# potamides/DeTikZify

Hardware: AMD Instinct MI355X
Metric: tikz_tokens_per_sec (higher is better)
Workload: dtype bf16; 1 GPU; detikzify-ds-7b (synthetic weights, seed 1234), 1 image 224x224->384x384, 243-token prefix, greedy decode of 512 tokens per rollout, batch 1 per GPU, hipGraph per token; rollouts_per_gpu=5

## Files before the change

### detikzify_amd/_lib.py

```python
from __future__ import annotations

import ctypes as C
import os
from pathlib import Path

_HERE = Path(__file__).resolve().parent
LIB_PATH = _HERE / "lib" / "libdtk_hip.so"

DTK_ABI_VERSION = 7
DTK_VIT_BATCH = 8
DTK_F32, DTK_BF16, DTK_F16 = 0, 1, 2
DTK_ARCH_PROJ_NO_BIAS = 1
DTK_PREFILL_REUSE_PREFIX, DTK_PREFILL_REUSE_IMAGE = 1, 2
DTK_MAX_INFLIGHT = 4
DTK_MAX_BATCH = 64
DTK_MAX_TOP = 8
DTK_EPI_BIAS, DTK_EPI_GELU, DTK_EPI_RESIDUAL, DTK_GEMM_NAIVE = 1, 2, 4, 256
DTK_GEMM_WT = 512
DTK_GEMM_SL = 1024
DTK_GEMM_KSLICES_SHIFT = 12


class DtkConfig(C.Structure):
    _fields_ = [
        ("hidden", C.c_int32), ("layers", C.c_int32), ("heads", C.c_int32), ("head_dim", C.c_int32),
        ("ffn", C.c_int32), ("vocab", C.c_int32), ("max_positions", C.c_int32),
        ("rms_eps", C.c_float), ("rope_theta", C.c_float), ("rope_factor", C.c_float),
        ("vit_dim", C.c_int32), ("vit_depth", C.c_int32), ("vit_heads", C.c_int32),
        ("vit_mlp", C.c_int32), ("vit_patch", C.c_int32), ("vit_image", C.c_int32),
        ("vit_feature_layer", C.c_int32), ("vit_ln_eps", C.c_float), ("vit_gelu_tanh", C.c_int32),
        ("concat_patches", C.c_int32), ("image_token_id", C.c_int32), ("attn_splits", C.c_int32),
        ("reserved", C.c_int32 * 7),
    ]


class DtkAdapterConfig(C.Structure):
    _fields_ = [
        ("every_n", C.c_int32), ("text_max", C.c_int32),
        ("hidden", C.c_int32), ("layers", C.c_int32), ("heads", C.c_int32), ("kv_heads", C.c_int32), ("head_dim", C.c_int32),
        ("ffn", C.c_int32), ("vocab", C.c_int32), ("rms_eps", C.c_float), ("rope_theta", C.c_float), ("rope_factor", C.c_float),
        ("rope_low_freq_factor", C.c_float), ("rope_high_freq_factor", C.c_float), ("rope_original_max_position", C.c_int32),
        ("reserved", C.c_int32 * 3),
    ]


class DtkSampling(C.Structure):
    _fields_ = [
        ("do_sample", C.c_int32), ("temperature", C.c_float), ("top_p", C.c_float),
        ("top_k", C.c_int32), ("seed", C.c_uint64),
        ("n_bad", C.c_int32), ("bad_ids", C.c_int32 * 8),
        ("n_begin_suppress", C.c_int32), ("begin_suppress_ids", C.c_int32 * 8),
        ("n_always_suppress", C.c_int32), ("always_suppress_ids", C.c_int32 * 8),
    ]


class DtkSamplingExt(C.Structure):
    _fields_ = [("min_p", C.c_float), ("epsilon_cutoff", C.c_float), ("reserved", C.c_int32 * 6)]


class DtkStats(C.Structure):
    _fields_ = [
        ("weight_bytes_per_token", C.c_uint64), ("kv_bytes_per_ctx_token", C.c_uint64),
        ("decode_steps", C.c_uint64), ("prefill_tokens", C.c_uint64), ("vit_images", C.c_uint64),
        ("last_prefill_ms", C.c_double), ("last_vit_ms", C.c_double),
        ("probe_kernel_ms_sum", C.c_double), ("probe_kernel_launches", C.c_uint64),
        ("probe_kernel_bytes", C.c_uint64), ("probe_event_pair_ms", C.c_double),
        ("last_batch_step_slots", C.c_uint32), ("device_errors", C.c_uint32),
        ("last_batch_step_fp8_mfma", C.c_uint32), ("reserved0", C.c_uint32),
    ]


class DtkJoin(C.Structure):
    _fields_ = [
        ("slot", C.c_int32), ("n_ids", C.c_int32), ("ids", C.c_void_p), ("pixels", C.c_void_p), ("image_key", C.c_uint64),
        ("try_resume", C.c_int32), ("n_candidates", C.c_int32), ("candidates", C.c_int32 * DTK_MAX_BATCH),
        ("prefix_len", C.c_int32), ("prefix_src", C.c_int32), ("prefix_src_whole", C.c_int32), ("prefix_encode", C.c_int32),
        ("prefix_in_place", C.c_int32), ("full_flags", C.c_int32), ("sampling", DtkSampling),
        ("max_new_tokens", C.c_int32), ("n_stop", C.c_int32), ("stop_ids", C.c_int64 * 8),
        ("flush_mode", C.c_int32), ("flush_max", C.c_int32), ("slot_out", C.c_int32), ("how_out", C.c_int32),
        ("error_out", C.c_char * 240),
    ]


class DtkEngineStats(C.Structure):
    _fields_ = [(n, C.c_uint64) for n in ("steps", "tokens_out", "joins", "resumed", "steps_below_half_occupancy", "host_bound_steps",
                                          "reader_wakeups", "wasted_slot_steps")] + \
               [(n, C.c_double) for n in ("wait_s", "launch_s", "join_s", "idle_s", "drain_s", "first_launch_t", "last_collect_t")]


_I32P, _I64P = C.POINTER(C.c_int32), C.POINTER(C.c_int64)


class DtkEngineOps(C.Structure):
    LAUNCH = C.CFUNCTYPE(C.c_int, C.c_void_p, _I32P)
    WAIT = C.CFUNCTYPE(C.c_int, C.c_void_p, _I64P)
    PREFILL = C.CFUNCTYPE(C.c_int, C.c_void_p, C.c_int, _I64P, C.c_int, C.c_void_p, C.c_uint64, C.c_int)
    SAMPLING = C.CFUNCTYPE(C.c_int, C.c_void_p, C.c_int, C.POINTER(DtkSampling))
    FORK = C.CFUNCTYPE(C.c_int, C.c_void_p, C.c_int, C.c_int, C.c_int)
    LCP = C.CFUNCTYPE(C.c_int, C.c_void_p, C.c_int, _I64P, C.c_int, C.c_uint64, C.POINTER(C.c_int))
    RESUME = C.CFUNCTYPE(C.c_int, C.c_void_p, C.c_int, _I64P, C.c_int, C.c_uint64)
    CTXLEN = C.CFUNCTYPE(C.c_int, C.c_void_p, C.c_int)
    LASTERR = C.CFUNCTYPE(C.c_void_p, C.c_void_p)
    PREFILL_TEXT = C.CFUNCTYPE(C.c_int, C.c_void_p, C.c_int, _I64P, C.c_int, C.c_void_p, C.c_uint64, _I64P, C.c_int, C.c_uint64, C.c_int)
    WAIT_LP = C.CFUNCTYPE(C.c_int, C.c_void_p, _I64P, C.POINTER(C.c_float), C.POINTER(C.c_float))
    SAMPLING_EXT = C.CFUNCTYPE(C.c_int, C.c_void_p, C.c_int, C.POINTER(DtkSamplingExt))
    PENALTIES = C.CFUNCTYPE(C.c_int, C.c_void_p, C.c_int, C.c_float, C.c_float, C.c_int)
    _fields_ = [
        ("dev", C.c_void_p), ("launch", LAUNCH), ("wait", WAIT), ("prefill_slot", PREFILL), ("set_sampling_slot", SAMPLING),
        ("kv_fork", FORK), ("slot_lcp", LCP), ("resume_slot", RESUME), ("context_len_slot", CTXLEN), ("last_error", LASTERR),
        ("max_positions", C.c_int32), ("decode_slots", C.c_int32),
    ]


DTK_JOIN_FULL, DTK_JOIN_FORK_TAIL, DTK_JOIN_FORK_WHOLE, DTK_JOIN_RESUMED, DTK_JOIN_IN_PLACE = range(5)
DTK_SEQ_RUNNING, DTK_SEQ_FINISHED, DTK_SEQ_LEFT = 1, 2, 3

_P = C.c_void_p
SYMBOLS = {
    "dtk_abi_version": (C.c_int, []),
    "dtk_abi_struct_size": (C.c_int, [C.c_int]),
    "dtk_last_error": (C.c_char_p, [_P]),
# ... 22 lines not shown
    "dtk_engine_create": (C.c_int, [_P, C.POINTER(_P)]),
    "dtk_engine_create_ops": (C.c_int, [C.POINTER(DtkEngineOps), C.POINTER(_P)]),
    "dtk_engine_destroy": (None, [_P]),
    "dtk_engine_last_error": (C.c_char_p, [_P]),
    "dtk_engine_set_flush_tokens": (C.c_int, [_P, C.POINTER(C.c_int64), C.c_int]),
    "dtk_engine_set_option": (C.c_int, [_P, C.c_char_p, C.c_int]),
    "dtk_engine_expect": (C.c_int, [_P, C.c_int, C.c_int]),
    "dtk_engine_join": (C.c_int, [_P, C.POINTER(DtkJoin)]),
    "dtk_engine_submit": (C.c_int, [_P, C.POINTER(DtkJoin), C.POINTER(C.c_uint64)]),
    "dtk_engine_await": (C.c_int, [_P, C.c_uint64]),
    "dtk_engine_read": (C.c_int, [_P, C.c_int, C.POINTER(C.c_int64), C.c_int, C.POINTER(C.c_int32), C.POINTER(C.c_int32), C.c_int]),
    "dtk_engine_leave": (C.c_int, [_P, C.c_int]),
    "dtk_engine_get_stats": (C.c_int, [_P, C.POINTER(DtkEngineStats)]),
    "dtk_engine_submit_text": (C.c_int, [_P, C.POINTER(DtkJoin), C.POINTER(C.c_int64), C.c_int, C.c_uint64, C.POINTER(C.c_uint64)]),
    "dtk_engine_set_prefill_text_op": (C.c_int, [_P, DtkEngineOps.PREFILL_TEXT]),
    "dtk_prefill_slot": (C.c_int, [_P, C.c_int, _P, C.c_int, _P, C.c_uint64, C.c_int, _P]),
    "dtk_set_sampling_slot": (C.c_int, [_P, C.c_int, C.POINTER(DtkSampling)]),
    "dtk_decode_batch_launch": (C.c_int, [_P, C.POINTER(C.c_int32)]),
    "dtk_decode_batch_wait": (C.c_int, [_P, C.POINTER(C.c_int64)]),
    "dtk_kv_fork": (C.c_int, [_P, C.c_int, C.c_int, C.c_int]),
    "dtk_get_logits_slot": (C.c_int, [_P, C.c_int, _P]),
    "dtk_context_len_slot": (C.c_int, [_P, C.c_int]),
    "dtk_slot_lcp": (C.c_int, [_P, C.c_int, _P, C.c_int, C.c_uint64, C.POINTER(C.c_int)]),
    "dtk_slot_cached_ids": (C.c_int, [_P, C.c_int, _P, C.c_int]),
    "dtk_resume_slot": (C.c_int, [_P, C.c_int, _P, C.c_int, C.c_uint64]),
    "dtk_bench_gemv": (C.c_int, [_P, C.c_int, C.c_int, C.c_int, C.POINTER(C.c_float)]),
    "dtk_set_gemv_variant": (C.c_int, [_P, C.c_int, C.c_int]),
    "dtk_set_option": (C.c_int, [_P, C.c_char_p, C.c_int]),
    "dtk_op_gemm": (C.c_int, [_P, _P, _P, _P, _P, C.c_int, C.c_int, C.c_int, C.c_int, _P]),
    "dtk_adapter_create": (C.c_int, [_P, C.POINTER(DtkAdapterConfig)]),
    "dtk_adapter_destroy": (C.c_int, [_P]),
    "dtk_has_adapter": (C.c_int, [_P]),
    "dtk_vit_encode_text": (C.c_int, [_P, _P, C.c_int, _P, C.c_int, C.c_uint64, _P, _P]),
    "dtk_prefill_text": (C.c_int, [_P, _P, C.c_int, _P, C.c_uint64, _P, C.c_int, C.c_uint64, C.c_int, _P]),
    "dtk_prefill_slot_text": (C.c_int, [_P, C.c_int, _P, C.c_int, _P, C.c_uint64, _P, C.c_int, C.c_uint64, C.c_int, _P]),
    "dtk_adapter_embed": (C.c_int, [_P, _P, C.c_int, _P]),
    "dtk_text_image_key": (C.c_uint64, [C.c_uint64, C.c_uint64]),
    "dtk_op_gemm_gated": (C.c_int, [_P, _P, _P, _P, _P, _P, C.c_int, C.c_int, C.c_int, C.c_int, _P]),
    "dtk_score": (C.c_int, [_P, _P, C.c_int, _P, C.c_uint64, C.c_uint32, C.c_int, _P, _P, _P]),
    "dtk_score_text": (C.c_int, [_P, _P, C.c_int, _P, C.c_uint64, _P, C.c_int, C.c_uint64, C.c_uint32, C.c_int, _P, _P, _P]),
    "dtk_op_score": (C.c_int, [_P, _P, _P, _P, C.c_int, C.c_int, C.c_int, C.c_int, _P, _P, _P, _P]),
    "dtk_score_packed": (C.c_int, [_P, _P, C.c_int, _P, C.c_uint64, C.c_uint32, _P, _P, C.c_int, _P, _P, _P]),
    "dtk_score_packed_text": (C.c_int, [_P, _P, C.c_int, _P, C.c_uint64, _P, C.c_int, C.c_uint64, C.c_uint32, _P, _P, C.c_int, _P, _P, _P]),
    "dtk_op_attention_seg": (C.c_int, [_P, _P, _P, _P, C.c_int, C.c_int, C.c_int, C.c_int, C.c_int, _P, _P, _P]),
    "dtk_op_attn_decode": (C.c_int, [_P, _P, _P, _P, C.c_int, C.c_int, C.c_int, C.c_int, _P, C.c_int, C.c_int, C.c_int, C.c_int, C.c_int,
                                     _P, _P, _P, _P]),
    "dtk_op_attn_decode_b": (C.c_int, [_P, _P, _P, _P, C.c_int, C.c_int, C.c_int, C.c_int, _P, _P, _P, _P,
                                       C.c_int, C.c_int, C.c_int, C.c_int, C.c_int, _P]),
    "dtk_op_gemv_b": (C.c_int, [_P, C.c_int, _P, _P, _P, C.c_int, C.c_int, _P, _P, C.c_float, _P, _P, C.c_int,
                                C.c_int, C.c_int, C.c_int, C.c_int, C.c_int, _P, _P, _P, _P, _P, _P, _P, _P, _P, _P]),
    "dtk_op_gemv_bkp": (C.c_int, [_P, _P, _P, _P, C.c_int, C.c_int, _P, _P, C.c_int, _P, C.c_float, _P, _P, _P, _P]),
    "dtk_op_gemv_role": (C.c_int, [_P, C.c_int, C.c_int, C.c_int, _P, _P, _P, _P, _P] + [C.c_int] * 9 + [C.c_float, _P, _P, _P, _P,
                                   C.c_int, _P, _P, _P, C.c_int, _P, _P, _P, _P, _P]),
    "dtk_op_gemv": (C.c_int, [_P, _P, _P, _P, C.c_int, C.c_int, C.c_int, C.c_float, _P]),
    "dtk_op_gemv_mv": (C.c_int, [_P, _P, _P, _P, C.c_int, C.c_int, C.c_int, C.c_float, C.c_int, _P]),
    "dtk_op_gemv_q4": (C.c_int, [_P, _P, _P, _P, C.c_int, C.c_int, C.c_int, C.c_float, _P, _P]),
    "dtk_mx_layout": (C.c_int, [C.c_int, C.c_int, C.c_int, _P, _P]),
    "dtk_op_gemv_mx": (C.c_int, [_P, _P, _P, _P, C.c_int, C.c_int, C.c_int, C.c_int, C.c_int, _P, _P, _P, _P, _P]),
    "dtk_op_attention": (C.c_int, [_P, _P, _P, _P, C.c_int, C.c_int, C.c_int, C.c_int, C.c_int, C.c_int, _P]),
    "dtk_op_layernorm": (C.c_int, [_P, _P, _P, _P, C.c_int, C.c_int, C.c_float, _P]),
    "dtk_op_sample": (C.c_int, [_P, _P, C.c_int, C.c_int, C.POINTER(C.c_int64), _P]),
    "dtk_decode_wait_lp": (C.c_int, [_P, C.POINTER(C.c_int64), C.POINTER(C.c_float)]),
    "dtk_decode_batch_wait_lp": (C.c_int, [_P, C.POINTER(C.c_int64), C.POINTER(C.c_float), C.POINTER(C.c_float)]),
    "dtk_engine_read_lp": (C.c_int, [_P, C.c_int, C.POINTER(C.c_int64), C.POINTER(C.c_float), C.POINTER(C.c_float), C.c_int,
                                     C.POINTER(C.c_int32), C.POINTER(C.c_int32), C.c_int]),
    "dtk_engine_set_wait_lp_op": (C.c_int, [_P, DtkEngineOps.WAIT_LP]),
    "dtk_op_sample_lp": (C.c_int, [_P, _P, C.c_int, C.c_int, C.POINTER(C.c_int64), _P, C.POINTER(C.c_float)]),
    "dtk_score_top": (C.c_int, [_P, _P, C.c_int, _P, C.c_uint64, C.c_uint32, C.c_int, _P, _P, _P, C.c_int, _P, _P]),
    "dtk_score_top_text": (C.c_int, [_P, _P, C.c_int, _P, C.c_uint64, _P, C.c_int, C.c_uint64, C.c_uint32, C.c_int, _P, _P, _P,
                                     C.c_int, _P, _P]),
    "dtk_score_packed_top": (C.c_int, [_P, _P, C.c_int, _P, C.c_uint64, C.c_uint32, _P, _P, C.c_int, _P, _P, _P, C.c_int, _P, _P]),
    "dtk_score_packed_top_text": (C.c_int, [_P, _P, C.c_int, _P, C.c_uint64, _P, C.c_int, C.c_uint64, C.c_uint32, _P, _P, C.c_int,
                                            _P, _P, _P, C.c_int, _P, _P]),
    "dtk_op_score_top": (C.c_int, [_P, _P, _P, _P, C.c_int, C.c_int, C.c_int, C.c_int, _P, _P, _P, _P, C.c_int, _P, _P, _P]),
    "dtk_decode_wait_top": (C.c_int, [_P, C.POINTER(C.c_int64), C.POINTER(C.c_float), C.POINTER(C.c_int32), C.POINTER(C.c_float)]),
    "dtk_decode_batch_wait_top": (C.c_int, [_P, C.POINTER(C.c_int64), C.POINTER(C.c_float), C.POINTER(C.c_float),
                                            C.POINTER(C.c_int32), C.POINTER(C.c_float)]),
    "dtk_set_sampling_ext": (C.c_int, [_P, C.POINTER(DtkSamplingExt)]),
    "dtk_set_sampling_slot_ext": (C.c_int, [_P, C.c_int, C.POINTER(DtkSamplingExt)]),
    "dtk_op_sample_ext": (C.c_int, [_P, _P, C.c_int, C.c_int, C.POINTER(C.c_int64), _P, C.POINTER(C.c_float), C.POINTER(DtkSamplingExt)]),
    "dtk_engine_submit_ext": (C.c_int, [_P, C.POINTER(DtkJoin), C.POINTER(DtkSamplingExt), C.POINTER(C.c_int64), C.c_int, C.c_uint64,
                                        C.POINTER(C.c_uint64)]),
    "dtk_engine_set_sampling_ext_op": (C.c_int, [_P, DtkEngineOps.SAMPLING_EXT]),
    "dtk_set_penalties": (C.c_int, [_P, C.c_float, C.c_float, C.c_int]),
    "dtk_set_penalties_slot": (C.c_int, [_P, C.c_int, C.c_float, C.c_float, C.c_int]),
    "dtk_op_sample_pen": (C.c_int, [_P, _P, C.c_int, C.c_int, C.POINTER(C.c_int64), _P, C.POINTER(C.c_float), C.POINTER(DtkSamplingExt),
                                    C.c_float, C.c_float, C.POINTER(C.c_int64), C.c_int]),
    "dtk_token_counts": (C.c_int, [_P, C.c_int, C.POINTER(C.c_uint16), C.c_int]),
    "dtk_engine_submit_pen": (C.c_int, [_P, C.POINTER(DtkJoin), C.POINTER(DtkSamplingExt), C.c_float, C.c_float, C.c_int,
                                        C.POINTER(C.c_int64), C.c_int, C.c_uint64, C.POINTER(C.c_uint64)]),
    "dtk_engine_set_penalties_op": (C.c_int, [_P, DtkEngineOps.PENALTIES]),
}

_lib = None


class DtkError(RuntimeError):
    pass


def load_library() -> C.CDLL:
    global _lib
    if _lib is not None:
        return _lib
    if not LIB_PATH.exists():
        raise DtkError(
# ... 37 lines not shown
```

### detikzify_amd/csrc/dtk_api.hip

```cpp
#include <hip/hip_runtime.h>

#include <cmath>
#include <cstdarg>
#include <cstdio>
#include <cstdlib>
#include <cstring>
#include <atomic>
#include <mutex>
#include <string>
#include <unordered_map>
#include <vector>

#include "../../include/dtk.h"
#include "kernels.h"
#include "mx_quant.h"

int& dtk_lds_attr_error(int device) {
  static int e[65] = {};
  return e[(device >= 0 && device < 64) ? device : 64];
}

namespace {

thread_local std::string g_create_error;
thread_local std::string g_thread_error;
thread_local const void* g_thread_error_ctx = nullptr;

struct TensorEntry {
  std::string name;
  bf16_t* ptr = nullptr;
  int64_t rows = 1;
  int64_t cols = 0;
  int64_t stride = 0;
  float synth_scale = 0.02f;
  float synth_offset = 0.f;
  bool loaded = false;
  int64_t numel() const { return rows * cols; }
};

struct SeqHost {
  std::vector<int64_t> cached_ids;
  bool cached_with_image = false;
  uint64_t image_key = 0;
  int host_next_pos = 0;
  bool have_logits = false;
  int share_src = -1;
  int share_len = 0;
  int last_reuse_start = 0;
  int64_t forced_pending = -1;
};

struct LayerW {
  bf16_t *wqkv, *wo, *wgu, *wdown, *ln1, *ln2;
  bf16_t *t_wqkv = nullptr, *t_wo = nullptr, *t_wgu = nullptr, *t_wdown = nullptr;
  bf16_t *p_wqkv = nullptr, *p_wo = nullptr, *p_wgu = nullptr, *p_wdown = nullptr;
  bf16_t* p_wgui = nullptr;
  uint8_t *q_wqkv = nullptr, *q_wo = nullptr, *q_wgu = nullptr, *q_wdown = nullptr;
  float *s_wqkv = nullptr, *s_wo = nullptr, *s_wgu = nullptr, *s_wdown = nullptr;
  uint8_t *f4_wqkv = nullptr, *f4_wo = nullptr, *f4_wgu = nullptr, *f4_wdown = nullptr;
  uint8_t *e4_wqkv = nullptr, *e4_wo = nullptr, *e4_wgu = nullptr, *e4_wdown = nullptr;
  uint8_t *t8_wqkv = nullptr, *t8_wo = nullptr, *t8_wgu = nullptr, *t8_wdown = nullptr;
  uint8_t *m_wqkv = nullptr, *m_wo = nullptr, *m_wgu = nullptr, *m_wdown = nullptr;
};
struct VitBlockW {
  bf16_t *n1w, *n1b, *qkvw, *qkvb, *projw, *projb, *n2w, *n2b, *fc1w, *fc1b, *fc2w, *fc2b;
};
struct CrossW {
  bf16_t *ln1w, *ln1b, *qw, *qb, *kw, *kb, *vw, *vb, *ow, *ob, *qnw, *qnb, *knw, *knb, *ln2w, *ln2b, *f1w, *f1b, *f2w, *f2b;
  bf16_t *gate_a, *gate_m;
  bf16_t *K, *V;
};
struct Adapter {
  dtk_adapter_config cfg{};
  dtk_ctx* emb = nullptr;
  unsigned char* arena = nullptr;
  size_t first_tensor = 0;
  bf16_t *conn_w = nullptr, *conn_b = nullptr, *dummy = nullptr, *ctext = nullptr;
  std::vector<CrossW> layers;
  std::vector<char> present;
  std::vector<int64_t> text_ids;
  std::vector<float> dummy_host;
};

}

struct dtk_ctx {
  dtk_config cfg;
  int device = 0;
  hipStream_t stream = nullptr;
  std::string err;
  std::mutex err_mu;
  std::mutex vit_mu;

  int d, L, H, ff, V, Tmax, S;
  int vD, vDepth, vH, vHd, vMlp, vN, vPatchK, vPatchLd, nImg;

  unsigned char* arena = nullptr;
  size_t arena_bytes = 0;
  std::vector<TensorEntry> tensors;
  std::unordered_map<std::string, int> tindex;
  std::vector<LayerW> layers;
  bf16_t *embed, *final_norm, *lm_head, *mm_w, *mm_b;
  bf16_t *rope_cos, *rope_sin;
  std::vector<VitBlockW> vblocks;
  bf16_t *pe_w, *pe_b, *pos_embed, *vnorm_w, *vnorm_b;
  bf16_t *ap_latent, *ap_qw, *ap_qb, *ap_kvw, *ap_kvb, *ap_pw, *ap_pb, *ap_nw, *ap_nb, *ap_f1w,
      *ap_f1b, *ap_f2w, *ap_f2b;

  bf16_t* kv = nullptr;

  bf16_t *X, *Xn, *QKV, *Qh, *AO, *GU, *ACT;
  int sk_sl_min_rows = SK_SL_MIN_ROWS;
  float* skpart = nullptr;
  size_t skpart_floats = 0;
  int swiglu_fused = 1;
  int qkv_rope_fused = 1;
  int prefill_sk = 1;
  int32_t* ids_dev = nullptr;
  float* score_rec = nullptr;
  float* score_out = nullptr;
  float* score_top = nullptr;
  int32_t* packed_rows = nullptr;
  bf16_t *x, *q, *act;
  float *logits, *pm, *pl, *po;
  bf16_t* attn_out = nullptr;
  unsigned* attn_ctr = nullptr;
  int attn_combine = 0;
  DecState* st = nullptr;
  SamplingDev* sp = nullptr;
  int64_t* tok_ring_dev = nullptr;
  int64_t* tok_ring_host = nullptr;
  float* probs_dev = nullptr;
  int logprobs = 0;
  std::atomic<int> engine_holds{0};
  float2* lp_ring_dev = nullptr;
  float2* lp_ring_host = nullptr;
  float2* lpb_dev = nullptr;
  float2* lpb_host = nullptr;
  int top_logprobs = 0;
  TopRec* top_ring_dev = nullptr;
  TopRec* top_ring_host = nullptr;
  float* lse_ring_dev = nullptr;
  float* lse_ring_host = nullptr;
  TopRec* topb_dev = nullptr;
  TopRec* topb_host = nullptr;
  float* lseb_dev = nullptr;
  float* lseb_host = nullptr;
  float* pixels_dev = nullptr;
  bf16_t *patches, *VX, *VN, *VQKV, *VAO, *VH, *feats, *last_hidden;
  bf16_t *pq, *pkv, *pao, *px, *pn, *ph, *pooled;
  bf16_t* IMG;
  Adapter* ad = nullptr;
  unsigned char* scratch = nullptr;
  size_t scratch_bytes = 0;

  SeqHost seq0;
  int wfmt = 0;
  bool fp8_ready = false;
  uint8_t* q_lm_head = nullptr;
  float* s_lm_head = nullptr;
  uint64_t cached_image_key = 0;
  bool have_image = false;
  int KVH = 0;
  int hd = 128;
  bool proj_bias = true;
  int nb = 0;
  bool share_reads = true;
  int nt = 1;
  std::vector<SeqHost> bseq;
  bf16_t* kvb = nullptr;
  size_t kv_slot_stride = 0;
  bf16_t *xb = nullptr, *xnb = nullptr, *qb = nullptr, *aob = nullptr, *actb = nullptr;
  float* logits_b = nullptr;
  float* kpart = nullptr; unsigned* kctr = nullptr;
  int attn_nt = 1;
  bool resid_kparts = true;
  float *pfx_m = nullptr, *pfx_l = nullptr, *pfx_o = nullptr;
  int prefix_mfma = 0;
  int pfx_splits = 4;
  int gqa_fused = 1;
  int tail_threads = 256;
  DecState* st_b = nullptr;
  SamplingDev* sp_b = nullptr;
  BatchState* bs_dev = nullptr;
  bf16_t* t_lm_head = nullptr;
  uint8_t* t8_lm_head = nullptr;
  uint8_t* m_lm_head = nullptr;
  uint8_t *xn8 = nullptr, *xns = nullptr, *ao8 = nullptr, *aos = nullptr, *act8 = nullptr, *acts = nullptr;
  bool mx_ok = false;
  int act_fp8 = 0;
  bool launch_refused = false;
  bool tiled_ready = false;
  bool ptiled_ready = false;
  BatchState* bs_host = nullptr;
  SamplingDev* sp_stage = nullptr; uint32_t* draw_stage = nullptr;
  DecState* st_stage = nullptr;
  int64_t* tokb_dev = nullptr;
  int64_t* tokb_host = nullptr;
  uint64_t blaunched = 0, bwaited = 0;
  hipEvent_t bstep_done[DTK_MAX_INFLIGHT] = {};
  bool bgraph_ready[6] = {false, false, false, false, false, false};
  hipGraph_t bgraph[6] = {nullptr, nullptr, nullptr, nullptr, nullptr, nullptr};
  hipGraphExec_t bgraph_exec[6] = {nullptr, nullptr, nullptr, nullptr, nullptr, nullptr};
  int nt_step = 1;
  int mv_slots = 4;
  int mv_step = 0;
  int mv_tail_threads = 512;
  dtk_sampling sampling{};
  SampleMB* smb = nullptr;
  SampleMB* smb_b = nullptr;
  bool mb_single = false;
  bool mb_batch = false;
  bool slot_topk[DTK_MAX_SLOTS] = {};
// ... 493 lines not shown
    a.nbatch = B; a.q_sb = 0; a.k_sb = a.v_sb = (long)N * 2 * D; a.o_sb = D;
    launch_attention(a, s);
  }
  gemm(c, c->pao, D, c->ap_pw, D, c->ap_pb, nullptr, 0, c->px, D, B, D, D, GEMM_BIAS);
  launch_layernorm_rows(c->px, D, c->ap_nw, c->ap_nb, c->pn, D, B, D, c->cfg.vit_ln_eps, s);
  gemm(c, c->pn, D, c->ap_f1w, D, c->ap_f1b, nullptr, 0, c->ph, mlp, B, mlp, D, GEMM_BIAS | gelu_flag(c));
  gemm(c, c->ph, mlp, c->ap_f2w, mlp, c->ap_f2b, c->px, D, c->pooled, D, B, D, mlp, GEMM_BIAS | GEMM_RESIDUAL);
}

void project_image(dtk_ctx* c) {
  const int K = c->cfg.concat_patches * c->vD;
  gemm(c, c->feats, K, c->mm_w, K, c->proj_bias ? c->mm_b : nullptr, nullptr, 0, c->IMG, c->d, c->nImg, c->d, K,
       c->proj_bias ? GEMM_BIAS : 0);
}

#define TOKB_ERR ((size_t)DTK_MAX_INFLIGHT * DTK_MAX_BATCH)
#define TOKB_WORDS (TOKB_ERR + 1)
static inline unsigned* batch_err_word(const dtk_ctx* c) { return reinterpret_cast<unsigned*>(c->tokb_dev + TOKB_ERR); }

#define LPB_BYTES (sizeof(float2) * (size_t)DTK_MAX_INFLIGHT * DTK_MAX_BATCH)
static inline hipError_t copy_lp_ring(dtk_ctx* c, bool batch) {
  if (!c->logprobs) return hipSuccess;
  if (c->top_logprobs) {
    hipError_t e = batch ? hipMemcpyAsync(c->topb_host, c->topb_dev, sizeof(TopRec) * (size_t)DTK_MAX_INFLIGHT * DTK_MAX_BATCH, hipMemcpyDeviceToHost, c->stream)
                         : hipMemcpyAsync(c->top_ring_host, c->top_ring_dev, sizeof(TopRec) * DTK_MAX_INFLIGHT, hipMemcpyDeviceToHost, c->stream);
    if (e != hipSuccess) return e;
    e = batch ? hipMemcpyAsync(c->lseb_host, c->lseb_dev, sizeof(float) * (size_t)DTK_MAX_INFLIGHT * DTK_MAX_BATCH, hipMemcpyDeviceToHost, c->stream)
              : hipMemcpyAsync(c->lse_ring_host, c->lse_ring_dev, sizeof(float) * DTK_MAX_INFLIGHT, hipMemcpyDeviceToHost, c->stream);
    if (e != hipSuccess) return e;
  }
  return batch ? hipMemcpyAsync(c->lpb_host, c->lpb_dev, LPB_BYTES, hipMemcpyDeviceToHost, c->stream)
               : hipMemcpyAsync(c->lp_ring_host, c->lp_ring_dev, sizeof(float2) * DTK_MAX_INFLIGHT, hipMemcpyDeviceToHost, c->stream);
}

static void pen_args(const dtk_ctx* c, SampleArgs& sa, bool batch) {
  if (!(batch ? c->pen_batch : c->pen_single) || !c->pen_tab) return;
  const int first = batch ? 1 : 0;
  sa.pen = c->pen_dev + first; sa.pen_cnt = c->pen_tab + (size_t)first * c->pen_stride; sa.pen_stride = c->pen_stride; sa.pen_tok = c->pen_tok + first;
}
static void sampler_launch(dtk_ctx* c, SampleArgs& sa, bool mb, bool batch) {
  pen_args(c, sa, batch);
  if (mb) launch_sample_mb(sa, c->stream); else launch_sample_b(sa, c->stream);
  if (sa.pen) launch_count_token(sa, c->stream);
}

static void top_logits_launch(dtk_ctx* c, const SampleArgs& sa) {
  if (!c->top_logprobs || !c->logprobs) return;
  TopArgs t;
  t.logits = sa.logits; t.V = sa.V; t.logits_stride = sa.logits_stride; t.st = sa.st; t.bs = sa.bs; t.nslots = sa.nslots;
  t.ring = sa.ring; t.k = c->top_logprobs; t.top_ring = sa.bs ? c->topb_dev : c->top_ring_dev;
  launch_top_logits(t, c->stream);
}

void decode_step_launches(dtk_ctx* c, bool with_probe, bool short_ctx = false) {
  hipStream_t s = c->stream;
  SampleArgs sa;
  sa.logits = c->logits; sa.V = c->V; sa.sp = c->sp; sa.st = c->st; sa.embed = c->embed;
  sa.x = c->x; sa.d = c->d; sa.tok_ring = c->tok_ring_dev; sa.ring = DTK_MAX_INFLIGHT;
  sa.probs_out = nullptr; sa.advance = 1; sa.step_override = -1; sa.bs = nullptr; sa.logits_stride = 0; sa.nslots = 1; sa.mb = c->smb;
  sa.lp_ring = c->logprobs ? c->lp_ring_dev : nullptr;
  sa.trunc = c->trunc_single ? 1 : 0;
  sa.lse_ring = (c->logprobs && c->top_logprobs) ? c->lse_ring_dev : nullptr;
  top_logits_launch(c, sa);
  sampler_launch(c, sa, c->mb_single, false);
  const float scale = 1.0f / sqrtf((float)c->hd);
  for (int l = 0; l < c->L; ++l) {
    const LayerW& w = c->layers[l];
    GemvArgs g{};
    g.eps = c->cfg.rms_eps; g.st = c->st; g.T_max = c->Tmax; g.d = c->d; g.ff = c->ff; g.H = c->H; g.KVH = c->KVH; g.hd = c->hd;
    g.rope_cos = c->rope_cos; g.rope_sin = c->rope_sin;
    g.pm = c->pm; g.pl = c->pl; g.po = c->po; g.S = c->S;
    g.W = w.wqkv; g.W8 = w.q_wqkv; g.wscale = w.s_wqkv; g.N = c->d + 2 * c->KVH * c->hd; g.K = c->d; g.x = c->x; g.norm_w = w.ln1;
    g.W4 = w.f4_wqkv; g.S4 = w.e4_wqkv;
    g.q_out = c->q; g.kcache = kcache(c, l); g.vcache = vcache(c, l);
    launch_gemv(PRO_RMSNORM, EPI_QKV, g, s);
    AttnDecArgs ad;
    ad.q = c->q; ad.kcache = kcache(c, l); ad.vcache = vcache(c, l); ad.st = c->st;
    ad.pm = c->pm; ad.pl = c->pl; ad.po = c->po; ad.H = c->H; ad.S = c->S; ad.T_max = c->Tmax; ad.G = c->H / c->KVH;
    ad.scale = scale; ad.hd = c->hd;
    ad.threads = c->attn_threads;
    ad.combine = (!ad.threads && short_ctx && c->attn_combine == 2) ? 3 : c->attn_combine; ad.out = c->attn_out; ad.counters = c->attn_ctr;
    if (ad.threads && ad.combine == 1) ad.combine = 2;
    launch_attn_decode(ad, s);
    g.W = w.wo; g.W8 = w.q_wo; g.wscale = w.s_wo; g.N = c->d; g.K = c->d; g.y = c->x;
    g.W4 = w.f4_wo; g.S4 = w.e4_wo;
    const bool partials = ad.combine == 0 && !(ad.threads && ad.S == 1);
    if (!partials) { g.x = c->attn_out; launch_gemv(PRO_COPY, EPI_RESID, g, s); }
    else launch_gemv(PRO_ATTN, EPI_RESID, g, s);
    g.W = w.wgu; g.W8 = w.q_wgu; g.wscale = w.s_wgu; g.N = 2 * c->ff; g.K = c->d; g.x = c->x; g.norm_w = w.ln2; g.y = c->act;
    g.W4 = w.f4_wgu; g.S4 = w.e4_wgu;
    const bool probe_here = with_probe && (l == c->L / 2);
    if (probe_here) (void)hipEventRecord(c->probe_a, s);
    launch_gemv(PRO_RMSNORM, EPI_SWIGLU, g, s);
    if (probe_here) (void)hipEventRecord(c->probe_b, s);
    g.W = w.wdown; g.W8 = w.q_wdown; g.wscale = w.s_wdown; g.N = c->d; g.K = c->ff; g.x = c->act; g.y = c->x;
    g.W4 = w.f4_wdown; g.S4 = w.e4_wdown;
    launch_gemv(PRO_COPY, EPI_RESID, g, s);
  }
  GemvArgs g{};
  g.W = c->lm_head; g.W8 = c->q_lm_head; g.wscale = c->s_lm_head; g.N = c->V; g.K = c->d; g.x = c->x; g.norm_w = c->final_norm;
  g.eps = c->cfg.rms_eps; g.logits = c->logits;
  launch_gemv(PRO_RMSNORM, EPI_LOGITS, g, s);
}

static inline bool mx_step(const dtk_ctx* c) { return c->wfmt == 1 && c->mx_ok && c->act_fp8 != 0; }

void batch_step_launches_mx(dtk_ctx* c) {
  hipStream_t s = c->stream;
  const int d = c->d, ff = c->ff, nslots = 16 * c->nt_step;
  SampleArgs sa;
  sa.logits = c->logits_b; sa.V = c->V; sa.sp = c->sp_b; sa.st = c->st_b; sa.embed = c->embed;
  sa.x = c->xb; sa.d = d; sa.tok_ring = c->tokb_dev; sa.ring = DTK_MAX_INFLIGHT;
  sa.probs_out = nullptr; sa.advance = 1; sa.step_override = -1; sa.bs = c->bs_dev; sa.logits_stride = c->V; sa.nslots = nslots; sa.mb = c->smb_b;
  sa.lp_ring = c->logprobs ? c->lpb_dev : nullptr;
  sa.trunc = c->trunc_batch ? 1 : 0;
  sa.lse_ring = (c->logprobs && c->top_logprobs) ? c->lseb_dev : nullptr;
  top_logits_launch(c, sa);
  sampler_launch(c, sa, c->mb_batch, true);
  const float scale = 1.0f / sqrtf(128.f);
  const size_t kv_layer = (size_t)2 * c->KVH * c->Tmax * 128;
  for (int l = 0; l < c->L; ++l) {
    const LayerW& w = c->layers[l];
    bf16_t* kc = c->kvb + (size_t)l * kv_layer;
    bf16_t* vc = kc + (size_t)c->KVH * c->Tmax * 128;
    GemvBArgs g{};
    g.bs = c->bs_dev; g.st = c->st_b; g.T_max = c->Tmax; g.d = d; g.ff = ff; g.H = c->H; g.KVH = c->KVH; g.nt = c->nt_step;
    g.rope_cos = c->rope_cos; g.rope_sin = c->rope_sin; g.kv_slot_stride = c->kv_slot_stride; g.kpart = c->kpart; g.err = batch_err_word(c);
    if (l == 0) launch_rmsnorm_b(c->xb, d, w.ln1, c->xnb, d, d, c->cfg.rms_eps, c->bs_dev, nslots, s, c->xn8, c->xns);
    g.Wm = w.m_wqkv; g.wscale = w.s_wqkv; g.N = d + 2 * c->KVH * 128; g.K = d; g.X8 = c->xn8; g.XS = c->xns; g.q_out = c->qb; g.kcache = kc; g.vcache = vc;
    launch_gemv_mxu(EPI_QKV, g, s);
    AttnDecBArgs ad;
    ad.q = c->qb; ad.kcache = kc; ad.vcache = vc; ad.kv_slot_stride = c->kv_slot_stride; ad.st = c->st_b; ad.bs = c->bs_dev;
    ad.out = c->aob; ad.H = c->H; ad.T_max = c->Tmax; ad.d = d; ad.G = c->H / c->KVH; ad.nslots = nslots;
    ad.scale = scale;
    ad.use_prefix = c->prefix_mfma; ad.pfx_splits = c->pfx_splits; ad.tail_threads = c->tail_threads; ad.gqa_fused = c->gqa_fused; ad.nt_private = c->attn_nt;
    ad.pfx_m = c->pfx_m; ad.pfx_l = c->pfx_l; ad.pfx_o = c->pfx_o;
    ad.out8 = c->ao8; ad.outs = c->aos;
    launch_attn_decode_b(ad, s);
    g.Wm = w.m_wo; g.wscale = w.s_wo; g.N = d; g.K = d; g.X8 = c->ao8; g.XS = c->aos;
    if (!launch_gemv_mxk(g, 32, s)) c->launch_refused = true;
    launch_resid_norm_b(c->kpart, c->xb, d, w.ln2, c->xnb, d, c->cfg.rms_eps, c->bs_dev, nslots, s, c->xn8, c->xns);
    g.Wm = w.m_wgu; g.wscale = w.s_wgu; g.N = 2 * ff; g.K = d; g.X8 = c->xn8; g.XS = c->xns; g.Y8 = c->act8; g.YS = c->acts;
    launch_gemv_mxu(EPI_SWIGLU, g, s);
    g.Wm = w.m_wdown; g.wscale = w.s_wdown; g.N = d; g.K = ff; g.X8 = c->act8; g.XS = c->acts;
    if (!launch_gemv_mxk(g, 16, s)) c->launch_refused = true;
    launch_resid_norm_b(c->kpart, c->xb, d, l + 1 < c->L ? c->layers[l + 1].ln1 : c->final_norm, c->xnb, d, c->cfg.rms_eps, c->bs_dev, nslots, s, c->xn8, c->xns);
  }
  GemvBArgs g{};
  g.bs = c->bs_dev; g.st = c->st_b; g.Wm = c->m_lm_head; g.wscale = c->s_lm_head; g.N = c->V; g.K = d; g.X8 = c->xn8; g.XS = c->xns; g.logits = c->logits_b;
  g.d = d; g.ff = ff; g.nt = c->nt_step; g.H = c->H; g.KVH = c->KVH; g.err = batch_err_word(c);
  launch_gemv_mxu(EPI_LOGITS, g, s);
}
// ... 84 lines not shown
  const float scale = 1.0f / sqrtf(128.f);
  const size_t kv_layer = (size_t)2 * c->KVH * c->Tmax * 128;
  GemvMvArgs g{};
  g.bs = c->bs_dev; g.st = c->st_b; g.T_max = c->Tmax; g.d = d; g.ff = ff; g.H = c->H; g.KVH = c->KVH; g.eps = c->cfg.rms_eps;
  g.rope_cos = c->rope_cos; g.rope_sin = c->rope_sin; g.kv_slot_stride = c->kv_slot_stride;
  for (int l = 0; l < c->L; ++l) {
    const LayerW& w = c->layers[l];
    bf16_t* kc = c->kvb + (size_t)l * kv_layer;
    bf16_t* vc = kc + (size_t)c->KVH * c->Tmax * 128;
    g.W = w.wqkv; g.W8 = w.q_wqkv; g.wscale = w.s_wqkv; g.N = d + 2 * c->KVH * 128; g.K = d; g.X = c->xb; g.ldx = d; g.norm_w = w.ln1;
    g.q_out = c->qb; g.kcache = kc; g.vcache = vc;
    launch_gemv_mv(PRO_RMSNORM, EPI_QKV, NB, g, s);
    AttnDecBArgs ad;
    ad.q = c->qb; ad.kcache = kc; ad.vcache = vc; ad.kv_slot_stride = c->kv_slot_stride; ad.st = c->st_b; ad.bs = c->bs_dev;
    ad.out = c->aob; ad.H = c->H; ad.T_max = c->Tmax; ad.d = d; ad.G = c->H / c->KVH; ad.nslots = NB;
    ad.scale = scale;
    ad.use_prefix = 0; ad.pfx_splits = c->pfx_splits; ad.tail_threads = c->mv_tail_threads; ad.gqa_fused = c->gqa_fused; ad.nt_private = c->attn_nt;
    ad.pfx_m = c->pfx_m; ad.pfx_l = c->pfx_l; ad.pfx_o = c->pfx_o;
    launch_attn_decode_b(ad, s);
    g.W = w.wo; g.W8 = w.q_wo; g.wscale = w.s_wo; g.N = d; g.K = d; g.X = c->aob; g.Y = c->xb; g.ldy = d;
    launch_gemv_mv(PRO_COPY, EPI_RESID, NB, g, s);
    g.W = w.wgu; g.W8 = w.q_wgu; g.wscale = w.s_wgu; g.N = 2 * ff; g.K = d; g.X = c->xb; g.ldx = d; g.norm_w = w.ln2; g.Y = c->actb; g.ldy = ff;
    launch_gemv_mv(PRO_RMSNORM, EPI_SWIGLU, NB, g, s);
    g.W = w.wdown; g.W8 = w.q_wdown; g.wscale = w.s_wdown; g.N = d; g.K = ff; g.X = c->actb; g.Y = c->xb; g.ldy = d;
    launch_gemv_mv(PRO_COPY, EPI_RESID, NB, g, s);
  }
  g.W = c->lm_head; g.W8 = c->q_lm_head; g.wscale = c->s_lm_head; g.N = c->V; g.K = d; g.X = c->xb; g.ldx = d; g.norm_w = c->final_norm;
  g.logits = c->logits_b;
  launch_gemv_mv(PRO_RMSNORM, EPI_LOGITS, NB, g, s);
}

void ensure_fp8_weights(dtk_ctx* c) {
  if (c->wfmt == 0 || c->fp8_ready) return;
  for (int l = 0; l < c->L && c->wfmt == 2; ++l) {
    LayerW& w = c->layers[l];
    launch_quant_mxfp4_rows(w.wqkv, w.f4_wqkv, w.e4_wqkv, c->d + 2 * c->KVH * c->hd, c->d, c->stream);
    launch_quant_mxfp4_rows(w.wo, w.f4_wo, w.e4_wo, c->d, c->d, c->stream);
    launch_quant_mxfp4_rows(w.wgu, w.f4_wgu, w.e4_wgu, 2 * c->ff, c->d, c->stream);
    launch_quant_mxfp4_rows(w.wdown, w.f4_wdown, w.e4_wdown, c->d, c->ff, c->stream);
  }
  for (int l = 0; l < c->L && c->wfmt == 1; ++l) {
    LayerW& w = c->layers[l];
    launch_quant_fp8_rows(w.wqkv, w.q_wqkv, w.s_wqkv, c->d + 2 * c->KVH * c->hd, c->d, c->stream);
    launch_quant_fp8_rows(w.wo, w.q_wo, w.s_wo, c->d, c->d, c->stream);
    launch_quant_fp8_rows(w.wgu, w.q_wgu, w.s_wgu, 2 * c->ff, c->d, c->stream);
    launch_quant_fp8_rows(w.wdown, w.q_wdown, w.s_wdown, c->d, c->ff, c->stream);
  }
  launch_quant_fp8_rows(c->lm_head, c->q_lm_head, c->s_lm_head, c->V, c->d, c->stream);
  c->fp8_ready = true;
  c->tiled_ready = false;
  c->ptiled_ready = false;
}

void ensure_tiled_weights(dtk_ctx* c);
void ensure_prefill_tiles(dtk_ctx* c) {
  ensure_fp8_weights(c);
  if (c->ptiled_ready) return;
  for (int l = 0; l < c->L; ++l)
    if (c->layers[l].p_wgui) launch_retile_pairs(c->layers[l].wgu, c->layers[l].p_wgui, c->ff, c->d, c->stream);
  if (c->nb > 0 && c->wfmt != 1) { ensure_tiled_weights(c); c->ptiled_ready = true; return; }
  for (int l = 0; l < c->L; ++l) {
    LayerW& w = c->layers[l];
    launch_retile(w.wqkv, w.p_wqkv, c->d + 2 * c->KVH * c->hd, c->d, c->stream);
    launch_retile(w.wo, w.p_wo, c->d, c->d, c->stream);
    launch_retile(w.wgu, w.p_wgu, 2 * c->ff, c->d, c->stream);
    launch_retile(w.wdown, w.p_wdown, c->d, c->ff, c->stream);
  }
  c->ptiled_ready = true;
}

void ensure_tiled_weights(dtk_ctx* c) {
  ensure_fp8_weights(c);
  if (c->tiled_ready || c->nb <= 0) return;
  if (c->wfmt == 1) {
    const int qkvn = c->d + 2 * c->KVH * 128;
    for (int l = 0; l < c->L; ++l) {
      LayerW& w = c->layers[l];
      launch_retile_f8(w.q_wqkv, w.t8_wqkv, qkvn, c->d, c->stream);
      launch_retile_f8(w.q_wo, w.t8_wo, c->d, c->d, c->stream);
      launch_retile_f8(w.q_wgu, w.t8_wgu, 2 * c->ff, c->d, c->stream);
      launch_retile_f8(w.q_wdown, w.t8_wdown, c->d, c->ff, c->stream);
    }
    launch_retile_f8(c->q_lm_head, c->t8_lm_head, c->V, c->d, c->stream);
    if (c->mx_ok) {
      for (int l = 0; l < c->L; ++l) {
        LayerW& w = c->layers[l];
        launch_retile_mx(w.q_wqkv, w.m_wqkv, qkvn, c->d, 32, c->stream);
        launch_retile_mx(w.q_wo, w.m_wo, c->d, c->d, 32, c->stream);
        launch_retile_mx(w.q_wgu, w.m_wgu, 2 * c->ff, c->d, 32, c->stream);
        launch_retile_mx(w.q_wdown, w.m_wdown, c->d, c->ff, 16, c->stream);
      }
      launch_retile_mx(c->q_lm_head, c->m_lm_head, c->V, c->d, 32, c->stream);
    }
    c->tiled_ready = true;
    return;
  }
  for (int l = 0; l < c->L; ++l) {
    LayerW& w = c->layers[l];
    launch_retile(w.wqkv, w.t_wqkv, c->d + 2 * c->KVH * 128, c->d, c->stream);
    launch_retile(w.wo, w.t_wo, c->d, c->d, c->stream);
    launch_retile(w.wgu, w.t_wgu, 2 * c->ff, c->d, c->stream);
    launch_retile(w.wdown, w.t_wdown, c->d, c->ff, c->stream);
  }
  launch_retile(c->lm_head, c->t_lm_head, c->V, c->d, c->stream);
  c->tiled_ready = true;
}
// ... 232 lines not shown
  if (const char* fm = getenv("DTK_ATTN_FULL_MAX")) c->attn_full_max = atoi(fm);
  if (const char* gv = getenv("DTK_GEMV_VARIANTS")) {
    int e = 0, v = 0;
    const char* p = gv;
    while (sscanf(p, "%d:%d", &e, &v) == 2) {
      set_gemv_default_variant(e, v);
      p = strchr(p, ',');
      if (!p) break;
      ++p;
    }
  }

#define CCHK(call)                                                                         \
  do {                                                                                     \
    hipError_t e_ = (call);                                                                \
    if (e_ != hipSuccess) {                                                                \
      fail(nullptr, DTK_ERR_HIP, "%s failed: %s", #call, hipGetErrorString(e_));           \
      dtk_destroy(c);                                                                      \
      return DTK_ERR_HIP;                                                                  \
    }                                                                                      \
  } while (0)
  CCHK(hipSetDevice(device));
  CCHK(hipStreamCreateWithFlags(&c->stream, hipStreamNonBlocking));
  CCHK(hipStreamCreateWithFlags(&c->stream_vit, hipStreamNonBlocking));
  Planner sz;
  plan(c, sz, false);
  c->arena_bytes = align_up(sz.off, 256) + 256;
  CCHK(hipMalloc((void**)&c->arena, c->arena_bytes));
  Planner real;
  real.base = c->arena;
  plan(c, real, true);
  CCHK(hipMemsetAsync(c->arena, 0, c->arena_bytes, c->stream));
  CCHK(hipHostMalloc((void**)&c->tok_ring_host, sizeof(int64_t) * DTK_MAX_INFLIGHT, hipHostMallocDefault));
  CCHK(hipHostMalloc((void**)&c->lp_ring_host, sizeof(float2) * DTK_MAX_INFLIGHT, hipHostMallocDefault));
  for (int i = 0; i < DTK_MAX_INFLIGHT; ++i) CCHK(hipEventCreateWithFlags(&c->step_done[i], hipEventDisableTiming));
  if (c->nb > 0) {
    CCHK(hipHostMalloc((void**)&c->bs_host, sizeof(BatchState) * DTK_MAX_INFLIGHT, hipHostMallocDefault));
    CCHK(hipHostMalloc((void**)&c->tokb_host, sizeof(int64_t) * TOKB_WORDS, hipHostMallocDefault));
    CCHK(hipHostMalloc((void**)&c->lpb_host, LPB_BYTES, hipHostMallocDefault));
    CCHK(hipHostMalloc((void**)&c->st_stage, sizeof(DecState) * (DTK_MAX_SLOTS), hipHostMallocDefault));
    CCHK(hipHostMalloc((void**)&c->sp_stage, sizeof(SamplingDev) * (DTK_MAX_SLOTS), hipHostMallocDefault));
    CCHK(hipHostMalloc((void**)&c->draw_stage, sizeof(uint32_t) * (DTK_MAX_SLOTS), hipHostMallocDefault));
    for (int i = 0; i < DTK_MAX_INFLIGHT; ++i) CCHK(hipEventCreateWithFlags(&c->bstep_done[i], hipEventDisableTiming));
  }
  CCHK(hipEventCreate(&c->ev_a)); CCHK(hipEventCreate(&c->ev_b)); CCHK(hipEventCreate(&c->ev_c));
  CCHK(hipEventCreate(&c->ev_va)); CCHK(hipEventCreate(&c->ev_vb));
  CCHK(hipEventCreate(&c->probe_a)); CCHK(hipEventCreate(&c->probe_b));
  std::vector<uint16_t> cosv, sinv;
  compute_rope_tables(*cfg, cosv, sinv);
  CCHK(hipMemcpyAsync(c->rope_cos, cosv.data(), cosv.size() * 2, hipMemcpyHostToDevice, c->stream));
  CCHK(hipMemcpyAsync(c->rope_sin, sinv.data(), sinv.size() * 2, hipMemcpyHostToDevice, c->stream));
  CCHK(hipStreamSynchronize(c->stream));
#undef CCHK
  const uint64_t kvd = (uint64_t)c->KVH * c->hd;
  const uint64_t attn_lin = (uint64_t)2 * c->d * c->d + 2 * kvd * c->d;
  const uint64_t per_layer = attn_lin + (uint64_t)3 * c->d * c->ff + 2 * (uint64_t)c->d;
  c->stats.weight_bytes_per_token = 2 * (per_layer * c->L + (uint64_t)c->d + (uint64_t)c->V * c->d);
  if (c->wfmt == 1) {
    const uint64_t lin = attn_lin + (uint64_t)3 * c->d * c->ff;
    const uint64_t rows = (uint64_t)3 * c->d + 2 * kvd + (uint64_t)2 * c->ff;
    c->stats.weight_bytes_per_token = (lin + 4 * rows + 4 * (uint64_t)c->d) * c->L + 2 * (uint64_t)c->d + (uint64_t)c->V * c->d + 4 * (uint64_t)c->V;
  }
  if (c->wfmt == 2) {
    const uint64_t bd = mxfp4_row_scales(c->d), bf = mxfp4_row_scales(c->ff);
    const uint64_t blocks = ((uint64_t)2 * c->d + 2 * kvd + (uint64_t)2 * c->ff) * bd + (uint64_t)c->d * bf;
    c->stats.weight_bytes_per_token = (17 * blocks + 4 * (uint64_t)c->d) * c->L + 2 * (uint64_t)c->d + (uint64_t)c->V * c->d + 4 * (uint64_t)c->V;
  }
  c->stats.kv_bytes_per_ctx_token = (uint64_t)2 * c->L * kvd * 2;
  c->stats.probe_kernel_bytes = (uint64_t)2 * c->ff * c->d * (c->wfmt == 1 ? 1 : 2);
  if (c->wfmt == 2) c->stats.probe_kernel_bytes = (uint64_t)2 * c->ff * 17 * mxfp4_row_scales(c->d);
  *out = c;
  if (c->nb > 0) {
    const bool big = max_decode_slots(c) >= 64;
    c->prefix_mfma = big ? 1 : 0;
    c->tail_threads = big ? 128 : 256;
  }
  if (const char* opts = getenv("DTK_OPTIONS")) {
    std::string all(opts);
    size_t at = 0;
    while (at < all.size()) {
      size_t end = all.find(',', at);
      if (end == std::string::npos) end = all.size();
      const std::string item = all.substr(at, end - at);
      const size_t eq = item.find('=');
      if (eq != std::string::npos && dtk_set_option(c, item.substr(0, eq).c_str(), atoi(item.c_str() + eq + 1)) != DTK_OK)
        fprintf(stderr, "DTK_OPTIONS: %s rejected (%s)\n", item.c_str(), c->err.c_str());
      at = end + 1;
    }
  }
  return DTK_OK;
}

void dtk_destroy(dtk_ctx* c) {
  if (!c) return;
  (void)hipSetDevice(c->device);
  if (c->ad) (void)dtk_adapter_destroy(c);
  if (c->stream) (void)hipStreamSynchronize(c->stream);
  if (c->graph_exec) (void)hipGraphExecDestroy(c->graph_exec);
  if (c->graph) (void)hipGraphDestroy(c->graph);
  if (c->graph_short_exec) (void)hipGraphExecDestroy(c->graph_short_exec);
  if (c->graph_short) (void)hipGraphDestroy(c->graph_short);
  drop_batch_graphs(c);
  for (int i = 0; i < DTK_MAX_INFLIGHT; ++i) if (c->bstep_done[i]) (void)hipEventDestroy(c->bstep_done[i]);
  if (c->bs_host) (void)hipHostFree(c->bs_host);
  if (c->tokb_host) (void)hipHostFree(c->tokb_host);
  if (c->lpb_host) (void)hipHostFree(c->lpb_host);
  if (c->lp_ring_host) (void)hipHostFree(c->lp_ring_host);
  if (c->st_stage) (void)hipHostFree(c->st_stage);
  if (c->sp_stage) (void)hipHostFree(c->sp_stage);
  if (c->draw_stage) (void)hipHostFree(c->draw_stage);
  for (int i = 0; i < DTK_MAX_INFLIGHT; ++i) if (c->step_done[i]) (void)hipEventDestroy(c->step_done[i]);
  hipEvent_t evs[] = {c->ev_a, c->ev_b, c->ev_c, c->probe_a, c->probe_b};
  for (hipEvent_t e : evs) if (e) (void)hipEventDestroy(e);
  if (c->tok_ring_host) (void)hipHostFree(c->tok_ring_host);
  if (c->arena) (void)hipFree(c->arena);
  if (c->score_rec) (void)hipFree(c->score_rec);
  if (c->score_out) (void)hipFree(c->score_out);
  if (c->score_top) (void)hipFree(c->score_top);
  if (c->pen_tab) (void)hipFree(c->pen_tab);
  if (c->pen_dev) (void)hipFree(c->pen_dev);
  if (c->pen_tok) (void)hipFree(c->pen_tok);
  if (c->pen_ids_dev) (void)hipFree(c->pen_ids_dev);
  if (c->pen_ids_stage) (void)hipHostFree(c->pen_ids_stage);
  if (c->pen_stage) (void)hipHostFree(c->pen_stage);
  if (c->top_ring_dev) (void)hipFree(c->top_ring_dev);
  if (c->lse_ring_dev) (void)hipFree(c->lse_ring_dev);
  if (c->topb_dev) (void)hipFree(c->topb_dev);
  if (c->lseb_dev) (void)hipFree(c->lseb_dev);
  if (c->top_ring_host) (void)hipHostFree(c->top_ring_host);
  if (c->lse_ring_host) (void)hipHostFree(c->lse_ring_host);
  if (c->topb_host) (void)hipHostFree(c->topb_host);
  if (c->lseb_host) (void)hipHostFree(c->lseb_host);
  if (c->packed_rows) (void)hipFree(c->packed_rows);
  if (c->stream_vit) (void)hipStreamDestroy(c->stream_vit);
  if (c->ev_va) (void)hipEventDestroy(c->ev_va);
  if (c->ev_vb) (void)hipEventDestroy(c->ev_vb);
  if (c->stream) (void)hipStreamDestroy(c->stream);
  delete c;
}

int dtk_num_tensors(const dtk_ctx* c) { return c ? (int)c->tensors.size() : 0; }
const char* dtk_tensor_name(const dtk_ctx* c, int i) {
  if (!c || i < 0 || i >= (int)c->tensors.size()) return nullptr;
  return c->tensors[i].name.c_str();
}
int64_t dtk_tensor_numel(const dtk_ctx* c, const char* name) {
  if (!c || !name) return -1;
  auto it = c->tindex.find(name);
  return it == c->tindex.end() ? -1 : c->tensors[it->second].numel();
}

int dtk_load_tensor(dtk_ctx* c, const char* name, const void* host, int dtype, const int64_t* shape, int ndim) {
  if (!c || !name || !host || !shape || ndim < 1) return fail(c, DTK_ERR_ARG, "dtk_load_tensor: null argument");
  auto it = c->tindex.find(name);
  if (it == c->tindex.end()) return fail(c, DTK_ERR_ARG, "unknown tensor '%s'", name);
  TensorEntry& t = c->tensors[it->second];
  int64_t n = 1;
  for (int i = 0; i < ndim; ++i) n *= shape[i];
  if (n != t.numel()) return fail(c, DTK_ERR_ARG, "tensor '%s': %lld elements given, %lld expected", name, (long long)n, (long long)t.numel());
  HIPCHK(c, hipSetDevice(c->device));
  std::vector<uint16_t> tmp;
  const uint16_t* src16 = nullptr;
  if (dtype == DTK_BF16) {
    src16 = static_cast<const uint16_t*>(host);
  } else if (dtype == DTK_F32) {
    tmp.resize((size_t)n);
    const float* f = static_cast<const float*>(host);
    for (int64_t i = 0; i < n; ++i) tmp[(size_t)i] = host_f2bf(f[i]);
    src16 = tmp.data();
  } else if (dtype == DTK_F16) {
    tmp.resize((size_t)n);
    const uint16_t* hf = static_cast<const uint16_t*>(host);
    for (int64_t i = 0; i < n; ++i) tmp[(size_t)i] = host_f2bf(host_h2f(hf[i]));
    src16 = tmp.data();
  } else {
    return fail(c, DTK_ERR_ARG, "bad dtype %d", dtype);
  }
  HIPCHK(c, hipStreamSynchronize(c->stream));
  HIPCHK(c, hipMemcpy2D(t.ptr, (size_t)t.stride * 2, src16, (size_t)t.cols * 2, (size_t)t.cols * 2, (size_t)t.rows, hipMemcpyHostToDevice));
  t.loaded = true;
  if (c->ad) { c->ad->text_ids.clear(); c->ad->dummy_host.clear(); c->ad->emb->ptiled_ready = false; }
  c->have_image = false;
  c->seq0.cached_ids.clear();
  for (auto& b : c->bseq) b.cached_ids.clear();
  pen_clear_all(c);
  c->tiled_ready = false;
  c->ptiled_ready = false;
  c->fp8_ready = false;
  return DTK_OK;
}

int dtk_read_tensor(dtk_ctx* c, const char* name, void* host_out, int64_t n_elems) {
  if (!c || !name || !host_out) return fail(c, DTK_ERR_ARG, "dtk_read_tensor: null argument");
  auto it = c->tindex.find(name);
  if (it == c->tindex.end()) return fail(c, DTK_ERR_ARG, "unknown tensor '%s'", name);
  const TensorEntry& t = c->tensors[it->second];
  if (n_elems != t.numel()) return fail(c, DTK_ERR_ARG, "tensor '%s' has %lld elements", name, (long long)t.numel());
  HIPCHK(c, hipSetDevice(c->device));
  ensure_fp8_weights(c);
  HIPCHK(c, hipStreamSynchronize(c->stream));
  HIPCHK(c, hipMemcpy2D(host_out, (size_t)t.cols * 2, t.ptr, (size_t)t.stride * 2, (size_t)t.cols * 2, (size_t)t.rows, hipMemcpyDeviceToHost));
  return DTK_OK;
}

int dtk_fill_synthetic(dtk_ctx* c, uint64_t seed) {
  if (!c) return DTK_ERR_ARG;
  HIPCHK(c, hipSetDevice(c->device));
  for (size_t i = 0; i < c->tensors.size(); ++i) {
    TensorEntry& t = c->tensors[i];
    if (t.name == "rope.cos" || t.name == "rope.sin" || t.name == "embedding_model.rope.cos" || t.name == "embedding_model.rope.sin") continue;
    t.loaded = true;
    if (t.stride == t.cols) {
      launch_fill_synth(t.ptr, t.numel(), seed, (uint32_t)i, t.synth_scale, t.synth_offset, c->stream);
    } else {
      if ((size_t)t.numel() * 2 > c->scratch_bytes) return fail(c, DTK_ERR_ARG, "scratch too small");
      bf16_t* tmp = reinterpret_cast<bf16_t*>(c->scratch);
      launch_fill_synth(tmp, t.numel(), seed, (uint32_t)i, t.synth_scale, t.synth_offset, c->stream);
      HIPCHK(c, hipMemcpy2DAsync(t.ptr, (size_t)t.stride * 2, tmp, (size_t)t.cols * 2, (size_t)t.cols * 2, (size_t)t.rows, hipMemcpyDeviceToDevice, c->stream));
    }
  }
  HIPCHK(c, hipStreamSynchronize(c->stream));
  if (c->ad) { c->ad->text_ids.clear(); c->ad->dummy_host.clear(); c->ad->emb->ptiled_ready = false; }
  c->have_image = false;
  c->seq0.cached_ids.clear();
  for (auto& b : c->bseq) b.cached_ids.clear();
  pen_clear_all(c);
  c->tiled_ready = false;
  c->ptiled_ready = false;
  c->fp8_ready = false;
  return DTK_OK;
}

static int vit_encode_impl(dtk_ctx* c, const float* pixels, int batch, void* feats_out, void* pooled_out, const int64_t* text_ids, int T_text);
static int text_prepare(dtk_ctx* c, const int64_t* ids, int T, hipStream_t s);
int dtk_vit_encode(dtk_ctx* c, const float* pixels, int batch, void* feats_out, void* pooled_out) {
  return vit_encode_impl(c, pixels, batch, feats_out, pooled_out, nullptr, 0);
}

static int vit_encode_impl(dtk_ctx* c, const float* pixels, int batch, void* feats_out, void* pooled_out, const int64_t* text_ids, int T_text) {
  if (!c || !pixels || batch < 1) return fail(c, DTK_ERR_ARG, "dtk_vit_encode: bad argument");
  if (pooled_out) {
    for (const TensorEntry& t : c->tensors)
      if (!t.loaded && t.name.compare(0, 23, "vision_model.attn_pool.") == 0)
        return fail(c, DTK_ERR_STATE, "pooler_output requested but '%s' was never loaded (checkpoint without the pooling head)", t.name.c_str());
  }
  std::lock_guard<std::mutex> vit_guard(c->vit_mu);
  HIPCHK(c, hipSetDevice(c->device));
  const size_t img = (size_t)3 * c->cfg.vit_image * c->cfg.vit_image;
  hipStream_t sv = c->stream_vit;
  const bf16_t* hidden = (pooled_out && c->cfg.vit_feature_layer != c->vDepth - 1) ? c->last_hidden : c->feats;
  if (text_ids) { const int rc = text_prepare(c, text_ids, T_text, sv); if (rc != DTK_OK) return rc; }
  for (int b0 = 0; b0 < batch; b0 += DTK_VIT_BATCH) {
    const int B = std::min(batch - b0, (int)DTK_VIT_BATCH);
    HIPCHK(c, hipMemcpyAsync(c->pixels_dev, pixels + (size_t)b0 * img, (size_t)B * img * 4, hipMemcpyHostToDevice, sv));
    HIPCHK(c, hipEventRecord(c->ev_va, sv));
    vit_forward(c, pooled_out != nullptr, sv, B, text_ids != nullptr);
    HIPCHK(c, hipEventRecord(c->ev_vb, sv));
    if (feats_out)
      HIPCHK(c, hipMemcpyAsync((bf16_t*)feats_out + (size_t)b0 * c->vN * c->vD, hidden, (size_t)B * c->vN * c->vD * 2, hipMemcpyDeviceToHost, sv));
    if (pooled_out)
      HIPCHK(c, hipMemcpyAsync((bf16_t*)pooled_out + (size_t)b0 * c->vD, c->pooled, (size_t)B * c->vD * 2, hipMemcpyDeviceToHost, sv));
    HIPCHK(c, hipStreamSynchronize(sv));
    HIPCHK(c, hipGetLastError());
    float ms = 0.f;
    if (hipEventElapsedTime(&ms, c->ev_va, c->ev_vb) == hipSuccess) c->stats.last_vit_ms = ms / (float)B;
    c->stats.vit_images += (uint64_t)B;
  }
  return DTK_OK;
}

struct PackedRows { const int2* rope; const int2* seg; int shared_len; };
static void decoder_layers(dtk_ctx* c, int n, int start, int T, bf16_t* kvbase, hipStream_t s, const PackedRows* pk = nullptr) {
  const int hd = c->hd, d = c->d, ff = c->ff;
  const size_t kv_layer = (size_t)2 * c->KVH * c->Tmax * hd;
  auto kc = [&](int l) { return kvbase + (size_t)l * kv_layer; };
  auto vc = [&](int l) { return kvbase + (size_t)l * kv_layer + (size_t)c->KVH * c->Tmax * hd; };
  const float scale = 1.0f / sqrtf((float)hd);
  for (int l = 0; l < c->L; ++l) {
    const LayerW& w = c->layers[l];
    const int qkvn = d + 2 * c->KVH * hd;
    if (!qkv_rope_fused(c, w, n, start, kc(l), vc(l), s, pk ? pk->rope : nullptr)) {
      gemm_role(c, c->Xn, d, w.wqkv, w.p_wqkv, d, nullptr, 0, c->QKV, qkvn, n, qkvn, d, 0, nullptr, nullptr, 0);
// ... 831 lines not shown
  sh.cached_ids.resize((size_t)T - 1);
  sh.forced_pending = ids[T - 1];
  if (const int rc = pen_rebuild(c, 1 + slot, ids, T)) return rc;
  sh.host_next_pos = T - 1;
  sh.have_logits = true;
  sh.last_reuse_start = T - 1;
  DecState& st0 = c->st_stage[slot];
  st0 = DecState{};
  st0.pos = T - 2; st0.next_pos = T - 1; st0.token = (int32_t)ids[T - 2]; st0.draw = 0; st0.force_plus1 = (int32_t)ids[T - 1] + 1;
  HIPCHK(c, hipMemcpyAsync(c->st_b + slot, &st0, sizeof st0, hipMemcpyHostToDevice, c->stream));
  return DTK_OK;
}

int dtk_get_logits_slot(dtk_ctx* c, int slot, float* out) {
  if (!c || !out || slot < 0 || slot >= c->nb) return fail(c, DTK_ERR_ARG, "dtk_get_logits_slot: bad argument");
  if (!c->bseq[(size_t)slot].have_logits) return fail(c, DTK_ERR_STATE, "no logits yet");
  HIPCHK(c, hipSetDevice(c->device));
  HIPCHK(c, hipStreamSynchronize(c->stream));
  HIPCHK(c, hipMemcpy(out, c->logits_b + (size_t)slot * c->V, (size_t)c->V * 4, hipMemcpyDeviceToHost));
  return DTK_OK;
}

int dtk_context_len_slot(const dtk_ctx* c, int slot) {
  return (c && slot >= 0 && slot < c->nb) ? c->bseq[(size_t)slot].host_next_pos : -1;
}

int dtk_set_graph_mode(dtk_ctx* c, int enabled) {
  if (!c) return DTK_ERR_ARG;
  c->use_graph = enabled == 1;
  c->probe = enabled == 2;
  if (c->probe && c->stats.probe_event_pair_ms == 0.0) {
    HIPCHK(c, hipSetDevice(c->device));
    HIPCHK(c, hipStreamSynchronize(c->stream));
    double sum = 0.0; int n = 0;
    for (int i = 0; i < 40; ++i) {
      HIPCHK(c, hipEventRecord(c->probe_a, c->stream));
      HIPCHK(c, hipEventRecord(c->probe_b, c->stream));
      HIPCHK(c, hipEventSynchronize(c->probe_b));
      float ms = 0.f;
      if (hipEventElapsedTime(&ms, c->probe_a, c->probe_b) == hipSuccess && i >= 8) { sum += ms; ++n; }
    }
    if (n) c->stats.probe_event_pair_ms = sum / n;
  }
  return DTK_OK;
}

int dtk_decode_launch(dtk_ctx* c) {
  if (!c) return DTK_ERR_ARG;
  if (!c->seq0.have_logits) return fail(c, DTK_ERR_STATE, "dtk_decode before dtk_prefill");
  if (c->launched - c->waited >= DTK_MAX_INFLIGHT) return fail(c, DTK_ERR_STATE, "too many decode steps in flight");
  if (c->seq0.host_next_pos >= c->Tmax) return fail(c, DTK_ERR_RANGE, "context length %d reached max_positions", c->seq0.host_next_pos);
  HIPCHK(c, hipSetDevice(c->device));
  ensure_fp8_weights(c);
  if (c->use_graph) {
    int rc = ensure_graph(c);
    if (rc) return rc;
    const bool short_ctx = c->seq0.host_next_pos < c->attn_full_max;
    HIPCHK(c, hipGraphLaunch(short_ctx ? c->graph_short_exec : c->graph_exec, c->stream));
  } else {
    if (c->probe && c->launched > c->waited) HIPCHK(c, hipStreamSynchronize(c->stream));
    if (c->probe && c->probe_pending) {
      float ms = 0.f;
      HIPCHK(c, hipStreamSynchronize(c->stream));
      if (hipEventElapsedTime(&ms, c->probe_a, c->probe_b) == hipSuccess) {
        c->stats.probe_kernel_ms_sum += ms;
        c->stats.probe_kernel_launches++;
      }
      c->probe_pending = false;
    }
    decode_step_launches(c, c->probe != 0, c->seq0.host_next_pos < c->attn_full_max);
    if (c->probe) c->probe_pending = true;
    HIPCHK(c, hipMemcpyAsync(c->tok_ring_host, c->tok_ring_dev, sizeof(int64_t) * DTK_MAX_INFLIGHT, hipMemcpyDeviceToHost, c->stream));
    HIPCHK(c, copy_lp_ring(c, false));
  }
  HIPCHK(c, hipEventRecord(c->step_done[c->launched % DTK_MAX_INFLIGHT], c->stream));
  c->launched++;
  c->seq0.host_next_pos++;
  c->stats.decode_steps++;
  c->seq0.cached_ids.push_back(-1);
  return DTK_OK;
}

static int decode_wait_impl(dtk_ctx* c, int64_t* token_out, float* lp_out, int32_t* top_ids_out = nullptr, float* top_logprob_out = nullptr) {
  if (c->waited >= c->launched) return fail(c, DTK_ERR_STATE, "no decode step in flight");
  HIPCHK(c, hipSetDevice(c->device));
  const uint64_t k = c->waited;
  HIPCHK(c, hipEventSynchronize(c->step_done[k % DTK_MAX_INFLIGHT]));
  const int64_t tok = ((volatile int64_t*)c->tok_ring_host)[k % DTK_MAX_INFLIGHT];
  *token_out = tok;
  if (lp_out) {
    const volatile float* lp = (volatile float*)(c->lp_ring_host + k % DTK_MAX_INFLIGHT);
    lp_out[0] = lp[0]; lp_out[1] = lp[1];
  }
  if (top_ids_out)
    top_unpack(c->top_ring_host + k % DTK_MAX_INFLIGHT, c->lse_ring_host + k % DTK_MAX_INFLIGHT, c->top_logprobs, top_ids_out, top_logprob_out);
  const size_t idx = c->seq0.cached_ids.size() - (size_t)(c->launched - k);
  c->seq0.cached_ids[idx] = tok;
  c->waited++;
  return DTK_OK;
}

int dtk_decode_wait(dtk_ctx* c, int64_t* token_out) {
  if (!c || !token_out) return fail(c, DTK_ERR_ARG, "dtk_decode_wait: null argument");
  return decode_wait_impl(c, token_out, nullptr);
}

int dtk_decode_wait_lp(dtk_ctx* c, int64_t* token_out, float* lp_out) {
  if (!c || !token_out || !lp_out) return fail(c, DTK_ERR_ARG, "dtk_decode_wait_lp: null argument");
  if (!c->logprobs) return fail(c, DTK_ERR_ARG, "dtk_decode_wait_lp: the context does not compute log-probabilities (dtk_set_option \"logprobs\", 1)");
  return decode_wait_impl(c, token_out, lp_out);
}

int dtk_decode_wait_top(dtk_ctx* c, int64_t* token_out, float* lp_out, int32_t* top_ids_out, float* top_logprob_out) {
  if (!c || !token_out || !lp_out || !top_ids_out || !top_logprob_out) return fail(c, DTK_ERR_ARG, "dtk_decode_wait_top: null argument");
  if (!c->logprobs || !c->top_logprobs)
    return fail(c, DTK_ERR_ARG, "dtk_decode_wait_top: the context does not compute top-k alternatives (dtk_set_option \"logprobs\", 1 and \"top_logprobs\", k)");
  return decode_wait_impl(c, token_out, lp_out, top_ids_out, top_logprob_out);
}

int dtk_decode(dtk_ctx* c, int64_t* token_out) {
  int rc = dtk_decode_launch(c);
  if (rc) return rc;
  return dtk_decode_wait(c, token_out);
}

int dtk_get_logits(dtk_ctx* c, float* out) {
  if (!c || !out) return fail(c, DTK_ERR_ARG, "dtk_get_logits: null argument");
  if (!c->seq0.have_logits) return fail(c, DTK_ERR_STATE, "no logits yet");
  HIPCHK(c, hipSetDevice(c->device));
  HIPCHK(c, hipStreamSynchronize(c->stream));
  HIPCHK(c, hipMemcpy(out, c->logits, (size_t)c->V * 4, hipMemcpyDeviceToHost));
  return DTK_OK;
}

int dtk_context_len(const dtk_ctx* c) { return c ? c->seq0.host_next_pos : -1; }

int dtk_synchronize(dtk_ctx* c) {
  if (!c) return DTK_ERR_ARG;
  HIPCHK(c, hipSetDevice(c->device));
  HIPCHK(c, hipStreamSynchronize(c->stream));
  HIPCHK(c, hipGetLastError());
  return DTK_OK;
}

int dtk_get_stats(dtk_ctx* c, dtk_stats* out) {
  if (!c || !out) return DTK_ERR_ARG;
  *out = c->stats;
  return DTK_OK;
}

int dtk_bench_gemv(dtk_ctx* c, int role, int variant, int reps, float* avg_us) {
  if (!c || !avg_us || reps < 1) return fail(c, DTK_ERR_ARG, "dtk_bench_gemv: bad argument");
  HIPCHK(c, hipSetDevice(c->device));
  hipStream_t s = c->stream;
  if (role < 0 || role > 4) return fail(c, DTK_ERR_ARG, "dtk_bench_gemv: role %d (0 qkv, 1 o_proj, 2 gate/up, 3 down, 4 lm_head)", role);
  const bool same_layer = (variant & 0x100) != 0;
  const int plain = (variant >> 9) & 3;
  const bool fmt = (variant & 0x800) != 0;
  if (fmt && ((variant & 0xff) != 0xff || plain))
    return fail(c, DTK_ERR_ARG, "dtk_bench_gemv: 0x800 (the context's weight format) goes with variant 0xff only");
  if (fmt) ensure_fp8_weights(c);
  variant &= 0xff;
  const bool shipped = variant == 0xff;
  auto launch = [&](int pro, int epi, const GemvArgs& g) { if (shipped) launch_gemv(pro, epi, g, s); else launch_gemv_variant(pro, epi, variant, g, s); };
  auto one_pass = [&]() {
    for (int l = 0; l < c->L; ++l) {
      const LayerW& w = c->layers[same_layer ? 0 : l];
      GemvArgs g{};
      if (plain) {
        g.eps = c->cfg.rms_eps; g.y = c->GU;
        if (role == 0) { g.W = w.wqkv; g.N = c->d + 2 * c->KVH * c->hd; g.K = c->d; g.x = c->x; g.norm_w = w.ln1; }
        else if (role == 1) { g.W = w.wo; g.N = c->d; g.K = c->d; g.x = c->attn_out; g.norm_w = w.ln1; }
        else if (role == 2) { g.W = w.wgu; g.N = 2 * c->ff; g.K = c->d; g.x = c->x; g.norm_w = w.ln2; }
        else if (role == 3) { g.W = w.wdown; g.N = c->d; g.K = c->ff; g.x = c->act; g.norm_w = w.ln2; }
        else { g.W = c->lm_head; g.N = c->V; g.K = c->d; g.x = c->x; g.norm_w = c->final_norm; }
        launch_gemv_variant(plain == 2 ? PRO_RMSNORM : PRO_COPY, EPI_STORE, variant, g, s);
        continue;
      }
      g.eps = c->cfg.rms_eps; g.st = c->st; g.T_max = c->Tmax; g.d = c->d; g.ff = c->ff; g.H = c->H; g.KVH = c->KVH; g.hd = c->hd;
      g.rope_cos = c->rope_cos; g.rope_sin = c->rope_sin; g.pm = c->pm; g.pl = c->pl; g.po = c->po; g.S = c->S;
      if (fmt) {
        if (role == 0) { g.W8 = w.q_wqkv; g.wscale = w.s_wqkv; g.W4 = w.f4_wqkv; g.S4 = w.e4_wqkv; }
        else if (role == 1) { g.W8 = w.q_wo; g.wscale = w.s_wo; g.W4 = w.f4_wo; g.S4 = w.e4_wo; }
        else if (role == 2) { g.W8 = w.q_wgu; g.wscale = w.s_wgu; g.W4 = w.f4_wgu; g.S4 = w.e4_wgu; }
        else if (role == 3) { g.W8 = w.q_wdown; g.wscale = w.s_wdown; g.W4 = w.f4_wdown; g.S4 = w.e4_wdown; }
        else { g.W8 = c->q_lm_head; g.wscale = c->s_lm_head; }
      }
      if (role == 0) { g.W = w.wqkv; g.N = c->d + 2 * c->KVH * c->hd; g.K = c->d; g.x = c->x; g.norm_w = w.ln1; g.q_out = c->q; g.kcache = kcache(c, l); g.vcache = vcache(c, l); launch(PRO_RMSNORM, EPI_QKV, g); }
      else if (role == 1) { g.W = w.wo; g.N = c->d; g.K = c->d; g.x = c->attn_out; g.y = c->q; launch(PRO_COPY, EPI_RESID, g); }
      else if (role == 2) { g.W = w.wgu; g.N = 2 * c->ff; g.K = c->d; g.x = c->x; g.norm_w = w.ln2; g.y = c->act; launch(PRO_RMSNORM, EPI_SWIGLU, g); }
      else if (role == 3) { g.W = w.wdown; g.N = c->d; g.K = c->ff; g.x = c->act; g.y = c->q; launch(PRO_COPY, EPI_RESID, g); }
      else { g.W = c->lm_head; g.N = c->V; g.K = c->d; g.x = c->x; g.norm_w = c->final_norm; g.logits = c->logits; launch(PRO_RMSNORM, EPI_LOGITS, g); }
    }
  };
  one_pass();
  HIPCHK(c, hipEventRecord(c->ev_a, s));
  for (int r = 0; r < reps; ++r) one_pass();
  HIPCHK(c, hipEventRecord(c->ev_b, s));
  HIPCHK(c, hipStreamSynchronize(s));
  HIPCHK(c, hipGetLastError());
  float ms = 0.f;
  HIPCHK(c, hipEventElapsedTime(&ms, c->ev_a, c->ev_b));
  *avg_us = ms * 1e3f / (float)(reps * c->L);
  c->seq0.have_logits = false;
  return DTK_OK;
}

int dtk_set_option(dtk_ctx* c, const char* name, int value) {
  if (!c || !name) return DTK_ERR_ARG;
  HIPCHK(c, hipSetDevice(c->device));
  HIPCHK(c, hipStreamSynchronize(c->stream));
  if (!strcmp(name, "attn_full_max")) c->attn_full_max = value;
  else if (!strcmp(name, "logprobs")) {
    if (value != 0 && value != 1) return fail(c, DTK_ERR_ARG, "logprobs must be 0 or 1");
    if (value == 0 && c->top_logprobs) return fail(c, DTK_ERR_STATE, "logprobs: top_logprobs = %d needs it (set \"top_logprobs\" to 0 first)", c->top_logprobs);
    if ((value != 0) != (c->logprobs != 0)) {
      if (c->blaunched != c->bwaited) return fail(c, DTK_ERR_STATE, "logprobs: a batch step is in flight");
      if (c->engine_holds.load() > 0) return fail(c, DTK_ERR_STATE, "logprobs: an engine holds %d sequence(s) in this context's slots", c->engine_holds.load());
      if (c->launched != c->waited) return fail(c, DTK_ERR_STATE, "logprobs: %d single-sequence decode step(s) are unread", (int)(c->launched - c->waited));
      c->logprobs = value; drop_graph(c); drop_batch_graphs(c);
    }
  }
  else if (!strcmp(name, "top_logprobs")) {
    if (value < 0 || value > DTK_MAX_TOP) return fail(c, DTK_ERR_ARG, "top_logprobs must be 0 .. %d", DTK_MAX_TOP);
    if (value > c->V) return fail(c, DTK_ERR_ARG, "top_logprobs = %d exceeds the vocabulary (%d)", value, c->V);
    if (value != 0 && !c->logprobs) return fail(c, DTK_ERR_STATE, "top_logprobs needs logprobs = 1 (dtk_set_option \"logprobs\", 1 first)");
    if (value != c->top_logprobs) {
      if (c->blaunched != c->bwaited) return fail(c, DTK_ERR_STATE, "top_logprobs: a batch step is in flight");
      if (c->engine_holds.load() > 0) return fail(c, DTK_ERR_STATE, "top_logprobs: an engine holds %d sequence(s) in this context's slots", c->engine_holds.load());
      if (c->launched != c->waited) return fail(c, DTK_ERR_STATE, "top_logprobs: %d single-sequence decode step(s) are unread", (int)(c->launched - c->waited));
      if (value) {
        const size_t n1 = DTK_MAX_INFLIGHT, nb = c->nb > 0 ? (size_t)DTK_MAX_INFLIGHT * DTK_MAX_BATCH : 0;
        if (!c->top_ring_dev) { HIPCHK(c, hipMalloc(&c->top_ring_dev, sizeof(TopRec) * n1)); HIPCHK(c, hipMemset(c->top_ring_dev, 0, sizeof(TopRec) * n1)); }
        if (!c->lse_ring_dev) { HIPCHK(c, hipMalloc(&c->lse_ring_dev, sizeof(float) * n1)); HIPCHK(c, hipMemset(c->lse_ring_dev, 0, sizeof(float) * n1)); }
        if (!c->top_ring_host) HIPCHK(c, hipHostMalloc((void**)&c->top_ring_host, sizeof(TopRec) * n1, hipHostMallocDefault));
        if (!c->lse_ring_host) HIPCHK(c, hipHostMalloc((void**)&c->lse_ring_host, sizeof(float) * n1, hipHostMallocDefault));
        if (nb && !c->topb_dev) { HIPCHK(c, hipMalloc(&c->topb_dev, sizeof(TopRec) * nb)); HIPCHK(c, hipMemset(c->topb_dev, 0, sizeof(TopRec) * nb)); }
        if (nb && !c->lseb_dev) { HIPCHK(c, hipMalloc(&c->lseb_dev, sizeof(float) * nb)); HIPCHK(c, hipMemset(c->lseb_dev, 0, sizeof(float) * nb)); }
        if (nb && !c->topb_host) HIPCHK(c, hipHostMalloc((void**)&c->topb_host, sizeof(TopRec) * nb, hipHostMallocDefault));
        if (nb && !c->lseb_host) HIPCHK(c, hipHostMalloc((void**)&c->lseb_host, sizeof(float) * nb, hipHostMallocDefault));
      }
      c->top_logprobs = value; drop_graph(c); drop_batch_graphs(c);
    }
  }
  else if (!strcmp(name, "gemm_tile")) {
    if (value < 0 || value > 5) return fail(c, DTK_ERR_ARG, "gemm_tile must be 0..5");
    set_gemm_tile(value);
  }
  else if (!strcmp(name, "share_prefix_reads")) c->share_reads = value != 0;
  else if (!strcmp(name, "prefix_mfma") || !strcmp(name, "pfx_splits") || !strcmp(name, "gemv_b_wide") ||
           !strcmp(name, "tail_threads")) {
    if (!strcmp(name, "prefix_mfma")) c->prefix_mfma = value != 0;
    else if (!strcmp(name, "tail_threads")) { if (value != 64 && value != 128 && value != 256 && value != 512) return fail(c, DTK_ERR_ARG, "tail_threads must be 64, 128, 256 or 512"); c->tail_threads = value; }
    else if (!strcmp(name, "pfx_splits")) { if (value < 1 || value > 4) return fail(c, DTK_ERR_ARG, "pfx_splits must be 1..4"); c->pfx_splits = value; }
    else { if (value < 0 || value > 6) return fail(c, DTK_ERR_ARG, "gemv_b_wide must be 0..6"); set_gemv_b_wide(value); }
    drop_batch_graphs(c);
  }
  else if (!strcmp(name, "gemm_impl")) {
    if (value < 0 || value > 4 || value == 1) return fail(c, DTK_ERR_ARG, "gemm_impl must be 0 (registers), 2 (k_gemm_glds where the shape has the tiles), 3 (auto) or 4 (k_gemm_g3: 8 waves, 3 LDS stages)");
    set_gemm_impl(value);
  }
  else if (!strcmp(name, "gemm_g3_min_blocks")) {
    if (value < 1) return fail(c, DTK_ERR_ARG, "gemm_g3_min_blocks must be >= 1");
    set_gemm_g3_min_blocks(value);
  }
// ... 800 lines not shown
  HIPCHK(c, hipMemcpyAsync(dq, q, (size_t)nslots * d * 2, hipMemcpyHostToDevice, s));
  HIPCHK(c, hipMemcpyAsync(dst, hst.data(), sizeof(DecState) * (size_t)nslots, hipMemcpyHostToDevice, s));
  HIPCHK(c, hipMemcpyAsync(dbs, &hbs, sizeof hbs, hipMemcpyHostToDevice, s));
  HIPCHK(c, hipMemsetAsync(dout, 0xFF, out_elems * 2, s));
  HIPCHK(c, hipMemsetAsync(dm, 0xFF, recs * 4, s));
  HIPCHK(c, hipMemsetAsync(dl, 0xFF, recs * 4, s));
  HIPCHK(c, hipMemsetAsync(dpo, 0xFF, recs * 128 * 4, s));
  AttnDecBArgs ad;
  ad.q = dq; ad.kcache = dK; ad.vcache = dV; ad.kv_slot_stride = kv_slot; ad.st = dst; ad.bs = dbs;
  ad.out = dout; ad.H = H; ad.T_max = T_max; ad.d = d; ad.G = G; ad.nslots = nslots; ad.scale = 1.0f / sqrtf(128.f);
  ad.use_prefix = use_prefix != 0; ad.pfx_splits = pfx_splits; ad.tail_threads = tail_threads; ad.gqa_fused = gqa_fused; ad.nt_private = attn_nt != 0;
  ad.pfx_m = dm; ad.pfx_l = dl; ad.pfx_o = dpo;
  launch_attn_decode_b(ad, s);
  HIPCHK(c, hipGetLastError());
  std::vector<bf16_t> frag(out_elems);
  HIPCHK(c, hipMemcpyAsync(frag.data(), dout, out_elems * 2, hipMemcpyDeviceToHost, s));
  HIPCHK(c, hipStreamSynchronize(s));
  HIPCHK(c, hipGetLastError());
  for (int j = 0; j < nslots; ++j)
    for (int k = 0; k < d; ++k)
      out[(size_t)j * d + k] = frag[((size_t)((j >> 4) * nsteps + (k >> 5)) * 64 + ((k & 31) >> 3) * 16 + (j & 15)) * 8 + (k & 7)];
  return DTK_OK;
}

static bool gemv_role_variant_ok(int fmt, int pro, int epi, int v) {
  if (fmt == 2) {
    const bool pair = (pro == PRO_RMSNORM && (epi == EPI_QKV || epi == EPI_SWIGLU || epi == EPI_STORE)) || (pro == PRO_ATTN && epi == EPI_RESID) ||
                      (pro == PRO_COPY && (epi == EPI_RESID || epi == EPI_STORE));
    return pair && v == -1;
  }
  if (fmt == 1) {
    const bool pair = (pro == PRO_RMSNORM && (epi == EPI_QKV || epi == EPI_SWIGLU || epi == EPI_LOGITS)) || ((pro == PRO_ATTN || pro == PRO_COPY) && epi == EPI_RESID);
    return pair && v >= -1 && v <= 9;
  }
  if (v < -1) return false;
  if (pro == PRO_RMSNORM && (epi == EPI_QKV || epi == EPI_SWIGLU)) return v <= 11;
  if (pro == PRO_COPY && epi == EPI_RESID) return v <= 22;
  if (pro == PRO_ATTN && epi == EPI_RESID) return v <= 8;
  if (pro == PRO_RMSNORM && epi == EPI_LOGITS) return v <= 4;
  if (pro == PRO_RMSNORM && epi == EPI_STORE) return v <= 0 || v == 20;
  if (pro == PRO_COPY && epi == EPI_STORE) return v <= 0 || v == 20 || v == 21;
  return false;
}

int dtk_op_gemv_role(dtk_ctx* c, int pro, int epi, int variant, const uint16_t* W, const uint8_t* W8, const float* wscale,
                     const uint8_t* W4, const uint8_t* S4, int N, int K, int d, int ff, int H, int KVH, int hd, int T_max, int pos, float eps,
                     const uint16_t* x, const uint16_t* norm_w, const uint16_t* rope_cos, const uint16_t* rope_sin,
                     int S, const float* pm, const float* pl, const float* po, int scratch_fill,
                     uint16_t* q_io, uint16_t* k_io, uint16_t* v_io, uint16_t* y_io, float* logits_io) {
  if (!c) return DTK_ERR_ARG;
  if ((W != nullptr) + (W8 != nullptr) + (W4 != nullptr) != 1 || (W8 && !wscale) || (!W8 && wscale) || (!W4 != !S4))
    return fail(c, DTK_ERR_ARG, "dtk_op_gemv_role: exactly one of W | W8 + wscale | W4 + S4");
  const int fmt = W4 ? 2 : (W8 ? 1 : 0);
  if (N < 1 || K < 8 || (K & 7) || (fmt == 1 && (K & 15))) return fail(c, DTK_ERR_ARG, "dtk_op_gemv_role: N >= 1, K a multiple of 8 (16 for fp8 weights)");
  if (pro < PRO_COPY || pro > PRO_ATTN || epi < EPI_STORE || epi > EPI_LOGITS) return fail(c, DTK_ERR_ARG, "dtk_op_gemv_role: unknown prologue %d or epilogue %d", pro, epi);
  if (!gemv_role_variant_ok(fmt, pro, epi, variant))
    return fail(c, DTK_ERR_ARG, "dtk_op_gemv_role: no %s kernel for prologue %d, epilogue %d, variant %d", fmt == 2 ? "MXFP4" : (fmt == 1 ? "fp8" : "bf16"), pro, epi, variant);
  if (hd != 128 && hd != 64) return fail(c, DTK_ERR_ARG, "dtk_op_gemv_role: head dim %d (128 or 64)", hd);
  if (scratch_fill < 0 || scratch_fill > 255 || d < 0) return fail(c, DTK_ERR_ARG, "dtk_op_gemv_role: scratch_fill is a byte, d >= 0");
  if (pro == PRO_ATTN) {
    if (S < 1 || S > 16) return fail(c, DTK_ERR_ARG, "dtk_op_gemv_role: S must be 1..16");
    if (H < 1 || K != H * hd || !pm || !pl || !po) return fail(c, DTK_ERR_ARG, "dtk_op_gemv_role: PRO_ATTN needs K = H * hd and the partials pm / pl / po");
  } else if (!x || (pro == PRO_RMSNORM && !norm_w)) return fail(c, DTK_ERR_ARG, "dtk_op_gemv_role: x (and norm_w for PRO_RMSNORM) required");
  if (epi == EPI_QKV) {
    if (H < 1 || KVH < 1 || H % KVH) return fail(c, DTK_ERR_ARG, "dtk_op_gemv_role: H %d query heads over KVH %d key / value heads", H, KVH);
    if (N != (H + 2 * KVH) * hd || d != H * hd) return fail(c, DTK_ERR_ARG, "dtk_op_gemv_role: QKV needs N = (H + 2 KVH) * hd and d = H * hd");
    if (T_max < 1 || pos < 0 || pos >= T_max) return fail(c, DTK_ERR_ARG, "dtk_op_gemv_role: position %d of %d rows", pos, T_max);
    if (!rope_cos || !rope_sin || !q_io || !k_io || !v_io) return fail(c, DTK_ERR_ARG, "dtk_op_gemv_role: QKV needs the rope tables and q / k / v buffers");
  } else if (epi == EPI_SWIGLU) {
    if (ff < 8 || (ff & 7) || N != 2 * ff || !y_io) return fail(c, DTK_ERR_ARG, "dtk_op_gemv_role: SWIGLU needs ff a multiple of 8 (as dtk_create), N = 2 ff and y");
  } else if (epi == EPI_LOGITS) {
    if (!logits_io) return fail(c, DTK_ERR_ARG, "dtk_op_gemv_role: LOGITS needs the logits buffer");
  } else if (!y_io) return fail(c, DTK_ERR_ARG, "dtk_op_gemv_role: RESID / STORE need y");
  HIPCHK(c, hipSetDevice(c->device));
  hipStream_t s = c->stream;
  const int KC4 = (K + 31) >> 5, hd2 = hd / 2;
  const size_t w_bytes = fmt == 2 ? (size_t)N * KC4 * 16 : (fmt == 1 ? (size_t)N * K : (size_t)N * K * 2);
  const size_t kv = epi == EPI_QKV ? (size_t)KVH * T_max * hd : 0, qn = epi == EPI_QKV ? (size_t)H * hd : 0, rope = epi == EPI_QKV ? (size_t)T_max * hd2 : 0;
  const size_t ny = epi == EPI_SWIGLU ? (size_t)ff : ((epi == EPI_STORE || epi == EPI_RESID) ? (size_t)N : 0), nl = epi == EPI_LOGITS ? (size_t)N : 0;
  const size_t hs = pro == PRO_ATTN ? (size_t)H * S : 0;
  size_t off = 0;
  OPBUF(uint8_t, dW, w_bytes); OPBUF(float, dws, fmt == 1 ? N : 0); OPBUF(uint8_t, dS4, fmt == 2 ? (size_t)N * KC4 : 0);
  OPBUF(bf16_t, dx, K); OPBUF(bf16_t, dn, K); OPBUF(bf16_t, dcos, rope); OPBUF(bf16_t, dsin, rope); OPBUF(DecState, dst, 1);
  OPBUF(float, dpm, hs); OPBUF(float, dpl, hs); OPBUF(float, dpo, hs * hd);
  constexpr size_t GUARD = 256;
  OPBUF(bf16_t, dq, qn + GUARD / 2); OPBUF(bf16_t, dk, kv + GUARD / 2); OPBUF(bf16_t, dv, kv + GUARD / 2); OPBUF(bf16_t, dy, ny + GUARD / 2);
  OPBUF(float, dl, nl + GUARD / 4);
  off = align_up(off, 256);
  if (off + 256 > c->scratch_bytes) return fail(c, DTK_ERR_ARG, "op scratch exhausted (%zu bytes)", off + 256);
  HIPCHK(c, hipMemsetAsync(c->scratch, scratch_fill, off + 256, s));
  HIPCHK(c, hipMemcpyAsync(dW, fmt == 2 ? (const void*)W4 : (fmt == 1 ? (const void*)W8 : (const void*)W), w_bytes, hipMemcpyHostToDevice, s));
  if (fmt == 1) HIPCHK(c, hipMemcpyAsync(dws, wscale, (size_t)N * 4, hipMemcpyHostToDevice, s));
  if (fmt == 2) HIPCHK(c, hipMemcpyAsync(dS4, S4, (size_t)N * KC4, hipMemcpyHostToDevice, s));
  if (pro != PRO_ATTN) HIPCHK(c, hipMemcpyAsync(dx, x, (size_t)K * 2, hipMemcpyHostToDevice, s));
  if (pro == PRO_RMSNORM) HIPCHK(c, hipMemcpyAsync(dn, norm_w, (size_t)K * 2, hipMemcpyHostToDevice, s));
  if (pro == PRO_ATTN) {
    HIPCHK(c, hipMemcpyAsync(dpm, pm, hs * 4, hipMemcpyHostToDevice, s));
    HIPCHK(c, hipMemcpyAsync(dpl, pl, hs * 4, hipMemcpyHostToDevice, s));
    HIPCHK(c, hipMemcpyAsync(dpo, po, hs * hd * 4, hipMemcpyHostToDevice, s));
  }
  DecState hst; memset(&hst, 0, sizeof hst);
  hst.pos = pos; hst.next_pos = pos + 1;
  HIPCHK(c, hipMemcpyAsync(dst, &hst, sizeof hst, hipMemcpyHostToDevice, s));
  if (epi == EPI_QKV) {
    HIPCHK(c, hipMemcpyAsync(dcos, rope_cos, rope * 2, hipMemcpyHostToDevice, s));
    HIPCHK(c, hipMemcpyAsync(dsin, rope_sin, rope * 2, hipMemcpyHostToDevice, s));
    HIPCHK(c, hipMemcpyAsync(dq, q_io, qn * 2, hipMemcpyHostToDevice, s));
    HIPCHK(c, hipMemcpyAsync(dk, k_io, kv * 2, hipMemcpyHostToDevice, s));
    HIPCHK(c, hipMemcpyAsync(dv, v_io, kv * 2, hipMemcpyHostToDevice, s));
  } else if (epi == EPI_LOGITS) HIPCHK(c, hipMemcpyAsync(dl, logits_io, nl * 4, hipMemcpyHostToDevice, s));
  else HIPCHK(c, hipMemcpyAsync(dy, y_io, ny * 2, hipMemcpyHostToDevice, s));
  HIPCHK(c, hipStreamSynchronize(s));
  GemvArgs g{};
  if (fmt == 0) g.W = reinterpret_cast<const bf16_t*>(dW);
  else if (fmt == 1) { g.W8 = dW; g.wscale = dws; }
  else { g.W4 = dW; g.S4 = dS4; }
  g.N = N; g.K = K; g.x = dx; g.norm_w = dn; g.eps = eps; g.pm = dpm; g.pl = dpl; g.po = dpo; g.S = S;
  g.y = dy; g.logits = dl; g.q_out = dq; g.kcache = dk; g.vcache = dv; g.rope_cos = dcos; g.rope_sin = dsin; g.st = dst;
  g.T_max = T_max; g.d = d; g.ff = ff; g.H = H; g.KVH = KVH; g.hd = hd;
  if (variant < 0) launch_gemv(pro, epi, g, s);
  else if (fmt == 1) launch_gemv_f8_variant(pro, epi, variant, g, s);
  else launch_gemv_variant(pro, epi, variant, g, s);
  HIPCHK(c, hipGetLastError());
  HIPCHK(c, hipStreamSynchronize(s));
  HIPCHK(c, hipGetLastError());
  {
    const unsigned char* ends[5] = {(unsigned char*)(dq + qn), (unsigned char*)(dk + kv), (unsigned char*)(dv + kv), (unsigned char*)(dy + ny), (unsigned char*)(dl + nl)};
    unsigned char guard[5][GUARD];
    for (int i = 0; i < 5; ++i) HIPCHK(c, hipMemcpy(guard[i], ends[i], GUARD, hipMemcpyDeviceToHost));
    for (int i = 0; i < 5; ++i)
      for (size_t j = 0; j < GUARD; ++j)
        if (guard[i][j] != (unsigned char)scratch_fill) return fail(c, DTK_ERR_STATE, "dtk_op_gemv_role: byte %zu behind the end of %s was written", j, i == 0 ? "q" : (i == 1 ? "k" : (i == 2 ? "v" : (i == 3 ? "y" : "logits"))));
  }
  if (epi == EPI_QKV) {
    HIPCHK(c, hipMemcpy(q_io, dq, qn * 2, hipMemcpyDeviceToHost));
    HIPCHK(c, hipMemcpy(k_io, dk, kv * 2, hipMemcpyDeviceToHost));
    HIPCHK(c, hipMemcpy(v_io, dv, kv * 2, hipMemcpyDeviceToHost));
  } else if (epi == EPI_LOGITS) HIPCHK(c, hipMemcpy(logits_io, dl, nl * 4, hipMemcpyDeviceToHost));
  else HIPCHK(c, hipMemcpy(y_io, dy, ny * 2, hipMemcpyDeviceToHost));
  return DTK_OK;
}

static inline size_t host_xtile_off(int slot, int k, int nsteps) {
  return ((size_t)((slot >> 4) * nsteps + (k >> 5)) * 64 + ((k & 31) >> 3) * 16 + (slot & 15)) * 8 + (k & 7);
}
static inline int op_nt_of(int nslots) { const int hi = nslots - 1; return hi < 16 ? 1 : (hi < 32 ? 2 : 4); }
static int op_tiled_weights(dtk_ctx* c, size_t& off, const uint16_t* W, const uint8_t* W8, const float* wscale, int N, int K, GemvBArgs& g) {
  hipStream_t s = c->stream;
  if (W8) {
    OPBUF(uint8_t, dW, (size_t)N * K); OPBUF(uint8_t, dT, tiled_bytes_f8(N, K)); OPBUF(float, dS, N);
    HIPCHK(c, hipMemcpyAsync(dW, W8, (size_t)N * K, hipMemcpyHostToDevice, s));
    HIPCHK(c, hipMemcpyAsync(dS, wscale, (size_t)N * 4, hipMemcpyHostToDevice, s));
    launch_retile_f8(dW, dT, N, K, s);
    g.W8 = dT; g.wscale = dS;
  } else {
    OPBUF(bf16_t, dW, (size_t)N * K); OPBUF(bf16_t, dT, tiled_elems(N, K));
    HIPCHK(c, hipMemcpyAsync(dW, W, (size_t)N * K * 2, hipMemcpyHostToDevice, s));
    launch_retile(dW, dT, N, K, s);
    g.W = dT;
  }
  g.N = N; g.K = K;
  return DTK_OK;
}
static int op_batch_state(dtk_ctx* c, size_t& off, const int32_t* active, const int32_t* pos, int nslots, GemvBArgs& g) {
  OPBUF(BatchState, dbs, 1); OPBUF(DecState, dst, DTK_MAX_BATCH);
  BatchState hbs; memset(&hbs, 0, sizeof hbs);
  DecState hst[DTK_MAX_BATCH]; memset(hst, 0, sizeof hst);
  for (int j = 0; j < DTK_MAX_BATCH; ++j) hbs.share_src[j] = -1;
  for (int j = 0; j < nslots; ++j) {
    hbs.active[j] = active[j] ? 1 : 0;
    if (pos) { hst[j].pos = pos[j]; hst[j].next_pos = pos[j] + 1; }
  }
  HIPCHK(c, hipMemcpyAsync(dbs, &hbs, sizeof hbs, hipMemcpyHostToDevice, c->stream));
  HIPCHK(c, hipMemcpyAsync(dst, hst, sizeof hst, hipMemcpyHostToDevice, c->stream));
  HIPCHK(c, hipStreamSynchronize(c->stream));
  g.bs = dbs; g.st = dst; g.nt = op_nt_of(nslots);
  return DTK_OK;
}
static int op_x_fragments(dtk_ctx* c, size_t& off, const uint16_t* X, int nslots, int K, bf16_t** out) {
  const int nsteps = (K + 31) >> 5;
  const size_t elems = (size_t)4 * nsteps * 512;
  OPBUF(bf16_t, dXf, elems);
  std::vector<bf16_t> h(elems, (bf16_t)0);
  for (int j = 0; j < nslots; ++j)
    for (int k = 0; k < K; ++k) h[host_xtile_off(j, k, nsteps)] = X[(size_t)j * K + k];
  HIPCHK(c, hipMemcpy(dXf, h.data(), elems * 2, hipMemcpyHostToDevice));
  *out = dXf;
  return DTK_OK;
}

int dtk_op_gemv_b(dtk_ctx* c, int epi, const uint16_t* W, const uint8_t* W8, const float* wscale, int N, int K,
                  const uint16_t* X, const uint16_t* norm_w, float eps, const int32_t* active, const int32_t* pos, int nslots,
                  int d, int ff, int H, int KVH, int T_max, const uint16_t* rope_cos, const uint16_t* rope_sin,
                  uint16_t* q_io, uint16_t* k_io, uint16_t* v_io, uint16_t* y_io, uint16_t* frag_io, float* logits_io,
// ... 241 lines not shown
```

### detikzify_amd/csrc/gemv_inl.h

```cpp
#pragma once
#include "common.h"

template <int NR, int U>
__device__ __forceinline__ void gemv_load(u32x4 (&w)[NR][U], const u32x4* (&rows)[NR],
                                          int g, int lane, int K8) {
  if (64 * (g * U + U) <= K8) {
#pragma unroll
    for (int u = 0; u < U; ++u) {
      const int c = lane + 64 * (g * U + u);
#pragma unroll
      for (int r = 0; r < NR; ++r) w[r][u] = ld_nt(rows[r] + c);
    }
    return;
  }
#pragma unroll
  for (int u = 0; u < U; ++u) {
    const int c = lane + 64 * (g * U + u);
    const bool ok = c < K8;
#pragma unroll
    for (int r = 0; r < NR; ++r) {
      u32x4 z = {0u, 0u, 0u, 0u};
      w[r][u] = ok ? ld_nt(rows[r] + c) : z;
    }
  }
}

template <int NR, int U>
__device__ __forceinline__ void gemv_fma(float (&acc)[NR], const u32x4 (&w)[NR][U],
                                         const u32x4* xs, int g, int lane, int K8) {
  const bool full = 64 * (g * U + U) <= K8;
#pragma unroll
  for (int u = 0; u < U; ++u) {
    const int c = lane + 64 * (g * U + u);
    u32x4 xv = {0u, 0u, 0u, 0u};
    if (full || c < K8) xv = xs[c];
#pragma unroll
    for (int r = 0; r < NR; ++r) acc[r] = dot8(w[r][u], xv, acc[r]);
  }
}

__device__ __forceinline__ float dot16_f8(const u32x4& w, const u32x4& x0, const u32x4& x1, float c) {
#pragma unroll
  for (int j = 0; j < 4; ++j) {
    const bf16x2_t lo = __builtin_amdgcn_cvt_scalef32_pk_bf16_fp8(w[j], 1.0f, false);
    const bf16x2_t hi = __builtin_amdgcn_cvt_scalef32_pk_bf16_fp8(w[j], 1.0f, true);
    const uint32_t xa = (j < 2) ? x0[2 * j] : x1[2 * j - 4];
    const uint32_t xb = (j < 2) ? x0[2 * j + 1] : x1[2 * j - 3];
    c = __builtin_amdgcn_fdot2_f32_bf16(lo, __builtin_bit_cast(bf16x2_t, xa), c, false);
    c = __builtin_amdgcn_fdot2_f32_bf16(hi, __builtin_bit_cast(bf16x2_t, xb), c, false);
  }
  return c;
}

template <int NR, int U>
// ... 3 lines not shown
  for (int u = 0; u < U; ++u) {
    const int c = lane + 64 * (g * U + u);
    u32x4 x0 = {0u, 0u, 0u, 0u}, x1 = {0u, 0u, 0u, 0u};
    if (64 * (g * U + U) <= KC || c < KC) { x0 = xs[2 * c]; x1 = xs[2 * c + 1]; }
#pragma unroll
    for (int r = 0; r < NR; ++r) acc[r] = dot16_f8(w[r][u], x0, x1, acc[r]);
  }
}

__device__ __forceinline__ int f4_xswz(int q) { return (q & ~63) | ((q & 3) << 4) | (((q >> 2) & 15) ^ ((q & 3) << 1)); }
__device__ __forceinline__ int f4_xrows(int KC) { return (4 * KC + 63) & ~63; }
__device__ __forceinline__ float f4_scale(unsigned e8m0) { return __uint_as_float(e8m0 << 23); }

__device__ __forceinline__ float dot32_f4(const u32x4& w, float sc, const u32x4& x0, const u32x4& x1, const u32x4& x2, const u32x4& x3, float c) {
#define F4_WORD(J, X)                                                                                                           \
  { const uint32_t xa = X[0], xb = X[1], xc = X[2], xd = X[3];                                                                  \
    c = __builtin_amdgcn_fdot2_f32_bf16(__builtin_amdgcn_cvt_scalef32_pk_bf16_fp4(w[J], sc, 0), __builtin_bit_cast(bf16x2_t, xa), c, false); \
    c = __builtin_amdgcn_fdot2_f32_bf16(__builtin_amdgcn_cvt_scalef32_pk_bf16_fp4(w[J], sc, 1), __builtin_bit_cast(bf16x2_t, xb), c, false); \
    c = __builtin_amdgcn_fdot2_f32_bf16(__builtin_amdgcn_cvt_scalef32_pk_bf16_fp4(w[J], sc, 2), __builtin_bit_cast(bf16x2_t, xc), c, false); \
    c = __builtin_amdgcn_fdot2_f32_bf16(__builtin_amdgcn_cvt_scalef32_pk_bf16_fp4(w[J], sc, 3), __builtin_bit_cast(bf16x2_t, xd), c, false); }
  F4_WORD(0, x0) F4_WORD(1, x1) F4_WORD(2, x2) F4_WORD(3, x3)
#undef F4_WORD
  return c;
}

template <int NR, int U>
__device__ __forceinline__ void gemv_load_f4(u32x4 (&w)[NR][U], unsigned (&sc)[NR][U], const u32x4* (&rows)[NR], const uint8_t* (&srows)[NR],
                                             int g, int lane, int KC) {
  gemv_load<NR, U>(w, rows, g, lane, KC);
  const bool full = 64 * (g * U + U) <= KC;
#pragma unroll
  for (int u = 0; u < U; ++u) {
    const int c = lane + 64 * (g * U + u);
#pragma unroll
    for (int r = 0; r < NR; ++r) sc[r][u] = (full || c < KC) ? (unsigned)srows[r][c] : 127u;
  }
}

template <int NR, int U>
__device__ __forceinline__ void gemv_fma_f4(float (&acc)[NR], const u32x4 (&w)[NR][U], const unsigned (&sc)[NR][U],
                                            const u32x4* xs, int g, int lane, int KC) {
#pragma unroll
  for (int u = 0; u < U; ++u) {
    const int c = lane + 64 * (g * U + u);
    u32x4 x0 = {0u, 0u, 0u, 0u}, x1 = x0, x2 = x0, x3 = x0;
    if (64 * (g * U + U) <= KC || c < KC) {
      const int b = ((c >> 4) << 6) | (c & 15);
      x0 = xs[b]; x1 = xs[(b + 16) ^ 2]; x2 = xs[(b + 32) ^ 4]; x3 = xs[(b + 48) ^ 6];
    }
#pragma unroll
    for (int r = 0; r < NR; ++r) acc[r] = dot32_f4(w[r][u], f4_scale(sc[r][u]), x0, x1, x2, x3, acc[r]);
  }
}
```

### detikzify_amd/csrc/kernels.h

```cpp
#pragma once
#include "common.h"
#include <stdlib.h>
#include <string.h>

enum { PRO_COPY = 0, PRO_RMSNORM = 1, PRO_ATTN = 2 };
enum { EPI_STORE = 0, EPI_RESID = 1, EPI_QKV = 2, EPI_SWIGLU = 3, EPI_LOGITS = 4 };

struct GemvArgs {
  const bf16_t* W;
  const uint8_t* W8;
  const float* wscale;
  int N;
  int K;
  const bf16_t* x;
  const bf16_t* norm_w;
  float eps;
  const float* pm;
  const float* pl;
  const float* po;
  int S;
  bf16_t* y;
  float* logits;
  bf16_t* q_out;
  bf16_t* kcache;
  bf16_t* vcache;
  const bf16_t* rope_cos;
  const bf16_t* rope_sin;
  const DecState* st;
  int T_max;
  int d;
  int ff;
  int H;
  int KVH;
  int hd = 128;
  const uint8_t* W4 = nullptr;
  const uint8_t* S4 = nullptr;
};

void launch_gemv(int pro, int epi, const GemvArgs& a, hipStream_t s);
void launch_gemv_q4(int pro, int epi, const GemvArgs& a, hipStream_t s);
void launch_gemv_variant(int pro, int epi, int variant, const GemvArgs& a, hipStream_t s);
void launch_gemv_f8(int pro, int epi, const GemvArgs& a, hipStream_t s);
void launch_gemv_f8_variant(int pro, int epi, int variant, const GemvArgs& a, hipStream_t s);
void set_gemv_default_variant(int epi, int variant);

struct AttnDecArgs {
  const bf16_t* q;
  const bf16_t* kcache;
  const bf16_t* vcache;
  const DecState* st;
  float* pm; float* pl; float* po;
  int H; int S; int T_max; float scale;
  int combine;
  bf16_t* out;
  unsigned* counters;
  int G;
  int threads;
  int hd = 128;
};
void launch_attn_decode(const AttnDecArgs& a, hipStream_t s);

struct SampleArgs {
  const float* logits; int V;
  const SamplingDev* sp;
  DecState* st;
  const bf16_t* embed;
  bf16_t* x;
  int d;
  int64_t* tok_ring;
  int ring;
  float* probs_out;
  int advance;
  int step_override;
  const BatchState* bs;
  int logits_stride;
  int nslots;
  SampleMB* mb;
  float2* lp_ring = nullptr;
  int trunc = 0;
  float* lse_ring = nullptr;
  const PenDev* pen = nullptr;
  const uint16_t* pen_cnt = nullptr;
  int pen_stride = 0;
  int32_t* pen_tok = nullptr;
};
void launch_count_token(const SampleArgs& a, hipStream_t s);
void launch_count_scatter(const int32_t* ids, int n, uint16_t* cnt, int V, hipStream_t s);
void launch_sample_b(const SampleArgs& a, hipStream_t s);
void launch_sample(const SampleArgs& a, hipStream_t s);
void launch_sample_mb(const SampleArgs& a, hipStream_t s);
struct TopArgs {
  const float* logits; int V; int logits_stride;
  const DecState* st; const BatchState* bs; int nslots;
  int ring; int k;
// ... 212 lines not shown
```

### detikzify_amd/csrc/kernels_decode.hip

```cpp
#include <cstdlib>
#include <cstring>
#include "kernels.h"
#include "gemv_inl.h"

template <int EPI, bool F8, int HD = 128>
__device__ __forceinline__ void gemv_epilogue(const GemvArgs& a, int u, float a0, float a1, float pre0, float pre1, int pos) {
    constexpr int HD2 = HD / 2, HSH = HD == 128 ? 6 : 5;
    static_assert(HD == 128 || HD == 64, "head dim 128 or 64");
    if (F8) {
      if (EPI == EPI_QKV) {
        const int r0 = (u >> HSH) * HD + (u & (HD2 - 1));
        a0 *= a.wscale[r0];
        a1 *= a.wscale[r0 + HD2];
      } else if (EPI == EPI_SWIGLU) {
        a0 *= a.wscale[u];
        a1 *= a.wscale[a.ff + u];
      } else {
        a0 *= a.wscale[u];
      }
    }
    if (EPI == EPI_STORE) {
      a.y[u] = f2bf(a0);
    } else if (EPI == EPI_RESID) {
      a.y[u] = f2bf(pre0 + rbf(a0));
    } else if (EPI == EPI_LOGITS) {
      a.logits[u] = rbf(a0);
    } else if (EPI == EPI_SWIGLU) {
      const float gte = rbf(a0);
      const float up = rbf(a1);
      const float sl = rbf(gte / (1.f + expf(-gte)));
      a.y[u] = f2bf(sl * up);
    } else if (EPI == EPI_QKV) {
      const int hb = u >> HSH, i = u & (HD2 - 1);
      const int sec = hb < a.H ? 0 : (hb < a.H + a.KVH ? 1 : 2);
      const int head = sec == 0 ? hb : (sec == 1 ? hb - a.H : hb - a.H - a.KVH);
      const float x1 = rbf(a0);
      const float x2 = rbf(a1);
      if (sec == 2) {
        bf16_t* dst = a.vcache + ((size_t)head * a.T_max + pos) * HD;
        dst[i] = f2bf(x1);
        dst[i + HD2] = f2bf(x2);
      } else {
        const float c = pre0, s = pre1;
        const float o1 = rbf(rbf(x1 * c) + rbf(-x2 * s));
        const float o2 = rbf(rbf(x2 * c) + rbf(x1 * s));
        bf16_t* dst = (sec == 0) ? (a.q_out + head * HD)
                                 : (a.kcache + ((size_t)head * a.T_max + pos) * HD);
        dst[i] = f2bf(o1);
        dst[i + HD2] = f2bf(o2);
      }
    }
}

template <int PRO, int EPI, int R, int U, int WAVES, bool PERSIST, bool F8 = false, int KS = 1, int HD = 128, bool F4 = false>
__global__ __launch_bounds__(WAVES * 64) void k_gemv(GemvArgs a) {
  static_assert(!(F4 && F8), "one weight format");
  constexpr bool PAIRED = (EPI == EPI_QKV) || (EPI == EPI_SWIGLU);
  constexpr int NR = PAIRED ? 2 * R : R;
  constexpr int THREADS = WAVES * 64;
  constexpr int RW = WAVES / KS;
  constexpr int HD2 = HD / 2, HC = HD / 8;
  constexpr int HSH = HD == 128 ? 6 : 5, CSH = HSH - 2;
  static_assert(HD == 128 || HD == 64, "head dim 128 or 64");
  static_assert(WAVES % KS == 0 && (KS == 1 || !PERSIST), "split-K variants are not persistent");
  extern __shared__ __attribute__((aligned(16))) unsigned char smem[];
  u32x4* xs = reinterpret_cast<u32x4*>(smem);
  const int K8 = a.K >> 3;
  const int KC = F4 ? ((a.K + 31) >> 5) : (F8 ? (a.K >> 4) : K8);
  const size_t row_bytes = F4 ? (size_t)KC * 16 : (F8 ? (size_t)a.K : (size_t)a.K * 2);
  const unsigned char* Wb = reinterpret_cast<const unsigned char*>(F4 ? (const void*)a.W4 : (F8 ? (const void*)a.W8 : (const void*)a.W));
  float* red = reinterpret_cast<float*>(smem + (size_t)(F4 ? f4_xrows(KC) : K8) * 16);
#define XI(c) (F4 ? f4_xswz(c) : (c))

  const int tid = threadIdx.x;
  const int lane = tid & 63;
  const int wave = tid >> 6;
  const int rw = KS > 1 ? wave / KS : wave;
  const int ks = KS > 1 ? wave % KS : 0;

  int n_units;
  if (EPI == EPI_QKV) n_units = (a.N >> 1);
  else if (EPI == EPI_SWIGLU) n_units = a.ff;
  else n_units = a.N;
  const int chunk_stride = PERSIST ? (int)gridDim.x * WAVES : 0;
  int chunk = PERSIST ? (int)blockIdx.x + (int)gridDim.x * wave : (int)blockIdx.x * RW + rw;
  int unit0 = chunk * R;

  const u32x4* rows[NR];
  const uint8_t* srows[NR];
  auto set_rows = [&](int u0) {
#pragma unroll
    for (int j = 0; j < R; ++j) {
      int u = u0 + j;
      if (u >= n_units) u = n_units - 1;
      int r0, r1 = 0;
      if (EPI == EPI_QKV) {
        r0 = (u >> HSH) * HD + (u & (HD2 - 1));
        r1 = r0 + HD2;
      } else if (EPI == EPI_SWIGLU) {
        r0 = u;
        r1 = a.ff + u;
      } else {
        r0 = u;
      }
      if (PAIRED) {
        rows[2 * j] = reinterpret_cast<const u32x4*>(Wb + (size_t)r0 * row_bytes);
        rows[2 * j + 1] = reinterpret_cast<const u32x4*>(Wb + (size_t)r1 * row_bytes);
      } else {
        rows[j] = reinterpret_cast<const u32x4*>(Wb + (size_t)r0 * row_bytes);
      }
      if (F4) {
        if (PAIRED) { srows[2 * j] = a.S4 + (size_t)r0 * KC; srows[2 * j + 1] = a.S4 + (size_t)r1 * KC; }
        else srows[j] = a.S4 + (size_t)r0 * KC;
      }
    }
  };
  set_rows(unit0);

  const int iters = (KC + 63) >> 6;
  const int Gall = (iters + U - 1) / U;
  const int G = KS > 1 ? (Gall - ks + KS - 1) / KS : Gall;
#define GIDX(g) (KS > 1 ? ks + KS * (g) : (g))
  u32x4 wa[NR][U], wb[NR][U];
  unsigned sa[NR][U], sb[NR][U];
  float acc[NR];
#define GLOAD(w, sc, g) do { if (F4) gemv_load_f4<NR, U>(w, sc, rows, srows, (g), lane, KC); else gemv_load<NR, U>(w, rows, (g), lane, KC); } while (0)
#define GFMA(w, sc, g) do { if (F4) gemv_fma_f4<NR, U>(acc, w, sc, xs, (g), lane, KC); else if (F8) gemv_fma_f8<NR, U>(acc, w, xs, (g), lane, KC); else gemv_fma<NR, U>(acc, w, xs, (g), lane, KC); } while (0)

  if (G > 0) GLOAD(wa, sa, GIDX(0));

  float pre0[R], pre1[R];
  int pos = 0;
  if (EPI == EPI_QKV) pos = a.st->pos;
  auto prefetch_epilogue = [&](int u0) {
#pragma unroll
    for (int j = 0; j < R; ++j) {
      pre0[j] = 0.f; pre1[j] = 0.f;
      if (lane == 0 && ks == 0) {
        int u = u0 + j;
        if (u >= n_units) u = n_units - 1;
        if (EPI == EPI_RESID) pre0[j] = bf2f(a.y[u]);
        if (EPI == EPI_QKV) {
          pre0[j] = bf2f(a.rope_cos[(size_t)pos * HD2 + (u & (HD2 - 1))]);
          pre1[j] = bf2f(a.rope_sin[(size_t)pos * HD2 + (u & (HD2 - 1))]);
        }
      }
    }
  };
  if (EPI == EPI_RESID || EPI == EPI_QKV) prefetch_epilogue(unit0);

  if (PRO == PRO_COPY) {
    const u32x4* x4 = reinterpret_cast<const u32x4*>(a.x);
    for (int c = tid; c < K8; c += THREADS) xs[XI(c)] = x4[c];
  } else if (PRO == PRO_RMSNORM) {
    const u32x4* x4 = reinterpret_cast<const u32x4*>(a.x);
    const u32x4* w4 = reinterpret_cast<const u32x4*>(a.norm_w);
    if (K8 <= 2 * THREADS) {
      const int c0 = tid, c1 = tid + THREADS;
      const bool h0 = c0 < K8, h1 = c1 < K8;
      const u32x4 zz = {0u, 0u, 0u, 0u};
      const u32x4 v0 = h0 ? x4[c0] : zz, v1 = h1 ? x4[c1] : zz;
      const u32x4 g0 = h0 ? w4[c0] : zz, g1 = h1 ? w4[c1] : zz;
      float ss = 0.f;
#pragma unroll
      for (int e = 0; e < 4; ++e) {
        const float lo = pk_lo(v0[e]), hi = pk_hi(v0[e]);
        ss += lo * lo;
        ss += hi * hi;
      }
#pragma unroll
      for (int e = 0; e < 4; ++e) {
        const float lo = pk_lo(v1[e]), hi = pk_hi(v1[e]);
        ss += lo * lo;
        ss += hi * hi;
      }
      ss = wave_sum(ss);
      if (lane == 0) red[wave] = ss;
      __syncthreads();
      float tot = 0.f;
#pragma unroll
// ... 133 lines not shown
#pragma unroll
        for (int r = 0; r < NR; ++r) {
          float t = part[(rw * NR + r) * KS];
#pragma unroll
          for (int k = 1; k < KS; ++k) t += part[(rw * NR + r) * KS + k];
          acc[r] = t;
        }
      }
    }

    if (active && lane == 0 && ks == 0) {
#pragma unroll
      for (int j = 0; j < R; ++j) {
        const int u = cur + j;
        if (u >= n_units) break;
        gemv_epilogue<EPI, F8, HD>(a, u, PAIRED ? acc[2 * j] : acc[j], PAIRED ? acc[2 * j + 1] : 0.f, q0[j], q1[j], pos);
      }
    }
    if (!PERSIST || unit0 >= n_units) break;
  }
#undef GIDX
#undef GLOAD
#undef GFMA
#undef XI
}

static int num_cus() {
  static int n = 0;
  if (!n) {
    int dev = 0;
    hipDeviceProp_t p;
    if (hipGetDevice(&dev) == hipSuccess && hipGetDeviceProperties(&p, dev) == hipSuccess) n = p.multiProcessorCount;
    if (n <= 0) n = 256;
  }
  return n;
}

template <int PRO, int EPI, int R, int U, int WAVES, bool PERSIST, int KS = 1>
static void launch_gemv_t(const GemvArgs& a, hipStream_t s, int blocks_per_cu) {
  int n_units = (EPI == EPI_QKV) ? (a.N >> 1) : (EPI == EPI_SWIGLU ? a.ff : a.N);
  const int per_block = (WAVES / KS) * R;
  int grid = (n_units + per_block - 1) / per_block;
  if (PERSIST) {
    const int cap = num_cus() * (blocks_per_cu > 0 ? blocks_per_cu : 2);
    if (grid > cap) grid = cap;
  }
  const size_t lds = (size_t)(a.K >> 3) * 16 + 64 + 1024;
  if constexpr (EPI == EPI_QKV || PRO == PRO_ATTN) {
    if (a.hd == 64) { hipLaunchKernelGGL((k_gemv<PRO, EPI, R, U, WAVES, PERSIST, false, KS, 64>), dim3(grid), dim3(WAVES * 64), lds, s, a); return; }
  }
  hipLaunchKernelGGL((k_gemv<PRO, EPI, R, U, WAVES, PERSIST, false, KS>), dim3(grid), dim3(WAVES * 64), lds, s, a);
}

#define GV(PRO, EPI, R, U, W, P, BPC) return launch_gemv_t<PRO, EPI, R, U, W, P>(a, s, BPC)
#define GVK(PRO, EPI, R, U, W, KS) return launch_gemv_t<PRO, EPI, R, U, W, false, KS>(a, s, 0)
void launch_gemv_variant(int pro, int epi, int variant, const GemvArgs& a, hipStream_t s) {
  if (pro == PRO_RMSNORM && epi == EPI_QKV) {
    switch (variant) {
      default: GV(PRO_RMSNORM, EPI_QKV, 1, 2, 4, false, 0);
      case 8: GV(PRO_RMSNORM, EPI_QKV, 2, 2, 4, false, 0);
      case 9: GV(PRO_RMSNORM, EPI_QKV, 1, 1, 4, false, 0);
      case 10: GV(PRO_RMSNORM, EPI_QKV, 1, 2, 8, false, 0);
      case 11: GV(PRO_RMSNORM, EPI_QKV, 1, 2, 2, false, 0);
      case 1: GV(PRO_RMSNORM, EPI_QKV, 1, 4, 4, false, 0);
      case 2: GV(PRO_RMSNORM, EPI_QKV, 2, 2, 8, false, 0);
      case 3: GV(PRO_RMSNORM, EPI_QKV, 2, 2, 4, true, 4);
      case 4: GV(PRO_RMSNORM, EPI_QKV, 2, 2, 8, true, 2);
      case 5: GV(PRO_RMSNORM, EPI_QKV, 1, 4, 8, true, 2);
      case 6: GV(PRO_RMSNORM, EPI_QKV, 4, 1, 4, false, 0);
      case 7: GV(PRO_RMSNORM, EPI_QKV, 1, 2, 4, false, 0);
    }
  }
  if (pro == PRO_RMSNORM && epi == EPI_SWIGLU) {
    switch (variant) {
      default: GV(PRO_RMSNORM, EPI_SWIGLU, 1, 2, 4, false, 0);
      case 8: GV(PRO_RMSNORM, EPI_SWIGLU, 2, 2, 4, false, 0);
      case 9: GV(PRO_RMSNORM, EPI_SWIGLU, 1, 1, 4, false, 0);
      case 10: GV(PRO_RMSNORM, EPI_SWIGLU, 1, 2, 8, false, 0);
      case 11: GV(PRO_RMSNORM, EPI_SWIGLU, 1, 2, 2, false, 0);
      case 1: GV(PRO_RMSNORM, EPI_SWIGLU, 1, 4, 4, false, 0);
      case 2: GV(PRO_RMSNORM, EPI_SWIGLU, 2, 2, 8, false, 0);
      case 3: GV(PRO_RMSNORM, EPI_SWIGLU, 2, 2, 4, true, 4);
      case 4: GV(PRO_RMSNORM, EPI_SWIGLU, 2, 2, 8, true, 2);
      case 5: GV(PRO_RMSNORM, EPI_SWIGLU, 1, 4, 8, true, 2);
      case 6: GV(PRO_RMSNORM, EPI_SWIGLU, 4, 1, 4, false, 0);
      case 7: GV(PRO_RMSNORM, EPI_SWIGLU, 1, 2, 4, false, 0);
    }
  }
  if (pro == PRO_COPY && epi == EPI_RESID) {
    switch (variant) {
      default: GV(PRO_COPY, EPI_RESID, 1, 8, 4, false, 0);
      case 8: GV(PRO_COPY, EPI_RESID, 2, 4, 4, false, 0);
      case 9: GV(PRO_COPY, EPI_RESID, 1, 2, 4, false, 0);
      case 10: GV(PRO_COPY, EPI_RESID, 1, 8, 8, false, 0);
      case 11: GV(PRO_COPY, EPI_RESID, 1, 8, 2, false, 0);
      case 12: GV(PRO_COPY, EPI_RESID, 1, 4, 2, false, 0);
      case 1: GV(PRO_COPY, EPI_RESID, 1, 4, 4, false, 0);
      case 2: GV(PRO_COPY, EPI_RESID, 4, 2, 4, false, 0);
      case 3: GV(PRO_COPY, EPI_RESID, 2, 4, 8, false, 0);
      case 4: GV(PRO_COPY, EPI_RESID, 2, 4, 4, true, 4);
      case 5: GV(PRO_COPY, EPI_RESID, 2, 4, 8, true, 2);
      case 6: GV(PRO_COPY, EPI_RESID, 1, 8, 4, false, 0);
      case 7: GV(PRO_COPY, EPI_RESID, 2, 2, 4, false, 0);
      case 13: GVK(PRO_COPY, EPI_RESID, 1, 4, 8, 2);
      case 14: GVK(PRO_COPY, EPI_RESID, 2, 4, 8, 2);
      case 15: GVK(PRO_COPY, EPI_RESID, 1, 6, 8, 2);
      case 16: GVK(PRO_COPY, EPI_RESID, 2, 6, 8, 2);
      case 17: GVK(PRO_COPY, EPI_RESID, 1, 6, 16, 4);
      case 18: GVK(PRO_COPY, EPI_RESID, 1, 2, 16, 4);
      case 19: GVK(PRO_COPY, EPI_RESID, 1, 3, 8, 2);
      case 20: GVK(PRO_COPY, EPI_RESID, 1, 4, 4, 2);
      case 21: GVK(PRO_COPY, EPI_RESID, 1, 6, 4, 2);
      case 22: GVK(PRO_COPY, EPI_RESID, 4, 2, 8, 2);
    }
  }
  if (pro == PRO_ATTN && epi == EPI_RESID) {
    switch (variant) {
      default: GV(PRO_ATTN, EPI_RESID, 2, 4, 8, false, 0);
      case 1: GV(PRO_ATTN, EPI_RESID, 2, 4, 4, false, 0);
      case 2: GV(PRO_ATTN, EPI_RESID, 1, 8, 8, false, 0);
      case 3: GV(PRO_ATTN, EPI_RESID, 4, 2, 8, false, 0);
      case 4: GV(PRO_ATTN, EPI_RESID, 4, 2, 4, false, 0);
      case 5: GVK(PRO_ATTN, EPI_RESID, 2, 4, 8, 2);
      case 6: GVK(PRO_ATTN, EPI_RESID, 4, 4, 8, 2);
      case 7: GV(PRO_ATTN, EPI_RESID, 2, 4, 16, false, 0);
      case 8: GVK(PRO_ATTN, EPI_RESID, 2, 4, 16, 2);
    }
  }
  if (pro == PRO_RMSNORM && epi == EPI_LOGITS) {
    switch (variant) {
      default: GV(PRO_RMSNORM, EPI_LOGITS, 2, 4, 4, false, 0);
      case 1: GV(PRO_RMSNORM, EPI_LOGITS, 4, 2, 8, true, 2);
      case 2: GV(PRO_RMSNORM, EPI_LOGITS, 4, 2, 4, false, 0);
      case 3: GV(PRO_RMSNORM, EPI_LOGITS, 1, 4, 4, false, 0);
      case 4: GV(PRO_RMSNORM, EPI_LOGITS, 1, 8, 4, false, 0);
    }
  }
  if (pro == PRO_RMSNORM && epi == EPI_STORE) {
    if (variant == 20) GV(PRO_RMSNORM, EPI_STORE, 1, 2, 4, false, 0);
    GV(PRO_RMSNORM, EPI_STORE, 4, 2, 4, false, 0);
  }
  if (variant == 20) GV(PRO_COPY, EPI_STORE, 1, 2, 4, false, 0);
  if (variant == 21) GV(PRO_COPY, EPI_STORE, 1, 8, 4, false, 0);
  GV(PRO_COPY, EPI_STORE, 4, 2, 4, false, 0);
}
#undef GV
#undef GVK

template <int PRO, int EPI, int R, int U, int WAVES, bool PERSIST = false, int BPC = 4>
static void launch_gemv_f8_t(const GemvArgs& a, hipStream_t s) {
  int n_units = (EPI == EPI_QKV) ? (a.N >> 1) : (EPI == EPI_SWIGLU ? a.ff : a.N);
  const int per_block = WAVES * R;
  int grid = (n_units + per_block - 1) / per_block;
  if (PERSIST && grid > num_cus() * BPC) grid = num_cus() * BPC;
  const size_t lds = (size_t)(a.K >> 3) * 16 + 64 + 1024;
  if constexpr (EPI == EPI_QKV || PRO == PRO_ATTN) {
    if (a.hd == 64) { hipLaunchKernelGGL((k_gemv<PRO, EPI, R, U, WAVES, PERSIST, true, 1, 64>), dim3(grid), dim3(WAVES * 64), lds, s, a); return; }
  }
  hipLaunchKernelGGL((k_gemv<PRO, EPI, R, U, WAVES, PERSIST, true>), dim3(grid), dim3(WAVES * 64), lds, s, a);
}
static int f8_variant() {
  static int v = -1;
  if (v < 0) { const char* e = getenv("DTK_F8_VARIANT"); v = e ? atoi(e) : 8; }
  return v;
}
#define F8(PRO, EPI, R, U, W) return launch_gemv_f8_t<PRO, EPI, R, U, W>(a, s)
#define F8P(PRO, EPI, R, U, W, BPC) return launch_gemv_f8_t<PRO, EPI, R, U, W, true, BPC>(a, s)
void launch_gemv_f8(int pro, int epi, const GemvArgs& a, hipStream_t s) { launch_gemv_f8_variant(pro, epi, f8_variant(), a, s); }
void launch_gemv_f8_variant(int pro, int epi, int v, const GemvArgs& a, hipStream_t s) {
  if (pro == PRO_RMSNORM && (epi == EPI_QKV || epi == EPI_SWIGLU)) {
    if (epi == EPI_QKV) {
      switch (v) { default: F8(PRO_RMSNORM, EPI_QKV, 2, 2, 4); case 0: F8(PRO_RMSNORM, EPI_QKV, 1, 2, 4);
                   case 2: F8(PRO_RMSNORM, EPI_QKV, 2, 4, 4); case 3: F8(PRO_RMSNORM, EPI_QKV, 4, 2, 4);
                   case 4: F8(PRO_RMSNORM, EPI_QKV, 2, 2, 8); case 5: F8(PRO_RMSNORM, EPI_QKV, 1, 4, 4);
                   case 6: F8P(PRO_RMSNORM, EPI_QKV, 1, 2, 4, 4); case 7: F8P(PRO_RMSNORM, EPI_QKV, 2, 2, 4, 4);
                   case 8: F8P(PRO_RMSNORM, EPI_QKV, 1, 2, 8, 2); case 9: F8P(PRO_RMSNORM, EPI_QKV, 1, 4, 4, 4); }
    }
    switch (v) { default: F8(PRO_RMSNORM, EPI_SWIGLU, 2, 2, 4); case 0: F8(PRO_RMSNORM, EPI_SWIGLU, 1, 2, 4);
                 case 2: F8(PRO_RMSNORM, EPI_SWIGLU, 2, 4, 4); case 3: F8(PRO_RMSNORM, EPI_SWIGLU, 4, 2, 4);
                 case 4: F8(PRO_RMSNORM, EPI_SWIGLU, 2, 2, 8); case 5: F8(PRO_RMSNORM, EPI_SWIGLU, 1, 4, 4);
                 case 6: F8P(PRO_RMSNORM, EPI_SWIGLU, 1, 2, 4, 4); case 7: F8P(PRO_RMSNORM, EPI_SWIGLU, 2, 2, 4, 4);
                 case 8: F8P(PRO_RMSNORM, EPI_SWIGLU, 1, 2, 8, 2); case 9: F8P(PRO_RMSNORM, EPI_SWIGLU, 1, 4, 4, 4); }
  }
  if (pro == PRO_RMSNORM && epi == EPI_LOGITS) {
    switch (v) { default: F8(PRO_RMSNORM, EPI_LOGITS, 4, 2, 4); case 0: F8(PRO_RMSNORM, EPI_LOGITS, 2, 2, 4);
                 case 2: F8(PRO_RMSNORM, EPI_LOGITS, 4, 4, 4); case 3: F8(PRO_RMSNORM, EPI_LOGITS, 8, 2, 4); }
  }
  if (pro == PRO_ATTN && epi == EPI_RESID) F8(PRO_ATTN, EPI_RESID, 2, 2, 4);
  switch (v) { default: F8(PRO_COPY, EPI_RESID, 2, 4, 4); case 0: F8(PRO_COPY, EPI_RESID, 1, 4, 4);
               case 2: F8(PRO_COPY, EPI_RESID, 2, 8, 4); case 3: F8(PRO_COPY, EPI_RESID, 4, 4, 4);
               case 4: F8(PRO_COPY, EPI_RESID, 2, 4, 8); case 5: F8(PRO_COPY, EPI_RESID, 1, 8, 4);
               case 6: F8P(PRO_COPY, EPI_RESID, 1, 4, 4, 4); case 7: F8P(PRO_COPY, EPI_RESID, 2, 4, 4, 4);
               case 8: F8P(PRO_COPY, EPI_RESID, 1, 4, 8, 2); case 9: F8P(PRO_COPY, EPI_RESID, 1, 8, 4, 4); }
}
#undef F8
#undef F8P

template <int PRO, int EPI, int R, int U, int WAVES, bool PERSIST = false, int BPC = 2>
static void launch_gemv_q4_t(const GemvArgs& a, hipStream_t s) {
  int n_units = (EPI == EPI_QKV) ? (a.N >> 1) : (EPI == EPI_SWIGLU ? a.ff : a.N);
  const int per_block = WAVES * R;
  int grid = (n_units + per_block - 1) / per_block;
  if (PERSIST && grid > num_cus() * BPC) grid = num_cus() * BPC;
  const int KC = (a.K + 31) >> 5;
  const size_t lds = (size_t)((4 * KC + 63) & ~63) * 16 + 64 + 1024;
  if constexpr (EPI == EPI_QKV || PRO == PRO_ATTN) {
    if (a.hd == 64) { hipLaunchKernelGGL((k_gemv<PRO, EPI, R, U, WAVES, PERSIST, false, 1, 64, true>), dim3(grid), dim3(WAVES * 64), lds, s, a); return; }
  }
  hipLaunchKernelGGL((k_gemv<PRO, EPI, R, U, WAVES, PERSIST, false, 1, 128, true>), dim3(grid), dim3(WAVES * 64), lds, s, a);
}
#define Q4(PRO, EPI, R, U, W) return launch_gemv_q4_t<PRO, EPI, R, U, W>(a, s)
#define Q4P(PRO, EPI, R, U, W, BPC) return launch_gemv_q4_t<PRO, EPI, R, U, W, true, BPC>(a, s)
void launch_gemv_q4(int pro, int epi, const GemvArgs& a, hipStream_t s) {
  if (pro == PRO_RMSNORM && epi == EPI_QKV) Q4P(PRO_RMSNORM, EPI_QKV, 1, 2, 8, 2);
  if (pro == PRO_RMSNORM && epi == EPI_SWIGLU) Q4P(PRO_RMSNORM, EPI_SWIGLU, 1, 2, 8, 2);
  if (pro == PRO_ATTN && epi == EPI_RESID) Q4(PRO_ATTN, EPI_RESID, 2, 2, 4);
  if (pro == PRO_COPY && epi == EPI_RESID) Q4(PRO_COPY, EPI_RESID, 2, 2, 4);
  if (pro == PRO_RMSNORM && epi == EPI_STORE) Q4(PRO_RMSNORM, EPI_STORE, 2, 2, 4);
  if (pro == PRO_COPY && epi == EPI_STORE) Q4(PRO_COPY, EPI_STORE, 2, 2, 4);
  fprintf(stderr, "launch_gemv_q4: no MXFP4 kernel for prologue %d, epilogue %d\n", pro, epi);
  abort();
}
#undef Q4
#undef Q4P

static int g_variant[8] = {0, 0, 0, 0, 0, -1, 0, 0};
void set_gemv_default_variant(int epi, int variant) { if (epi >= 0 && epi < 8) g_variant[epi] = variant; }

void launch_gemv(int pro, int epi, const GemvArgs& a, hipStream_t s) {
  if (a.W4) return launch_gemv_q4(pro, epi, a, s);
  if (a.W8) return launch_gemv_f8(pro, epi, a, s);
  if (pro == PRO_ATTN) {
    const int v = g_variant[6] ? g_variant[6] : (a.d > 2048 ? 8 : 1);
    return launch_gemv_variant(pro, epi, v, a, s);
  }
  int v = g_variant[epi & 7];
  const bool o_proj = epi == EPI_RESID && a.K == a.d;
  if (o_proj && g_variant[5] >= 0) v = g_variant[5];
  if (v == 0 && a.d > 0 && a.d <= 2048) {
    if (epi == EPI_SWIGLU) v = 5;
    else if (epi == EPI_RESID) v = o_proj ? 1 : 15;
    else if (epi == EPI_LOGITS) v = 3;
  } else if (v == 0 && a.d > 2048) {
    if (epi == EPI_RESID) v = 10;
    else if (epi == EPI_LOGITS) v = 3;
  }
  launch_gemv_variant(pro, epi, v, a, s);
}

__global__ __launch_bounds__(256) void k_attn_decode(AttnDecArgs a) {
  const int h = blockIdx.x, sp = blockIdx.y;
  const int tid = threadIdx.x, lane = tid & 63, wave = tid >> 6;
  const int sub = lane & 15;
  const int grp = lane >> 4;
  const int n = a.st->pos + 1;
  int chunk = (n + a.S - 1) / a.S;
  chunk = (chunk + 15) & ~15;
  const int j_begin = sp * chunk;
  const int j_end = min(n, j_begin + chunk);

  const u32x4 qv = reinterpret_cast<const u32x4*>(a.q + h * 128)[sub];
  const int kvh = h / a.G;
  const bf16_t* kbase = a.kcache + (size_t)kvh * a.T_max * 128;
  const bf16_t* vbase = a.vcache + (size_t)kvh * a.T_max * 128;

  float m = -1e30f, l = 0.f;
  float o[8];
#pragma unroll
  for (int e = 0; e < 8; ++e) o[e] = 0.f;

  for (int j0 = j_begin; j0 < j_end; j0 += 64) {
    u32x4 kv[4], vv[4];
    bool ok[4];
#pragma unroll
    for (int i = 0; i < 4; ++i) {
      const int j = j0 + i * 16 + wave * 4 + grp;
      ok[i] = j < j_end;
      const int jj = ok[i] ? j : j_begin;
      kv[i] = reinterpret_cast<const u32x4*>(kbase + (size_t)jj * 128)[sub];
      vv[i] = reinterpret_cast<const u32x4*>(vbase + (size_t)jj * 128)[sub];
    }
#pragma unroll
    for (int i = 0; i < 4; ++i) {
      float s = dot8(qv, kv[i], 0.f);
      s += __shfl_xor(s, 1, 64);
      s += __shfl_xor(s, 2, 64);
      s += __shfl_xor(s, 4, 64);
      s += __shfl_xor(s, 8, 64);
      s *= a.scale;
      if (ok[i]) {
        const float mn = fmaxf(m, s);
        const float corr = __expf(m - mn);
        const float p = __expf(s - mn);
        l = l * corr + p;
#pragma unroll
        for (int e = 0; e < 4; ++e) {
          o[2 * e] = o[2 * e] * corr + p * pk_lo(vv[i][e]);
          o[2 * e + 1] = o[2 * e + 1] * corr + p * pk_hi(vv[i][e]);
        }
        m = mn;
      }
// ... 1093 lines not shown
```

### include/dtk.h

```cpp
#ifndef DTK_H
#define DTK_H

#include <stdint.h>

#ifdef __cplusplus
extern "C" {
#endif

#define DTK_ABI_VERSION 7

typedef struct dtk_ctx dtk_ctx;

enum { DTK_F32 = 0, DTK_BF16 = 1, DTK_F16 = 2 };

enum {
  DTK_OK = 0,
  DTK_ERR_ARG = -1,
  DTK_ERR_HIP = -2,
  DTK_ERR_STATE = -3,
  DTK_ERR_RANGE = -4
};

typedef struct dtk_config {
  int32_t hidden;
// ... 7 lines not shown
  float   rope_theta;
  float   rope_factor;
  int32_t vit_dim;
  int32_t vit_depth;
  int32_t vit_heads;
  int32_t vit_mlp;
  int32_t vit_patch;
  int32_t vit_image;
  int32_t vit_feature_layer;
  float   vit_ln_eps;
  int32_t vit_gelu_tanh;
  int32_t concat_patches;
  int32_t image_token_id;
  int32_t attn_splits;
  int32_t reserved[7];
} dtk_config;
#define DTK_ARCH_PROJ_NO_BIAS 1

typedef struct dtk_sampling {
  int32_t do_sample;
  float   temperature;
  float   top_p;
  int32_t top_k;
  uint64_t seed;
  int32_t n_bad;
  int32_t bad_ids[8];
  int32_t n_begin_suppress;
  int32_t begin_suppress_ids[8];
  int32_t n_always_suppress;
  int32_t always_suppress_ids[8];
} dtk_sampling;

typedef struct dtk_sampling_ext {
  float   min_p;
  float   epsilon_cutoff;
  int32_t reserved[6];
} dtk_sampling_ext;

typedef struct dtk_stats {
  uint64_t weight_bytes_per_token;
  uint64_t kv_bytes_per_ctx_token;
  uint64_t decode_steps;
  uint64_t prefill_tokens;
  uint64_t vit_images;
  double   last_prefill_ms;
  double   last_vit_ms;
  double   probe_kernel_ms_sum;
  uint64_t probe_kernel_launches;
  uint64_t probe_kernel_bytes;
  double   probe_event_pair_ms;
  uint32_t last_batch_step_slots;
  uint32_t device_errors;
  uint32_t last_batch_step_fp8_mfma;
  uint32_t reserved0;
} dtk_stats;

int  dtk_abi_version(void);
int  dtk_abi_struct_size(int which);
const char* dtk_last_error(const dtk_ctx* ctx);

int  dtk_create(const dtk_config* cfg, int device, dtk_ctx** out);
void dtk_destroy(dtk_ctx* ctx);

int  dtk_load_tensor(dtk_ctx* ctx, const char* name, const void* host, int dtype,
                     const int64_t* shape, int ndim);
int  dtk_read_tensor(dtk_ctx* ctx, const char* name, void* host_out_bf16, int64_t n_elems);
int  dtk_fill_synthetic(dtk_ctx* ctx, uint64_t seed);
int  dtk_num_tensors(const dtk_ctx* ctx);
const char* dtk_tensor_name(const dtk_ctx* ctx, int i);
int64_t dtk_tensor_numel(const dtk_ctx* ctx, const char* name);

int  dtk_vit_encode(dtk_ctx* ctx, const float* pixels, int batch,
                    void* feats_out_bf16, void* pooled_out_bf16);

#define DTK_PREFILL_REUSE_PREFIX 1
#define DTK_PREFILL_REUSE_IMAGE  2
int  dtk_prefill(dtk_ctx* ctx, const int64_t* ids, int T, const float* pixels,
                 uint64_t image_key, int flags, float* logits_last_out);

int  dtk_score(dtk_ctx* ctx, const int64_t* ids, int T, const float* pixels, uint64_t image_key, uint32_t flags,
               int first, float* logprob_out, int32_t* argmax_out, float* lse_out);

int  dtk_score_packed(dtk_ctx* ctx, const int64_t* prefix_ids, int P, const float* pixels, uint64_t image_key, uint32_t flags,
                      const int64_t* cand_ids, const int32_t* cand_len, int N,
                      float* logprob_out, int32_t* argmax_out, float* lse_out);

int  dtk_set_sampling(dtk_ctx* ctx, const dtk_sampling* s);

#define DTK_MAX_INFLIGHT 4
#define DTK_VIT_BATCH 8
int  dtk_decode_launch(dtk_ctx* ctx);
int  dtk_decode_wait(dtk_ctx* ctx, int64_t* token_out);
int  dtk_decode(dtk_ctx* ctx, int64_t* token_out);
int  dtk_get_logits(dtk_ctx* ctx, float* logits_out);
int  dtk_context_len(const dtk_ctx* ctx);
int  dtk_set_graph_mode(dtk_ctx* ctx, int enabled);
int  dtk_synchronize(dtk_ctx* ctx);
int  dtk_get_stats(dtk_ctx* ctx, dtk_stats* out);

#define DTK_MAX_BATCH 64
#define DTK_MAX_SLOTS (DTK_MAX_BATCH + 8)
int  dtk_num_slots(const dtk_ctx* ctx);
int  dtk_max_decode_slots(const dtk_ctx* ctx);
int  dtk_prefill_slot(dtk_ctx* ctx, int slot, const int64_t* ids, int T, const float* pixels,
                      uint64_t image_key, int flags, float* logits_last_out);
int  dtk_set_sampling_slot(dtk_ctx* ctx, int slot, const dtk_sampling* s);
int  dtk_decode_batch_launch(dtk_ctx* ctx, const int32_t* active );
// ... 113 lines not shown
                                                                         uint64_t image_key, const int64_t* text_ids, int n_text,
                                                                         uint64_t text_key, int flags));

int  dtk_bench_gemv(dtk_ctx* ctx, int role, int variant, int reps, float* avg_us);
int  dtk_set_gemv_variant(dtk_ctx* ctx, int epi, int variant);
int  dtk_set_option(dtk_ctx* ctx, const char* name, int value);

#define DTK_EPI_NONE 0
#define DTK_EPI_BIAS 1
#define DTK_EPI_GELU 2
#define DTK_EPI_RESIDUAL 4
#define DTK_GEMM_NAIVE 256
#define DTK_GEMM_WT 512
#define DTK_GEMM_SL 1024
#define DTK_GEMM_KSLICES_SHIFT 12
int  dtk_op_gemm(dtk_ctx* ctx, const uint16_t* A, const uint16_t* W, const uint16_t* bias,
                 const uint16_t* residual, int M, int N, int K, int flags, uint16_t* C);
int  dtk_op_gemm_gated(dtk_ctx* ctx, const uint16_t* A, const uint16_t* W, const uint16_t* bias, const uint16_t* residual,
                       const uint16_t* gate, int M, int N, int K, int flags, uint16_t* C);
int  dtk_op_score(dtk_ctx* ctx, const uint16_t* Xn, const uint16_t* W, const int32_t* targets, int M, int N, int K, int flags,
                  float* logprob_out, float* lse_out, int32_t* argmax_out, float* zmax_out);
int  dtk_op_gemv(dtk_ctx* ctx, const uint16_t* W, const uint16_t* x, const uint16_t* norm_w,
                 int N, int K, int mode, float eps, uint16_t* y);
int  dtk_op_gemv_q4(dtk_ctx* ctx, const uint16_t* W, const uint16_t* x, const uint16_t* norm_w,
                    int N, int K, int mode, float eps, uint16_t* y, uint16_t* w_eff_out);
int  dtk_op_gemv_mv(dtk_ctx* ctx, const uint16_t* W, const uint16_t* X, const uint16_t* norm_w,
                    int N, int K, int mode, float eps, int nb, uint16_t* Y);
int  dtk_mx_layout(int G, int slot, int k, int64_t* data_off, int64_t* scale_off);
int  dtk_op_gemv_mx(dtk_ctx* ctx, const uint8_t* W8, const float* wscale, const uint16_t* X, int N, int K, int G, int nslots, int mode,
                    float* Y, uint8_t* x8_out, uint8_t* xs_out, uint8_t* y8_out, uint8_t* ys_out);
int  dtk_op_attention(dtk_ctx* ctx, const uint16_t* Q, const uint16_t* K, const uint16_t* V,
                      int H, int Tq, int Tk, int hd, int causal, int q_offset, uint16_t* O);
int  dtk_op_attention_seg(dtk_ctx* ctx, const uint16_t* Q, const uint16_t* K, const uint16_t* V,
                          int H, int Tq, int Tk, int hd, int shared_len, const int32_t* seg_begin, const int32_t* kv_row, uint16_t* O);
int  dtk_op_attn_decode(dtk_ctx* ctx, const uint16_t* q, const uint16_t* K, const uint16_t* V, int H, int KVH, int hd, int T_max,
                        const int32_t* pos, int npos, int threads, int splits, int mode, int variant, uint16_t* out,
                        float* pm_out, float* pl_out, float* po_out);
int  dtk_op_attn_decode_b(dtk_ctx* ctx, const uint16_t* q, const uint16_t* K, const uint16_t* V, int nslots, int H, int KVH, int T_max,
                          const int32_t* pos, const int32_t* active, const int32_t* share_src, const int32_t* share_len,
                          int use_prefix, int pfx_splits, int tail_threads, int gqa_fused, int attn_nt, uint16_t* out);
int  dtk_op_gemv_b(dtk_ctx* ctx, int epi, const uint16_t* W, const uint8_t* W8, const float* wscale, int N, int K,
                   const uint16_t* X, const uint16_t* norm_w, float eps, const int32_t* active, const int32_t* pos, int nslots,
                   int d, int ff, int H, int KVH, int T_max, const uint16_t* rope_cos, const uint16_t* rope_sin,
                   uint16_t* q_io, uint16_t* k_io, uint16_t* v_io, uint16_t* y_io, uint16_t* frag_io, float* logits_io,
                   uint16_t* xn_out, uint32_t* err_out);
int  dtk_op_gemv_bkp(dtk_ctx* ctx, const uint16_t* W, const uint8_t* W8, const float* wscale, int N, int K, const uint16_t* X,
                     const int32_t* active, int nslots, const uint16_t* norm_w, float eps, uint16_t* resid_io, uint16_t* xn_io,
                     float* part_out, uint32_t* err_out);
int  dtk_op_gemv_role(dtk_ctx* ctx, int pro, int epi, int variant, const uint16_t* W, const uint8_t* W8, const float* wscale,
                      const uint8_t* W4, const uint8_t* S4, int N, int K, int d, int ff, int H, int KVH, int hd, int T_max, int pos, float eps,
                      const uint16_t* x, const uint16_t* norm_w, const uint16_t* rope_cos, const uint16_t* rope_sin,
                      int S, const float* pm, const float* pl, const float* po, int scratch_fill,
                      uint16_t* q_io, uint16_t* k_io, uint16_t* v_io, uint16_t* y_io, float* logits_io);
int  dtk_op_layernorm(dtk_ctx* ctx, const uint16_t* X, const uint16_t* w, const uint16_t* b,
                      int M, int D, float eps, uint16_t* Y);
int  dtk_op_sample(dtk_ctx* ctx, const float* logits, int V, int step, int64_t* token_out,
                   float* filtered_probs_out);

int  dtk_decode_wait_lp(dtk_ctx* ctx, int64_t* token_out, float* lp_out );
int  dtk_decode_batch_wait_lp(dtk_ctx* ctx, int64_t* tokens_out , float* logprob_out ,
                              float* sample_logprob_out );
int  dtk_engine_read_lp(dtk_engine* e, int slot, int64_t* tokens_out, float* logprob_out, float* sample_logprob_out, int cap,
                        int32_t* n_out, int32_t* state_out, int timeout_ms);
int  dtk_engine_set_wait_lp_op(dtk_engine* e, int (*wait_lp)(void* dev, int64_t* tokens_out, float* logprob_out, float* sample_logprob_out));
int  dtk_op_sample_lp(dtk_ctx* ctx, const float* logits, int V, int step, int64_t* token_out, float* filtered_probs_out,
                      float* lp_out );

#define DTK_MAX_TOP 8
int  dtk_score_top(dtk_ctx* ctx, const int64_t* ids, int T, const float* pixels, uint64_t image_key, uint32_t flags, int first,
                   float* logprob_out, int32_t* argmax_out, float* lse_out, int k, int32_t* top_ids_out, float* top_logprob_out);
int  dtk_score_top_text(dtk_ctx* ctx, const int64_t* ids, int T, const float* pixels, uint64_t image_key, const int64_t* text_ids, int T_text,
                        uint64_t text_key, uint32_t flags, int first, float* logprob_out, int32_t* argmax_out, float* lse_out,
                        int k, int32_t* top_ids_out, float* top_logprob_out);
int  dtk_score_packed_top(dtk_ctx* ctx, const int64_t* prefix_ids, int P, const float* pixels, uint64_t image_key, uint32_t flags,
                          const int64_t* cand_ids, const int32_t* cand_len, int N, float* logprob_out, int32_t* argmax_out, float* lse_out,
                          int k, int32_t* top_ids_out, float* top_logprob_out);
int  dtk_score_packed_top_text(dtk_ctx* ctx, const int64_t* prefix_ids, int P, const float* pixels, uint64_t image_key, const int64_t* text_ids,
                               int T_text, uint64_t text_key, uint32_t flags, const int64_t* cand_ids, const int32_t* cand_len, int N,
                               float* logprob_out, int32_t* argmax_out, float* lse_out, int k, int32_t* top_ids_out, float* top_logprob_out);
int  dtk_op_score_top(dtk_ctx* ctx, const uint16_t* Xn, const uint16_t* W, const int32_t* targets, int M, int N, int K, int flags,
                      float* logprob_out, float* lse_out, int32_t* argmax_out, float* zmax_out, int k, int32_t* top_ids_out,
                      float* top_logprob_out, float* top_z_out);
int  dtk_decode_wait_top(dtk_ctx* ctx, int64_t* token_out, float* lp_out , int32_t* top_ids_out ,
                         float* top_logprob_out );
int  dtk_decode_batch_wait_top(dtk_ctx* ctx, int64_t* tokens_out , float* logprob_out ,
                               float* sample_logprob_out , int32_t* top_ids_out ,
                               float* top_logprob_out );

int  dtk_set_sampling_ext(dtk_ctx* ctx, const dtk_sampling_ext* x);
int  dtk_set_sampling_slot_ext(dtk_ctx* ctx, int slot, const dtk_sampling_ext* x);
int  dtk_op_sample_ext(dtk_ctx* ctx, const float* logits, int V, int step, int64_t* token_out, float* filtered_probs_out,
                       float* lp_out , const dtk_sampling_ext* x);
int  dtk_engine_submit_ext(dtk_engine* e, dtk_join* j, const dtk_sampling_ext* x, const int64_t* text_ids, int n_text, uint64_t text_key,
                           uint64_t* ticket_out);
int  dtk_engine_set_sampling_ext_op(dtk_engine* e, int (*set_sampling_slot_ext)(void* dev, int slot, const dtk_sampling_ext* x));

int  dtk_set_penalties(dtk_ctx* ctx, float presence, float frequency, int start);
int  dtk_set_penalties_slot(dtk_ctx* ctx, int slot, float presence, float frequency, int start);
int  dtk_op_sample_pen(dtk_ctx* ctx, const float* logits, int V, int step, int64_t* token_out, float* filtered_probs_out,
                       float* lp_out , const dtk_sampling_ext* x , float presence, float frequency,
                       const int64_t* counted_ids, int n_counted);
int  dtk_token_counts(dtk_ctx* ctx, int slot, uint16_t* out, int V);
int  dtk_engine_submit_pen(dtk_engine* e, dtk_join* j, const dtk_sampling_ext* x , float presence, float frequency, int start,
                           const int64_t* text_ids, int n_text, uint64_t text_key, uint64_t* ticket_out);
int  dtk_engine_set_penalties_op(dtk_engine* e, int (*set_penalties_slot)(void* dev, int slot, float presence, float frequency, int start));

// ... 5 lines not shown
```

Before: 380.8 tokens/s.

## Pack bf16 decode weights into lossless 13-bit planes with per-row exponent base

Adds a lossless 13-bit weight format for the bf16 decode path. Each row stores the low 8 bits of every weight, a 4-bit exponent offset from the row's maximum exponent, and a sign bit. Matrices are packed on the GPU at first decode, and decode GEMV launches route to new 13-bit kernel shapes whenever planes exist. The goal is to cut the weight bytes read per token in this memory-bound decode. A row with an exponent more than 15 below its row maximum cannot be packed, and that whole matrix then falls back to plain bf16; packing also costs extra memory and one-time setup.

```diff
diff --git a/detikzify_amd/_lib.py b/detikzify_amd/_lib.py
--- a/detikzify_amd/_lib.py
+++ b/detikzify_amd/_lib.py
@@ -66,7 +66,7 @@
         ("probe_kernel_ms_sum", C.c_double), ("probe_kernel_launches", C.c_uint64),
         ("probe_kernel_bytes", C.c_uint64), ("probe_event_pair_ms", C.c_double),
         ("last_batch_step_slots", C.c_uint32), ("device_errors", C.c_uint32),
-        ("last_batch_step_fp8_mfma", C.c_uint32), ("reserved0", C.c_uint32),
+        ("last_batch_step_fp8_mfma", C.c_uint32), ("w13_counts", C.c_uint32),
     ]
 
 
@@ -195,6 +195,10 @@
     "dtk_op_gemv_bkp": (C.c_int, [_P, _P, _P, _P, C.c_int, C.c_int, _P, _P, C.c_int, _P, C.c_float, _P, _P, _P, _P]),
     "dtk_op_gemv_role": (C.c_int, [_P, C.c_int, C.c_int, C.c_int, _P, _P, _P, _P, _P] + [C.c_int] * 9 + [C.c_float, _P, _P, _P, _P,
                                    C.c_int, _P, _P, _P, C.c_int, _P, _P, _P, _P, _P]),
+    "dtk_w13_row_bytes": (C.c_int, [C.c_int]),
+    "dtk_w13_pack_host": (C.c_int, [_P, C.c_int, C.c_int, _P, _P, _P]),
+    "dtk_w13_unpack_host": (C.c_int, [_P, _P, C.c_int, C.c_int, _P]),
+    "dtk_w13_op_bad_rows": (C.c_int, [_P]),
     "dtk_op_gemv": (C.c_int, [_P, _P, _P, _P, C.c_int, C.c_int, C.c_int, C.c_float, _P]),
     "dtk_op_gemv_mv": (C.c_int, [_P, _P, _P, _P, C.c_int, C.c_int, C.c_int, C.c_float, C.c_int, _P]),
     "dtk_op_gemv_q4": (C.c_int, [_P, _P, _P, _P, C.c_int, C.c_int, C.c_int, C.c_float, _P, _P]),
diff --git a/detikzify_amd/csrc/dtk_api.hip b/detikzify_amd/csrc/dtk_api.hip
--- a/detikzify_amd/csrc/dtk_api.hip
+++ b/detikzify_amd/csrc/dtk_api.hip
@@ -13,6 +13,10 @@
 
 #include "../../include/dtk.h"
 #include "kernels.h"
+#include "w13.h"
+#ifndef W13_DEFAULT
+#define W13_DEFAULT 1
+#endif
 #include "mx_quant.h"
 
 int& dtk_lds_attr_error(int device) {
@@ -59,6 +63,8 @@
   float *s_wqkv = nullptr, *s_wo = nullptr, *s_wgu = nullptr, *s_wdown = nullptr;
   uint8_t *f4_wqkv = nullptr, *f4_wo = nullptr, *f4_wgu = nullptr, *f4_wdown = nullptr;
   uint8_t *e4_wqkv = nullptr, *e4_wo = nullptr, *e4_wgu = nullptr, *e4_wdown = nullptr;
+  uint8_t *p13_wqkv = nullptr, *p13_wo = nullptr, *p13_wgu = nullptr, *p13_wdown = nullptr;
+  uint8_t *h13_wqkv = nullptr, *h13_wo = nullptr, *h13_wgu = nullptr, *h13_wdown = nullptr;
   uint8_t *t8_wqkv = nullptr, *t8_wo = nullptr, *t8_wgu = nullptr, *t8_wdown = nullptr;
   uint8_t *m_wqkv = nullptr, *m_wo = nullptr, *m_wgu = nullptr, *m_wdown = nullptr;
 };
@@ -159,6 +165,12 @@
   bool fp8_ready = false;
   uint8_t* q_lm_head = nullptr;
   float* s_lm_head = nullptr;
+  int w13 = W13_DEFAULT;
+  bool w13_ready = false;
+  uint8_t *p13_lm_head = nullptr, *h13_lm_head = nullptr;
+  unsigned* w13_bad = nullptr;
+  int w13_op_bad_rows = -1;
+  uint32_t w13_packed = 0, w13_unpacked = 0, w13_bad_rows = 0;
   uint64_t cached_image_key = 0;
   bool have_image = false;
   int KVH = 0;
@@ -758,6 +770,8 @@
   launch_top_logits(t, c->stream);
 }
 
+static inline bool w13_on(const dtk_ctx* c) { return c->wfmt == 0 && c->w13 != 0; }
+
 void decode_step_launches(dtk_ctx* c, bool with_probe, bool short_ctx = false) {
   hipStream_t s = c->stream;
   SampleArgs sa;
@@ -778,6 +792,8 @@
     g.pm = c->pm; g.pl = c->pl; g.po = c->po; g.S = c->S;
     g.W = w.wqkv; g.W8 = w.q_wqkv; g.wscale = w.s_wqkv; g.N = c->d + 2 * c->KVH * c->hd; g.K = c->d; g.x = c->x; g.norm_w = w.ln1;
     g.W4 = w.f4_wqkv; g.S4 = w.e4_wqkv;
+    const bool p13 = w13_on(c) && c->w13_ready;
+    g.Wp = p13 ? w.p13_wqkv : nullptr; g.Wh = w.h13_wqkv;
     g.q_out = c->q; g.kcache = kcache(c, l); g.vcache = vcache(c, l);
     launch_gemv(PRO_RMSNORM, EPI_QKV, g, s);
     AttnDecArgs ad;
@@ -790,20 +806,24 @@
     launch_attn_decode(ad, s);
     g.W = w.wo; g.W8 = w.q_wo; g.wscale = w.s_wo; g.N = c->d; g.K = c->d; g.y = c->x;
     g.W4 = w.f4_wo; g.S4 = w.e4_wo;
+    g.Wp = p13 ? w.p13_wo : nullptr; g.Wh = w.h13_wo;
     const bool partials = ad.combine == 0 && !(ad.threads && ad.S == 1);
     if (!partials) { g.x = c->attn_out; launch_gemv(PRO_COPY, EPI_RESID, g, s); }
     else launch_gemv(PRO_ATTN, EPI_RESID, g, s);
     g.W = w.wgu; g.W8 = w.q_wgu; g.wscale = w.s_wgu; g.N = 2 * c->ff; g.K = c->d; g.x = c->x; g.norm_w = w.ln2; g.y = c->act;
     g.W4 = w.f4_wgu; g.S4 = w.e4_wgu;
+    g.Wp = p13 ? w.p13_wgu : nullptr; g.Wh = w.h13_wgu;
     const bool probe_here = with_probe && (l == c->L / 2);
     if (probe_here) (void)hipEventRecord(c->probe_a, s);
     launch_gemv(PRO_RMSNORM, EPI_SWIGLU, g, s);
     if (probe_here) (void)hipEventRecord(c->probe_b, s);
     g.W = w.wdown; g.W8 = w.q_wdown; g.wscale = w.s_wdown; g.N = c->d; g.K = c->ff; g.x = c->act; g.y = c->x;
     g.W4 = w.f4_wdown; g.S4 = w.e4_wdown;
+    g.Wp = p13 ? w.p13_wdown : nullptr; g.Wh = w.h13_wdown;
     launch_gemv(PRO_COPY, EPI_RESID, g, s);
   }
   GemvArgs g{};
+  if (w13_on(c) && c->w13_ready) { g.Wp = c->p13_lm_head; g.Wh = c->h13_lm_head; }
   g.W = c->lm_head; g.W8 = c->q_lm_head; g.wscale = c->s_lm_head; g.N = c->V; g.K = c->d; g.x = c->x; g.norm_w = c->final_norm;
   g.eps = c->cfg.rms_eps; g.logits = c->logits;
   launch_gemv(PRO_RMSNORM, EPI_LOGITS, g, s);
@@ -994,6 +1014,93 @@
   c->ptiled_ready = false;
 }
 
+static void set_weight_bytes(dtk_ctx* c) {
+  const uint64_t kvd = (uint64_t)c->KVH * c->hd;
+  const uint64_t attn_lin = (uint64_t)2 * c->d * c->d + 2 * kvd * c->d;
+  const uint64_t per_layer = attn_lin + (uint64_t)3 * c->d * c->ff + 2 * (uint64_t)c->d;
+  c->stats.weight_bytes_per_token = 2 * (per_layer * c->L + (uint64_t)c->d + (uint64_t)c->V * c->d);
+  if (c->wfmt == 1) {
+    const uint64_t lin = attn_lin + (uint64_t)3 * c->d * c->ff;
+    const uint64_t rows = (uint64_t)3 * c->d + 2 * kvd + (uint64_t)2 * c->ff;
+    c->stats.weight_bytes_per_token = (lin + 4 * rows + 4 * (uint64_t)c->d) * c->L + 2 * (uint64_t)c->d + (uint64_t)c->V * c->d + 4 * (uint64_t)c->V;
+  }
+  if (c->wfmt == 2) {
+    const uint64_t bd = mxfp4_row_scales(c->d), bf = mxfp4_row_scales(c->ff);
+    const uint64_t blocks = ((uint64_t)2 * c->d + 2 * kvd + (uint64_t)2 * c->ff) * bd + (uint64_t)c->d * bf;
+    c->stats.weight_bytes_per_token = (17 * blocks + 4 * (uint64_t)c->d) * c->L + 2 * (uint64_t)c->d + (uint64_t)c->V * c->d + 4 * (uint64_t)c->V;
+  }
+  c->stats.probe_kernel_bytes = (uint64_t)2 * c->ff * c->d * (c->wfmt == 1 ? 1 : 2);
+  if (c->wfmt == 2) c->stats.probe_kernel_bytes = (uint64_t)2 * c->ff * 17 * mxfp4_row_scales(c->d);
+  if (w13_on(c) && c->w13_ready) {
+    auto mat = [](const uint8_t* planes, uint64_t N, int K) { return planes ? N * (w13_row_bytes(K) + 1) : 2 * N * (uint64_t)K; };
+    uint64_t W = 2 * ((uint64_t)2 * c->d * c->L + (uint64_t)c->d) + mat(c->p13_lm_head, (uint64_t)c->V, c->d);
+    for (int l = 0; l < c->L; ++l) {
+      const LayerW& w = c->layers[l];
+      W += mat(w.p13_wqkv, (uint64_t)c->d + 2 * kvd, c->d) + mat(w.p13_wo, (uint64_t)c->d, c->d) + mat(w.p13_wgu, (uint64_t)2 * c->ff, c->d) +
+           mat(w.p13_wdown, (uint64_t)c->d, c->ff);
+    }
+    c->stats.weight_bytes_per_token = W;
+    c->stats.probe_kernel_bytes = mat(c->layers[c->L / 2].p13_wgu, (uint64_t)2 * c->ff, c->d);
+  }
+}
+static void w13_set_stats(dtk_ctx* c) {
+  const uint32_t rows = c->w13_bad_rows > 4095u ? 4095u : c->w13_bad_rows;
+  c->stats.w13_counts = (c->w13_packed & 1023u) | ((c->w13_unpacked & 1023u) << 10) | (rows << 20);
+}
+static int w13_pack_one(dtk_ctx* c, int pro, int epi, const bf16_t* W, int N, int K, uint8_t** planes, uint8_t** hb) {
+  GemvArgs g{};
+  g.N = N; g.K = K; g.d = c->d; g.ff = c->ff; g.hd = c->hd;
+  if (!gemv_w13_takes(pro, epi, g)) {
+    if (*planes) { (void)hipFree(*planes); *planes = nullptr; }
+    if (*hb) { (void)hipFree(*hb); *hb = nullptr; }
+    return DTK_OK;
+  }
+  if (!*planes) HIPCHK(c, hipMalloc((void**)planes, (size_t)N * w13_row_bytes(K)));
+  if (!*hb) HIPCHK(c, hipMalloc((void**)hb, (size_t)N));
+  HIPCHK(c, hipMemsetAsync(c->w13_bad, 0, sizeof(unsigned), c->stream));
+  launch_pack_w13_rows(W, *planes, *hb, c->w13_bad, N, K, c->stream);
+  unsigned bad = 0;
+  HIPCHK(c, hipMemcpyAsync(&bad, c->w13_bad, sizeof(unsigned), hipMemcpyDeviceToHost, c->stream));
+  HIPCHK(c, hipStreamSynchronize(c->stream));
+  if (bad) {
+    (void)hipFree(*planes); *planes = nullptr;
+    (void)hipFree(*hb); *hb = nullptr;
+    c->w13_unpacked++; c->w13_bad_rows += bad;
+  } else c->w13_packed++;
+  return DTK_OK;
+}
+static void w13_free(dtk_ctx* c);
+int ensure_w13(dtk_ctx* c) {
+  if (!w13_on(c) || c->w13_ready) return DTK_OK;
+  if (!c->w13_bad) HIPCHK(c, hipMalloc((void**)&c->w13_bad, sizeof(unsigned)));
+  c->w13_packed = c->w13_unpacked = c->w13_bad_rows = 0;
+  const int qkvn = c->d + 2 * c->KVH * c->hd;
+  for (int l = 0; l < c->L; ++l) {
+    LayerW& w = c->layers[l];
+    int rc = w13_pack_one(c, PRO_RMSNORM, EPI_QKV, w.wqkv, qkvn, c->d, &w.p13_wqkv, &w.h13_wqkv);
+    if (!rc) rc = w13_pack_one(c, PRO_ATTN, EPI_RESID, w.wo, c->d, c->d, &w.p13_wo, &w.h13_wo);
+    if (!rc) rc = w13_pack_one(c, PRO_RMSNORM, EPI_SWIGLU, w.wgu, 2 * c->ff, c->d, &w.p13_wgu, &w.h13_wgu);
+    if (!rc) rc = w13_pack_one(c, PRO_COPY, EPI_RESID, w.wdown, c->d, c->ff, &w.p13_wdown, &w.h13_wdown);
+    if (rc) { w13_free(c); return rc; }
+  }
+  int rc = w13_pack_one(c, PRO_RMSNORM, EPI_LOGITS, c->lm_head, c->V, c->d, &c->p13_lm_head, &c->h13_lm_head);
+  if (rc) { w13_free(c); return rc; }
+  c->w13_ready = true;
+  w13_set_stats(c);
+  set_weight_bytes(c);
+  return DTK_OK;
+}
+static void w13_free(dtk_ctx* c) {
+  for (auto& w : c->layers) {
+    uint8_t** ps[8] = {&w.p13_wqkv, &w.h13_wqkv, &w.p13_wo, &w.h13_wo, &w.p13_wgu, &w.h13_wgu, &w.p13_wdown, &w.h13_wdown};
+    for (uint8_t** p : ps) if (*p) { (void)hipFree(*p); *p = nullptr; }
+  }
+  if (c->p13_lm_head) { (void)hipFree(c->p13_lm_head); c->p13_lm_head = nullptr; }
+  if (c->h13_lm_head) { (void)hipFree(c->h13_lm_head); c->h13_lm_head = nullptr; }
+  c->w13_ready = false;
+  c->w13_packed = c->w13_unpacked = c->w13_bad_rows = 0;
+}
+
 void ensure_tiled_weights(dtk_ctx* c);
 void ensure_prefill_tiles(dtk_ctx* c) {
   ensure_fp8_weights(c);
@@ -1332,23 +1439,8 @@
   CCHK(hipMemcpyAsync(c->rope_sin, sinv.data(), sinv.size() * 2, hipMemcpyHostToDevice, c->stream));
   CCHK(hipStreamSynchronize(c->stream));
 #undef CCHK
-  const uint64_t kvd = (uint64_t)c->KVH * c->hd;
-  const uint64_t attn_lin = (uint64_t)2 * c->d * c->d + 2 * kvd * c->d;
-  const uint64_t per_layer = attn_lin + (uint64_t)3 * c->d * c->ff + 2 * (uint64_t)c->d;
-  c->stats.weight_bytes_per_token = 2 * (per_layer * c->L + (uint64_t)c->d + (uint64_t)c->V * c->d);
-  if (c->wfmt == 1) {
-    const uint64_t lin = attn_lin + (uint64_t)3 * c->d * c->ff;
-    const uint64_t rows = (uint64_t)3 * c->d + 2 * kvd + (uint64_t)2 * c->ff;
-    c->stats.weight_bytes_per_token = (lin + 4 * rows + 4 * (uint64_t)c->d) * c->L + 2 * (uint64_t)c->d + (uint64_t)c->V * c->d + 4 * (uint64_t)c->V;
-  }
-  if (c->wfmt == 2) {
-    const uint64_t bd = mxfp4_row_scales(c->d), bf = mxfp4_row_scales(c->ff);
-    const uint64_t blocks = ((uint64_t)2 * c->d + 2 * kvd + (uint64_t)2 * c->ff) * bd + (uint64_t)c->d * bf;
-    c->stats.weight_bytes_per_token = (17 * blocks + 4 * (uint64_t)c->d) * c->L + 2 * (uint64_t)c->d + (uint64_t)c->V * c->d + 4 * (uint64_t)c->V;
-  }
-  c->stats.kv_bytes_per_ctx_token = (uint64_t)2 * c->L * kvd * 2;
-  c->stats.probe_kernel_bytes = (uint64_t)2 * c->ff * c->d * (c->wfmt == 1 ? 1 : 2);
-  if (c->wfmt == 2) c->stats.probe_kernel_bytes = (uint64_t)2 * c->ff * 17 * mxfp4_row_scales(c->d);
+  set_weight_bytes(c);
+  c->stats.kv_bytes_per_ctx_token = (uint64_t)2 * c->L * (uint64_t)c->KVH * c->hd * 2;
   *out = c;
   if (c->nb > 0) {
     const bool big = max_decode_slots(c) >= 64;
@@ -1376,6 +1468,8 @@
   (void)hipSetDevice(c->device);
   if (c->ad) (void)dtk_adapter_destroy(c);
   if (c->stream) (void)hipStreamSynchronize(c->stream);
+  w13_free(c);
+  if (c->w13_bad) (void)hipFree(c->w13_bad);
   if (c->graph_exec) (void)hipGraphExecDestroy(c->graph_exec);
   if (c->graph) (void)hipGraphDestroy(c->graph);
   if (c->graph_short_exec) (void)hipGraphExecDestroy(c->graph_short_exec);
@@ -1467,6 +1561,7 @@
   c->tiled_ready = false;
   c->ptiled_ready = false;
   c->fp8_ready = false;
+  if (c->w13_ready) { c->w13_ready = false; drop_graph(c); set_weight_bytes(c); }
   return DTK_OK;
 }
 
@@ -1508,6 +1603,7 @@
   c->tiled_ready = false;
   c->ptiled_ready = false;
   c->fp8_ready = false;
+  if (c->w13_ready) { c->w13_ready = false; drop_graph(c); set_weight_bytes(c); }
   return DTK_OK;
 }
 
@@ -2445,6 +2541,7 @@
   if (c->seq0.host_next_pos >= c->Tmax) return fail(c, DTK_ERR_RANGE, "context length %d reached max_positions", c->seq0.host_next_pos);
   HIPCHK(c, hipSetDevice(c->device));
   ensure_fp8_weights(c);
+  if (int rc = ensure_w13(c)) return rc;
   if (c->use_graph) {
     int rc = ensure_graph(c);
     if (rc) return rc;
@@ -2550,12 +2647,49 @@
   const bool same_layer = (variant & 0x100) != 0;
   const int plain = (variant >> 9) & 3;
   const bool fmt = (variant & 0x800) != 0;
+  const bool b13 = (variant & 0x1000) != 0, raw16 = (variant & 0x2000) != 0;
+  if (b13 && (fmt || raw16 || plain || same_layer || c->wfmt != 0 || !c->w13 || (variant & 0xff) == 0xff))
+    return fail(c, DTK_ERR_ARG, "dtk_bench_gemv: 0x1000 | shape (13-bit planes) needs a bf16 context with w13 = 1, a shape number and no other flag");
+  if (raw16 && ((variant & 0xff) != 0xff || plain || fmt)) return fail(c, DTK_ERR_ARG, "dtk_bench_gemv: 0x2000 (bf16 rows) goes with variant 0xff only");
+  const bool step13 = w13_on(c) && !raw16 && !plain && (variant & 0xff) == 0xff;
+  struct Tmp13 { std::vector<uint8_t*> p, h; ~Tmp13() { for (auto x : p) if (x) (void)hipFree(x); for (auto x : h) if (x) (void)hipFree(x); } } tmp13;
+  if (b13 || step13) { if (int rc = ensure_w13(c)) return rc; }
+  if (b13) {
+    for (int l = 0; l < c->L && role != 4; ++l) {
+      const LayerW& w = c->layers[l];
+      const uint8_t* p = role == 0 ? w.p13_wqkv : (role == 1 ? w.p13_wo : (role == 2 ? w.p13_wgu : w.p13_wdown));
+      if (p) continue;
+      if (role != 1) return fail(c, DTK_ERR_STATE, "dtk_bench_gemv: role %d has no 13-bit planes in layer %d (an unpackable row, or a bf16 fold no 13-bit shape has)", role, l);
+      if (!c->w13_bad) HIPCHK(c, hipMalloc((void**)&c->w13_bad, sizeof(unsigned)));
+      uint8_t *pp = nullptr, *hh = nullptr;
+      HIPCHK(c, hipMalloc((void**)&pp, (size_t)c->d * w13_row_bytes(c->d)));
+      tmp13.p.push_back(pp);
+      HIPCHK(c, hipMalloc((void**)&hh, (size_t)c->d));
+      tmp13.h.push_back(hh);
+      unsigned bad = 0;
+      HIPCHK(c, hipMemsetAsync(c->w13_bad, 0, sizeof(unsigned), s));
+      launch_pack_w13_rows(w.wo, pp, hh, c->w13_bad, c->d, c->d, s);
+      HIPCHK(c, hipMemcpyAsync(&bad, c->w13_bad, sizeof(unsigned), hipMemcpyDeviceToHost, s));
+      HIPCHK(c, hipStreamSynchronize(s));
+      if (bad) return fail(c, DTK_ERR_STATE, "dtk_bench_gemv: o_proj of layer %d has %u unpackable row(s)", l, bad);
+    }
+    if (role == 4 && !c->p13_lm_head) return fail(c, DTK_ERR_STATE, "dtk_bench_gemv: lm_head has no 13-bit planes");
+  }
   if (fmt && ((variant & 0xff) != 0xff || plain))
     return fail(c, DTK_ERR_ARG, "dtk_bench_gemv: 0x800 (the context's weight format) goes with variant 0xff only");
   if (fmt) ensure_fp8_weights(c);
   variant &= 0xff;
   const bool shipped = variant == 0xff;
-  auto launch = [&](int pro, int epi, const GemvArgs& g) { if (shipped) launch_gemv(pro, epi, g, s); else launch_gemv_variant(pro, epi, variant, g, s); };
+  if (b13) {
+    const int pro = (role == 1 || role == 3) ? PRO_COPY : PRO_RMSNORM;
+    const int epi = role == 0 ? EPI_QKV : (role == 2 ? EPI_SWIGLU : (role == 4 ? EPI_LOGITS : EPI_RESID));
+    if (!gemv_w13_has(pro, epi, variant)) return fail(c, DTK_ERR_ARG, "dtk_bench_gemv: no 13-bit shape %d for role %d", variant, role);
+  }
+  auto launch = [&](int pro, int epi, const GemvArgs& g) {
+    if (b13) launch_gemv_w13_variant(pro, epi, variant, g, s);
+    else if (shipped) launch_gemv(pro, epi, g, s);
+    else launch_gemv_variant(pro, epi, variant, g, s);
+  };
   auto one_pass = [&]() {
     for (int l = 0; l < c->L; ++l) {
       const LayerW& w = c->layers[same_layer ? 0 : l];
@@ -2579,6 +2713,13 @@
         else if (role == 3) { g.W8 = w.q_wdown; g.wscale = w.s_wdown; g.W4 = w.f4_wdown; g.S4 = w.e4_wdown; }
         else { g.W8 = c->q_lm_head; g.wscale = c->s_lm_head; }
       }
+      if (b13 || step13) {
+        if (role == 0) { g.Wp = w.p13_wqkv; g.Wh = w.h13_wqkv; }
+        else if (role == 1) { g.Wp = w.p13_wo; g.Wh = w.h13_wo; if (!g.Wp && b13) { g.Wp = tmp13.p[(size_t)l]; g.Wh = tmp13.h[(size_t)l]; } }
+        else if (role == 2) { g.Wp = w.p13_wgu; g.Wh = w.h13_wgu; }
+        else if (role == 3) { g.Wp = w.p13_wdown; g.Wh = w.h13_wdown; }
+        else { g.Wp = c->p13_lm_head; g.Wh = c->h13_lm_head; }
+      }
       if (role == 0) { g.W = w.wqkv; g.N = c->d + 2 * c->KVH * c->hd; g.K = c->d; g.x = c->x; g.norm_w = w.ln1; g.q_out = c->q; g.kcache = kcache(c, l); g.vcache = vcache(c, l); launch(PRO_RMSNORM, EPI_QKV, g); }
       else if (role == 1) { g.W = w.wo; g.N = c->d; g.K = c->d; g.x = c->attn_out; g.y = c->q; launch(PRO_COPY, EPI_RESID, g); }
       else if (role == 2) { g.W = w.wgu; g.N = 2 * c->ff; g.K = c->d; g.x = c->x; g.norm_w = w.ln2; g.y = c->act; launch(PRO_RMSNORM, EPI_SWIGLU, g); }
@@ -2604,6 +2745,15 @@
   HIPCHK(c, hipSetDevice(c->device));
   HIPCHK(c, hipStreamSynchronize(c->stream));
   if (!strcmp(name, "attn_full_max")) c->attn_full_max = value;
+  else if (!strcmp(name, "w13")) {
+    if (value != 0 && value != 1) return fail(c, DTK_ERR_ARG, "w13 must be 0 or 1");
+    if (value != c->w13) {
+      if (c->launched != c->waited) return fail(c, DTK_ERR_STATE, "w13: %d single-sequence decode step(s) are unread", (int)(c->launched - c->waited));
+      c->w13 = value; drop_graph(c);
+      if (!value) { w13_free(c); w13_set_stats(c); }
+      set_weight_bytes(c);
+    }
+  }
   else if (!strcmp(name, "logprobs")) {
     if (value != 0 && value != 1) return fail(c, DTK_ERR_ARG, "logprobs must be 0 or 1");
     if (value == 0 && c->top_logprobs) return fail(c, DTK_ERR_STATE, "logprobs: top_logprobs = %d needs it (set \"top_logprobs\" to 0 first)", c->top_logprobs);
@@ -3510,6 +3660,14 @@
   if ((W != nullptr) + (W8 != nullptr) + (W4 != nullptr) != 1 || (W8 && !wscale) || (!W8 && wscale) || (!W4 != !S4))
     return fail(c, DTK_ERR_ARG, "dtk_op_gemv_role: exactly one of W | W8 + wscale | W4 + S4");
   const int fmt = W4 ? 2 : (W8 ? 1 : 0);
+  const bool f13 = variant >= 0x1000;
+  const int v13 = variant - 0x1000;
+  if (f13) {
+    if (fmt != 0) return fail(c, DTK_ERR_ARG, "dtk_op_gemv_role: the 13-bit planes are packed from bf16 operands (W)");
+    if (v13 != 0xff && !gemv_w13_has(pro, epi, v13)) return fail(c, DTK_ERR_ARG, "dtk_op_gemv_role: no 13-bit kernel for prologue %d, epilogue %d, shape %d", pro, epi, v13);
+    if (v13 == 0xff && !gemv_w13_has(pro, epi, 0)) return fail(c, DTK_ERR_ARG, "dtk_op_gemv_role: no 13-bit kernel for prologue %d, epilogue %d", pro, epi);
+    variant = -1;
+  }
   if (N < 1 || K < 8 || (K & 7) || (fmt == 1 && (K & 15))) return fail(c, DTK_ERR_ARG, "dtk_op_gemv_role: N >= 1, K a multiple of 8 (16 for fp8 weights)");
   if (pro < PRO_COPY || pro > PRO_ATTN || epi < EPI_STORE || epi > EPI_LOGITS) return fail(c, DTK_ERR_ARG, "dtk_op_gemv_role: unknown prologue %d or epilogue %d", pro, epi);
   if (!gemv_role_variant_ok(fmt, pro, epi, variant))
@@ -3539,6 +3697,7 @@
   const size_t hs = pro == PRO_ATTN ? (size_t)H * S : 0;
   size_t off = 0;
   OPBUF(uint8_t, dW, w_bytes); OPBUF(float, dws, fmt == 1 ? N : 0); OPBUF(uint8_t, dS4, fmt == 2 ? (size_t)N * KC4 : 0);
+  OPBUF(uint8_t, dWp, f13 ? (size_t)N * w13_row_bytes(K) : 0); OPBUF(uint8_t, dWh, f13 ? (size_t)N : 0); OPBUF(unsigned, dbad, f13 ? 1 : 0);
   OPBUF(bf16_t, dx, K); OPBUF(bf16_t, dn, K); OPBUF(bf16_t, dcos, rope); OPBUF(bf16_t, dsin, rope); OPBUF(DecState, dst, 1);
   OPBUF(float, dpm, hs); OPBUF(float, dpl, hs); OPBUF(float, dpo, hs * hd);
   constexpr size_t GUARD = 256;
@@ -3576,7 +3735,18 @@
   g.N = N; g.K = K; g.x = dx; g.norm_w = dn; g.eps = eps; g.pm = dpm; g.pl = dpl; g.po = dpo; g.S = S;
   g.y = dy; g.logits = dl; g.q_out = dq; g.kcache = dk; g.vcache = dv; g.rope_cos = dcos; g.rope_sin = dsin; g.st = dst;
   g.T_max = T_max; g.d = d; g.ff = ff; g.H = H; g.KVH = KVH; g.hd = hd;
-  if (variant < 0) launch_gemv(pro, epi, g, s);
+  if (f13) {
+    unsigned bad = 0;
+    HIPCHK(c, hipMemsetAsync(dbad, 0, sizeof(unsigned), s));
+    launch_pack_w13_rows(g.W, dWp, dWh, dbad, N, K, s);
+    HIPCHK(c, hipMemcpyAsync(&bad, dbad, sizeof(unsigned), hipMemcpyDeviceToHost, s));
+    HIPCHK(c, hipStreamSynchronize(s));
+    HIPCHK(c, hipMemsetAsync(dbad, scratch_fill, sizeof(unsigned), s));
+    c->w13_op_bad_rows = (int)bad;
+    if (!bad) { g.Wp = dWp; g.Wh = dWh; }
+  }
+  if (f13 && g.Wp && v13 != 0xff) launch_gemv_w13_variant(pro, epi, v13, g, s);
+  else if (variant < 0) launch_gemv(pro, epi, g, s);
   else if (fmt == 1) launch_gemv_f8_variant(pro, epi, variant, g, s);
   else launch_gemv_variant(pro, epi, variant, g, s);
   HIPCHK(c, hipGetLastError());
@@ -3598,6 +3768,19 @@
   else HIPCHK(c, hipMemcpy(y_io, dy, ny * 2, hipMemcpyDeviceToHost));
   return DTK_OK;
 }
+
+int dtk_w13_row_bytes(int K) { return (K < 8 || (K & 7)) ? -1 : (int)w13_row_bytes(K); }
+int dtk_w13_pack_host(const uint16_t* W, int N, int K, uint8_t* planes, uint8_t* hb, int32_t* bad) {
+  if (!W || !planes || !hb || !bad || N < 1 || K < 8 || (K & 7)) return DTK_ERR_ARG;
+  for (int r = 0; r < N; ++r) bad[r] = w13_pack_row(W + (size_t)r * K, K, planes + (size_t)r * w13_row_bytes(K), hb + r);
+  return DTK_OK;
+}
+int dtk_w13_unpack_host(const uint8_t* planes, const uint8_t* hb, int N, int K, uint16_t* W) {
+  if (!W || !planes || !hb || N < 1 || K < 8 || (K & 7)) return DTK_ERR_ARG;
+  for (int r = 0; r < N; ++r) w13_unpack_row(planes + (size_t)r * w13_row_bytes(K), hb[r], K, W + (size_t)r * K);
+  return DTK_OK;
+}
+int dtk_w13_op_bad_rows(dtk_ctx* c) { return c ? c->w13_op_bad_rows : -1; }
 
 static inline size_t host_xtile_off(int slot, int k, int nsteps) {
   return ((size_t)((slot >> 4) * nsteps + (k >> 5)) * 64 + ((k & 31) >> 3) * 16 + (slot & 15)) * 8 + (k & 7);
diff --git a/detikzify_amd/csrc/gemv_inl.h b/detikzify_amd/csrc/gemv_inl.h
--- a/detikzify_amd/csrc/gemv_inl.h
+++ b/detikzify_amd/csrc/gemv_inl.h
@@ -1,5 +1,6 @@
 #pragma once
 #include "common.h"
+#include "w13.h"
 
 template <int NR, int U>
 __device__ __forceinline__ void gemv_load(u32x4 (&w)[NR][U], const u32x4* (&rows)[NR],
@@ -109,3 +110,79 @@
     for (int r = 0; r < NR; ++r) acc[r] = dot32_f4(w[r][u], f4_scale(sc[r][u]), x0, x1, x2, x3, acc[r]);
   }
 }
+
+typedef __attribute__((ext_vector_type(2))) unsigned short u16x2_t;
+
+__device__ __forceinline__ uint32_t w13_high4(uint32_t codes, uint32_t lo2) {
+  const uint32_t nz = ((codes + 0x0f0f0f0fu) >> 4) & 0x01010101u;
+  const u16x2_t r = __builtin_bit_cast(u16x2_t, nz) * __builtin_bit_cast(u16x2_t, lo2) + __builtin_bit_cast(u16x2_t, codes);
+  return __builtin_bit_cast(uint32_t, r);
+}
+
+__device__ __forceinline__ float dot8_w13(uint32_t la, uint32_t lb, uint32_t n, uint32_t s, int i, uint32_t lo2, const u32x4& x, float c) {
+  const uint32_t he = w13_high4(n & 0x0f0f0f0fu, lo2) | ((s << (7 - 2 * i)) & 0x80808080u);
+  const uint32_t ho = w13_high4((n >> 4) & 0x0f0f0f0fu, lo2) | ((s << (6 - 2 * i)) & 0x80808080u);
+  c = dot2(__builtin_amdgcn_perm(he, la, 0x05010400u), x[0], c);
+  c = dot2(__builtin_amdgcn_perm(he, la, 0x07030602u), x[1], c);
+  c = dot2(__builtin_amdgcn_perm(ho, lb, 0x05010400u), x[2], c);
+  c = dot2(__builtin_amdgcn_perm(ho, lb, 0x07030602u), x[3], c);
+  return c;
+}
+
+template <int NR, int U>
+__device__ __forceinline__ void gemv_load_w13(u32x4 (&wl)[NR][U / 2], u32x2 (&wn)[NR][U / 2], uint32_t (&ws)[NR][U / 4],
+                                              const u32x4* (&rows)[NR], int g, int lane, int J2, int n_off, int s_off) {
+  static_assert(U % 4 == 0, "a stage is whole sign blocks");
+  if (2 * (g * (U / 4) + U / 4) <= J2) {
+#pragma unroll
+    for (int ub = 0; ub < U / 4; ++ub) {
+      const int b = g * (U / 4) + ub;
+#pragma unroll
+      for (int r = 0; r < NR; ++r) {
+        const unsigned char* p = reinterpret_cast<const unsigned char*>(rows[r]);
+#pragma unroll
+        for (int h = 0; h < 2; ++h) {
+          wl[r][2 * ub + h] = ld_nt(rows[r] + ((2 * b + h) * 64 + lane));
+          wn[r][2 * ub + h] = __builtin_nontemporal_load(reinterpret_cast<const u32x2*>(p + n_off) + ((2 * b + h) * 64 + lane));
+        }
+        ws[r][ub] = __builtin_nontemporal_load(reinterpret_cast<const uint32_t*>(p + s_off) + (b * 64 + lane));
+      }
+    }
+    return;
+  }
+#pragma unroll
+  for (int ub = 0; ub < U / 4; ++ub) {
+    const int b = g * (U / 4) + ub;
+#pragma unroll
+    for (int r = 0; r < NR; ++r) {
+      const unsigned char* p = reinterpret_cast<const unsigned char*>(rows[r]);
+#pragma unroll
+      for (int h = 0; h < 2; ++h) {
+        const bool ok = 2 * b + h < J2;
+        const u32x4 zl = {0u, 0u, 0u, 0u};
+        const u32x2 zn = {0u, 0u};
+        wl[r][2 * ub + h] = ok ? ld_nt(rows[r] + ((2 * b + h) * 64 + lane)) : zl;
+        wn[r][2 * ub + h] = ok ? __builtin_nontemporal_load(reinterpret_cast<const u32x2*>(p + n_off) + ((2 * b + h) * 64 + lane)) : zn;
+      }
+      ws[r][ub] = (2 * b < J2) ? __builtin_nontemporal_load(reinterpret_cast<const uint32_t*>(p + s_off) + (b * 64 + lane)) : 0u;
+    }
+  }
+}
+
+template <int NR, int U>
+__device__ __forceinline__ void gemv_fma_w13(float (&acc)[NR], const u32x4 (&wl)[NR][U / 2], const u32x2 (&wn)[NR][U / 2],
+                                             const uint32_t (&ws)[NR][U / 4], const uint32_t (&lo2)[NR],
+                                             const u32x4* xs, int g, int lane, int K8) {
+  const bool full = 64 * (g * U + U) <= K8;
+#pragma unroll
+  for (int u = 0; u < U; ++u) {
+    const int c = lane + 64 * (g * U + u);
+    u32x4 xv = {0u, 0u, 0u, 0u};
+    if (full || c < K8) xv = xs[c];
+#pragma unroll
+    for (int r = 0; r < NR; ++r) {
+      const u32x4& l = wl[r][u >> 1];
+      acc[r] = dot8_w13((u & 1) ? l[2] : l[0], (u & 1) ? l[3] : l[1], wn[r][u >> 1][u & 1], ws[r][u >> 2], u & 3, lo2[r], xv, acc[r]);
+    }
+  }
+}
diff --git a/detikzify_amd/csrc/kernels.h b/detikzify_amd/csrc/kernels.h
--- a/detikzify_amd/csrc/kernels.h
+++ b/detikzify_amd/csrc/kernels.h
@@ -35,11 +35,17 @@
   int hd = 128;
   const uint8_t* W4 = nullptr;
   const uint8_t* S4 = nullptr;
+  const uint8_t* Wp = nullptr;
+  const uint8_t* Wh = nullptr;
 };
 
 void launch_gemv(int pro, int epi, const GemvArgs& a, hipStream_t s);
 void launch_gemv_q4(int pro, int epi, const GemvArgs& a, hipStream_t s);
 void launch_gemv_variant(int pro, int epi, int variant, const GemvArgs& a, hipStream_t s);
+void launch_gemv_w13_variant(int pro, int epi, int variant, const GemvArgs& a, hipStream_t s);
+bool gemv_w13_has(int pro, int epi, int variant);
+bool gemv_w13_takes(int pro, int epi, const GemvArgs& a);
+void launch_pack_w13_rows(const bf16_t* W, uint8_t* Wp, uint8_t* Wh, unsigned* bad_rows, int N, int K, hipStream_t s);
 void launch_gemv_f8(int pro, int epi, const GemvArgs& a, hipStream_t s);
 void launch_gemv_f8_variant(int pro, int epi, int variant, const GemvArgs& a, hipStream_t s);
 void set_gemv_default_variant(int epi, int variant);
diff --git a/detikzify_amd/csrc/kernels_decode.hip b/detikzify_amd/csrc/kernels_decode.hip
--- a/detikzify_amd/csrc/kernels_decode.hip
+++ b/detikzify_amd/csrc/kernels_decode.hip
@@ -52,9 +52,9 @@
     }
 }
 
-template <int PRO, int EPI, int R, int U, int WAVES, bool PERSIST, bool F8 = false, int KS = 1, int HD = 128, bool F4 = false>
+template <int PRO, int EPI, int R, int U, int WAVES, bool PERSIST, bool F8 = false, int KS = 1, int HD = 128, bool F4 = false, bool W13 = false>
 __global__ __launch_bounds__(WAVES * 64) void k_gemv(GemvArgs a) {
-  static_assert(!(F4 && F8), "one weight format");
+  static_assert(!(F4 && F8) && !(W13 && (F4 || F8)), "one weight format");
   constexpr bool PAIRED = (EPI == EPI_QKV) || (EPI == EPI_SWIGLU);
   constexpr int NR = PAIRED ? 2 * R : R;
   constexpr int THREADS = WAVES * 64;
@@ -67,8 +67,9 @@
   u32x4* xs = reinterpret_cast<u32x4*>(smem);
   const int K8 = a.K >> 3;
   const int KC = F4 ? ((a.K + 31) >> 5) : (F8 ? (a.K >> 4) : K8);
-  const size_t row_bytes = F4 ? (size_t)KC * 16 : (F8 ? (size_t)a.K : (size_t)a.K * 2);
-  const unsigned char* Wb = reinterpret_cast<const unsigned char*>(F4 ? (const void*)a.W4 : (F8 ? (const void*)a.W8 : (const void*)a.W));
+  const size_t row_bytes = W13 ? w13_row_bytes(a.K) : (F4 ? (size_t)KC * 16 : (F8 ? (size_t)a.K : (size_t)a.K * 2));
+  const unsigned char* Wb = reinterpret_cast<const unsigned char*>(W13 ? (const void*)a.Wp : (F4 ? (const void*)a.W4 : (F8 ? (const void*)a.W8 : (const void*)a.W)));
+  const int J2 = W13 ? w13_units(a.K) : 0, n13 = W13 ? (int)w13_n_off(a.K) : 0, s13 = W13 ? (int)w13_s_off(a.K) : 0;
   float* red = reinterpret_cast<float*>(smem + (size_t)(F4 ? f4_xrows(KC) : K8) * 16);
 #define XI(c) (F4 ? f4_xswz(c) : (c))
 
@@ -88,6 +89,7 @@
 
   const u32x4* rows[NR];
   const uint8_t* srows[NR];
+  uint32_t lo2[NR];
   auto set_rows = [&](int u0) {
 #pragma unroll
     for (int j = 0; j < R; ++j) {
@@ -113,6 +115,10 @@
         if (PAIRED) { srows[2 * j] = a.S4 + (size_t)r0 * KC; srows[2 * j + 1] = a.S4 + (size_t)r1 * KC; }
         else srows[j] = a.S4 + (size_t)r0 * KC;
       }
+      if (W13) {
+        if (PAIRED) { lo2[2 * j] = (uint32_t)w13_lo(a.Wh[r0]) * 0x10001u; lo2[2 * j + 1] = (uint32_t)w13_lo(a.Wh[r1]) * 0x10001u; }
+        else lo2[j] = (uint32_t)w13_lo(a.Wh[r0]) * 0x10001u;
+      }
     }
   };
   set_rows(unit0);
@@ -123,9 +129,13 @@
 #define GIDX(g) (KS > 1 ? ks + KS * (g) : (g))
   u32x4 wa[NR][U], wb[NR][U];
   unsigned sa[NR][U], sb[NR][U];
+  constexpr int UW = W13 ? U : 4;
+  u32x4 lwa[NR][UW / 2], lwb[NR][UW / 2];
+  u32x2 nwa[NR][UW / 2], nwb[NR][UW / 2];
+  uint32_t zwa[NR][UW / 4], zwb[NR][UW / 4];
   float acc[NR];
-#define GLOAD(w, sc, g) do { if (F4) gemv_load_f4<NR, U>(w, sc, rows, srows, (g), lane, KC); else gemv_load<NR, U>(w, rows, (g), lane, KC); } while (0)
-#define GFMA(w, sc, g) do { if (F4) gemv_fma_f4<NR, U>(acc, w, sc, xs, (g), lane, KC); else if (F8) gemv_fma_f8<NR, U>(acc, w, xs, (g), lane, KC); else gemv_fma<NR, U>(acc, w, xs, (g), lane, KC); } while (0)
+#define GLOAD(w, sc, g) do { if (W13) gemv_load_w13<NR, UW>(l##w, n##w, z##w, rows, (g), lane, J2, n13, s13); else if (F4) gemv_load_f4<NR, U>(w, sc, rows, srows, (g), lane, KC); else gemv_load<NR, U>(w, rows, (g), lane, KC); } while (0)
+#define GFMA(w, sc, g) do { if (W13) gemv_fma_w13<NR, UW>(acc, l##w, n##w, z##w, lo2, xs, (g), lane, K8); else if (F4) gemv_fma_f4<NR, U>(acc, w, sc, xs, (g), lane, KC); else if (F8) gemv_fma_f8<NR, U>(acc, w, xs, (g), lane, KC); else gemv_fma<NR, U>(acc, w, xs, (g), lane, KC); } while (0)
 
   if (G > 0) GLOAD(wa, sa, GIDX(0));
 
@@ -365,9 +375,10 @@
   hipLaunchKernelGGL((k_gemv<PRO, EPI, R, U, WAVES, PERSIST, false, KS>), dim3(grid), dim3(WAVES * 64), lds, s, a);
 }
 
-#define GV(PRO, EPI, R, U, W, P, BPC) return launch_gemv_t<PRO, EPI, R, U, W, P>(a, s, BPC)
-#define GVK(PRO, EPI, R, U, W, KS) return launch_gemv_t<PRO, EPI, R, U, W, false, KS>(a, s, 0)
-void launch_gemv_variant(int pro, int epi, int variant, const GemvArgs& a, hipStream_t s) {
+struct GemvShape { int R, U, waves, ks; bool persist; };
+#define GV(PRO, EPI, R, U, W, P, BPC) do { if (q) { *q = GemvShape{R, U, W, 1, P}; return; } return launch_gemv_t<PRO, EPI, R, U, W, P>(a, s, BPC); } while (0)
+#define GVK(PRO, EPI, R, U, W, KS) do { if (q) { *q = GemvShape{R, U, W, KS, false}; return; } return launch_gemv_t<PRO, EPI, R, U, W, false, KS>(a, s, 0); } while (0)
+static void gemv_variant_row(int pro, int epi, int variant, const GemvArgs& a, hipStream_t s, GemvShape* q) {
   if (pro == PRO_RMSNORM && epi == EPI_QKV) {
     switch (variant) {
       default: GV(PRO_RMSNORM, EPI_QKV, 1, 2, 4, false, 0);
@@ -459,6 +470,12 @@
 }
 #undef GV
 #undef GVK
+void launch_gemv_variant(int pro, int epi, int variant, const GemvArgs& a, hipStream_t s) { gemv_variant_row(pro, epi, variant, a, s, nullptr); }
+static GemvShape gemv_variant_shape(int pro, int epi, int variant) {
+  GemvShape q{};
+  gemv_variant_row(pro, epi, variant, GemvArgs{}, nullptr, &q);
+  return q;
+}
 
 template <int PRO, int EPI, int R, int U, int WAVES, bool PERSIST = false, int BPC = 4>
 static void launch_gemv_f8_t(const GemvArgs& a, hipStream_t s) {
@@ -537,16 +554,142 @@
 #undef Q4
 #undef Q4P
 
+template <int PRO, int EPI, int R, int U, int WAVES, bool PERSIST = false, int KS = 1, int BPC = 2>
+static void launch_gemv_w13_t(const GemvArgs& a, hipStream_t s) {
+  int n_units = (EPI == EPI_QKV) ? (a.N >> 1) : (EPI == EPI_SWIGLU ? a.ff : a.N);
+  const int per_block = (WAVES / KS) * R;
+  int grid = (n_units + per_block - 1) / per_block;
+  if (PERSIST && grid > num_cus() * BPC) grid = num_cus() * BPC;
+  const size_t lds = (size_t)(a.K >> 3) * 16 + 64 + 1024;
+  if constexpr (EPI == EPI_QKV || PRO == PRO_ATTN) {
+    if (a.hd == 64) { hipLaunchKernelGGL((k_gemv<PRO, EPI, R, U, WAVES, PERSIST, false, KS, 64, false, true>), dim3(grid), dim3(WAVES * 64), lds, s, a); return; }
+  }
+  hipLaunchKernelGGL((k_gemv<PRO, EPI, R, U, WAVES, PERSIST, false, KS, 128, false, true>), dim3(grid), dim3(WAVES * 64), lds, s, a);
+}
+#define WV(PRO, EPI, R, U, W) return launch_gemv_w13_t<PRO, EPI, R, U, W>(a, s)
+#define WVP(PRO, EPI, R, U, W, BPC) return launch_gemv_w13_t<PRO, EPI, R, U, W, true, 1, BPC>(a, s)
+#define WVK(PRO, EPI, R, U, W, KS) return launch_gemv_w13_t<PRO, EPI, R, U, W, false, KS>(a, s)
+bool gemv_w13_has(int pro, int epi, int v) {
+  if (pro == PRO_RMSNORM && (epi == EPI_QKV || epi == EPI_SWIGLU)) return v >= 0 && v <= 5;
+  if (pro == PRO_COPY && epi == EPI_RESID) return v >= 0 && v <= 6;
+  if (pro == PRO_ATTN && epi == EPI_RESID) return v >= 0 && v <= 2;
+  if (pro == PRO_RMSNORM && epi == EPI_LOGITS) return v >= 0 && v <= 4;
+  if ((pro == PRO_RMSNORM || pro == PRO_COPY) && epi == EPI_STORE) return v == 0;
+  return false;
+}
+void launch_gemv_w13_variant(int pro, int epi, int v, const GemvArgs& a, hipStream_t s) {
+  if (pro == PRO_RMSNORM && epi == EPI_QKV) {
+    switch (v) { default: WV(PRO_RMSNORM, EPI_QKV, 1, 4, 4); case 1: WV(PRO_RMSNORM, EPI_QKV, 2, 4, 4); case 2: WV(PRO_RMSNORM, EPI_QKV, 1, 4, 8);
+                 case 3: WVP(PRO_RMSNORM, EPI_QKV, 1, 4, 8, 2); case 4: WV(PRO_RMSNORM, EPI_QKV, 1, 8, 4);
+                 case 5: WVP(PRO_RMSNORM, EPI_QKV, 1, 4, 4, 4); }
+  }
+  if (pro == PRO_RMSNORM && epi == EPI_SWIGLU) {
+    switch (v) { default: WV(PRO_RMSNORM, EPI_SWIGLU, 1, 4, 4); case 1: WV(PRO_RMSNORM, EPI_SWIGLU, 2, 4, 4); case 2: WV(PRO_RMSNORM, EPI_SWIGLU, 1, 4, 8);
+                 case 3: WVP(PRO_RMSNORM, EPI_SWIGLU, 1, 4, 8, 2); case 4: WV(PRO_RMSNORM, EPI_SWIGLU, 1, 8, 4);
+                 case 5: WVP(PRO_RMSNORM, EPI_SWIGLU, 1, 4, 4, 4); }
+  }
+  if (pro == PRO_COPY && epi == EPI_RESID) {
+    switch (v) { default: WV(PRO_COPY, EPI_RESID, 1, 8, 8); case 1: WV(PRO_COPY, EPI_RESID, 1, 4, 8); case 2: WV(PRO_COPY, EPI_RESID, 2, 4, 4);
+                 case 3: WVK(PRO_COPY, EPI_RESID, 1, 4, 8, 2); case 4: WVK(PRO_COPY, EPI_RESID, 2, 4, 8, 2);
+                 case 5: WV(PRO_COPY, EPI_RESID, 1, 4, 4); case 6: WV(PRO_COPY, EPI_RESID, 1, 4, 16); }
+  }
+  if (pro == PRO_ATTN && epi == EPI_RESID) {
+    switch (v) { default: WVK(PRO_ATTN, EPI_RESID, 2, 4, 16, 2); case 1: WV(PRO_ATTN, EPI_RESID, 2, 4, 8); case 2: WV(PRO_ATTN, EPI_RESID, 2, 4, 4); }
+  }
+  if (pro == PRO_RMSNORM && epi == EPI_LOGITS) {
+    switch (v) { default: WV(PRO_RMSNORM, EPI_LOGITS, 1, 4, 4); case 1: WV(PRO_RMSNORM, EPI_LOGITS, 2, 4, 4); case 2: WVP(PRO_RMSNORM, EPI_LOGITS, 1, 4, 8, 2);
+                 case 3: WVP(PRO_RMSNORM, EPI_LOGITS, 2, 4, 8, 2); case 4: WV(PRO_RMSNORM, EPI_LOGITS, 2, 4, 8); }
+  }
+  if (pro == PRO_RMSNORM && epi == EPI_STORE) WV(PRO_RMSNORM, EPI_STORE, 2, 4, 4);
+  if (pro == PRO_COPY && epi == EPI_STORE) WV(PRO_COPY, EPI_STORE, 2, 4, 4);
+  fprintf(stderr, "launch_gemv_w13: no 13-bit kernel for prologue %d, epilogue %d\n", pro, epi);
+  abort();
+}
+#undef WV
+#undef WVP
+#undef WVK
+static int w13_shape_for(int pro, int epi, int v, const GemvArgs& a) {
+  const GemvShape sh = gemv_variant_shape(pro, epi, v);
+  if (pro == PRO_ATTN) return -1;
+  if (pro == PRO_COPY && epi == EPI_RESID) {
+    if (a.K == a.d) return -1;
+    if (sh.ks == 1) return 1;
+    return (sh.ks == 2 && sh.U == 4) ? 3 : -1;
+  }
+  if (pro == PRO_RMSNORM && (epi == EPI_QKV || epi == EPI_SWIGLU)) return sh.waves == 4 ? 5 : (sh.waves == 8 ? 3 : -1);
+  if (pro == PRO_RMSNORM && epi == EPI_LOGITS) return sh.waves == 4 ? 1 : (sh.waves == 8 ? 4 : -1);
+  if (pro == PRO_RMSNORM && epi == EPI_STORE) return sh.waves == 4 ? 0 : -1;
+  if (pro == PRO_COPY && epi == EPI_STORE) return 0;
+  return -1;
+}
+
+__global__ __launch_bounds__(256) void k_pack_w13_rows(const bf16_t* W, uint8_t* Wp, uint8_t* Wh, unsigned* bad_rows, int N, int K) {
+  const int row = blockIdx.x, tid = threadIdx.x;
+  const u32x4* w4 = reinterpret_cast<const u32x4*>(W + (size_t)row * K);
+  unsigned char* out = Wp + (size_t)row * w13_row_bytes(K);
+  __shared__ int red[4];
+  __shared__ int any_bad;
+  const int K8 = K >> 3, J2 = w13_units(K), J4 = w13_blocks(K);
+  int hb = 0;
+  for (int c = tid; c < K8; c += 256) {
+    const u32x4 v = w4[c];
+#pragma unroll
+    for (int e = 0; e < 4; ++e) hb = max(hb, max((int)((v[e] >> 8) & 0x7fu), (int)((v[e] >> 24) & 0x7fu)));
+  }
+#pragma unroll
+  for (int off = 32; off >= 1; off >>= 1) hb = max(hb, __shfl_xor(hb, off));
+  if ((tid & 63) == 0) red[tid >> 6] = hb;
+  if (tid == 0) any_bad = 0;
+  __syncthreads();
+  hb = max(max(red[0], red[1]), max(red[2], red[3]));
+  if (tid == 0) Wh[row] = (uint8_t)hb;
+  const int lo = w13_lo(hb);
+  int bad = 0;
+  for (int t = tid; t < J4 * 64; t += 256) {
+    const int b = t >> 6, l = t & 63;
+    uint32_t sg = 0;
+#pragma unroll
+    for (int h = 0; h < 2; ++h) {
+      const int j = 2 * b + h;
+      if (j >= J2) break;
+      u32x4 lv;
+      u32x2 nv;
+#pragma unroll
+      for (int i2 = 0; i2 < 2; ++i2) {
+        const int i = 2 * h + i2, c = 256 * b + 64 * i + l;
+        u32x4 v = {0u, 0u, 0u, 0u};
+        if (c < K8) v = w4[c];
+        uint32_t la = 0, lb = 0, n = 0;
+#pragma unroll
+        for (int k = 0; k < 8; ++k) {
+          unsigned wk = (v[k >> 1] >> (16 * (k & 1))) & 0xffffu;
+          int code = w13_code(wk, lo);
+          if (code < 0) { ++bad; code = 0; wk = 0; }
+          const int kb = 8 * (k & 3);
+          if (k < 4) la |= (wk & 0xffu) << kb; else lb |= (wk & 0xffu) << kb;
+          n |= (uint32_t)code << (kb + 4 * (k >> 2));
+          sg |= (wk >> 15) << (kb + 2 * i + (k >> 2));
+        }
+        lv[2 * i2] = la; lv[2 * i2 + 1] = lb; nv[i2] = n;
+      }
+      reinterpret_cast<u32x4*>(out)[j * 64 + l] = lv;
+      reinterpret_cast<u32x2*>(out + w13_n_off(K))[j * 64 + l] = nv;
+    }
+    reinterpret_cast<uint32_t*>(out + w13_s_off(K))[b * 64 + l] = sg;
+  }
+  if (bad) atomicOr(&any_bad, 1);
+  __syncthreads();
+  if (tid == 0 && any_bad) atomicAdd(bad_rows, 1u);
+}
+void launch_pack_w13_rows(const bf16_t* W, uint8_t* Wp, uint8_t* Wh, unsigned* bad_rows, int N, int K, hipStream_t s) {
+  hipLaunchKernelGGL(k_pack_w13_rows, dim3(N), dim3(256), 0, s, W, Wp, Wh, bad_rows, N, K);
+}
+
 static int g_variant[8] = {0, 0, 0, 0, 0, -1, 0, 0};
 void set_gemv_default_variant(int epi, int variant) { if (epi >= 0 && epi < 8) g_variant[epi] = variant; }
 
-void launch_gemv(int pro, int epi, const GemvArgs& a, hipStream_t s) {
-  if (a.W4) return launch_gemv_q4(pro, epi, a, s);
-  if (a.W8) return launch_gemv_f8(pro, epi, a, s);
-  if (pro == PRO_ATTN) {
-    const int v = g_variant[6] ? g_variant[6] : (a.d > 2048 ? 8 : 1);
-    return launch_gemv_variant(pro, epi, v, a, s);
-  }
+static int gemv_chosen_variant(int pro, int epi, const GemvArgs& a) {
+  if (pro == PRO_ATTN) return g_variant[6] ? g_variant[6] : (a.d > 2048 ? 8 : 1);
   int v = g_variant[epi & 7];
   const bool o_proj = epi == EPI_RESID && a.K == a.d;
   if (o_proj && g_variant[5] >= 0) v = g_variant[5];
@@ -558,8 +701,18 @@
     if (epi == EPI_RESID) v = 10;
     else if (epi == EPI_LOGITS) v = 3;
   }
+  return v;
+}
+
+void launch_gemv(int pro, int epi, const GemvArgs& a, hipStream_t s) {
+  if (a.W4) return launch_gemv_q4(pro, epi, a, s);
+  if (a.W8) return launch_gemv_f8(pro, epi, a, s);
+  const int v = gemv_chosen_variant(pro, epi, a);
+  const int v13 = a.Wp ? w13_shape_for(pro, epi, v, a) : -1;
+  if (v13 >= 0) return launch_gemv_w13_variant(pro, epi, v13, a, s);
   launch_gemv_variant(pro, epi, v, a, s);
 }
+bool gemv_w13_takes(int pro, int epi, const GemvArgs& a) { return w13_shape_for(pro, epi, gemv_chosen_variant(pro, epi, a), a) >= 0; }
 
 __global__ __launch_bounds__(256) void k_attn_decode(AttnDecArgs a) {
   const int h = blockIdx.x, sp = blockIdx.y;
diff --git a/detikzify_amd/csrc/w13.h b/detikzify_amd/csrc/w13.h
--- /dev/null
+++ b/detikzify_amd/csrc/w13.h
@@ -0,0 +1,63 @@
+#pragma once
+#include <stddef.h>
+#include <stdint.h>
+
+#if defined(__HIPCC__) || defined(__CUDACC__)
+#define W13_HD __host__ __device__
+#else
+#define W13_HD
+#endif
+
+W13_HD static inline int w13_units(int K) { return ((K >> 3) + 127) >> 7; }
+W13_HD static inline int w13_blocks(int K) { return (w13_units(K) + 1) >> 1; }
+W13_HD static inline size_t w13_n_off(int K) { return (size_t)w13_units(K) * 1024; }
+W13_HD static inline size_t w13_s_off(int K) { return (size_t)w13_units(K) * 1536; }
+W13_HD static inline size_t w13_row_bytes(int K) { return (size_t)w13_units(K) * 1536 + (size_t)w13_blocks(K) * 256; }
+W13_HD static inline int w13_lo(int hb) { return hb > 15 ? hb - 15 : 0; }
+
+struct W13Pos { size_t l, n, s; int nshift, sbit; };
+W13_HD static inline W13Pos w13_pos(int K, int k) {
+  const int c = k >> 3, e = k & 7, lane = c & 63;
+  W13Pos p;
+  p.l = (size_t)((c >> 7) * 64 + lane) * 16 + (size_t)(((c >> 6) & 1) * 8 + e);
+  p.n = w13_n_off(K) + (size_t)((c >> 7) * 64 + lane) * 8 + (size_t)(((c >> 6) & 1) * 4 + (e & 3));
+  p.nshift = (e >> 2) * 4;
+  p.s = w13_s_off(K) + (size_t)((c >> 8) * 64 + lane) * 4 + (size_t)(e & 3);
+  p.sbit = 2 * ((c >> 6) & 3) + (e >> 2);
+  return p;
+}
+
+static inline int w13_row_hb(const uint16_t* w, int K) {
+  int hb = 0;
+  for (int k = 0; k < K; ++k) { const int q = (w[k] >> 8) & 0x7f; if (q > hb) hb = q; }
+  return hb;
+}
+W13_HD static inline int w13_code(unsigned w, int lo) {
+  const int q = (int)((w >> 8) & 0x7fu);
+  if (q == 0) return 0;
+  return q > lo ? q - lo : -1;
+}
+static inline int w13_pack_row(const uint16_t* w, int K, uint8_t* row, uint8_t* hb_out) {
+  const int hb = w13_row_hb(w, K), lo = w13_lo(hb);
+  int bad = 0;
+  const size_t nb = w13_row_bytes(K);
+  for (size_t i = 0; i < nb; ++i) row[i] = 0;
+  for (int k = 0; k < K; ++k) {
+    const int code = w13_code(w[k], lo);
+    if (code < 0) { ++bad; continue; }
+    const W13Pos p = w13_pos(K, k);
+    row[p.l] = (uint8_t)(w[k] & 0xff);
+    row[p.n] = (uint8_t)(row[p.n] | (code << p.nshift));
+    row[p.s] = (uint8_t)(row[p.s] | (((w[k] >> 15) & 1) << p.sbit));
+  }
+  *hb_out = (uint8_t)hb;
+  return bad;
+}
+static inline void w13_unpack_row(const uint8_t* row, int hb, int K, uint16_t* w) {
+  const int lo = w13_lo(hb);
+  for (int k = 0; k < K; ++k) {
+    const W13Pos p = w13_pos(K, k);
+    const int code = (row[p.n] >> p.nshift) & 15, sign = (row[p.s] >> p.sbit) & 1;
+    w[k] = (uint16_t)((sign << 15) | ((code ? lo + code : 0) << 8) | row[p.l]);
+  }
+}
diff --git a/include/dtk.h b/include/dtk.h
--- a/include/dtk.h
+++ b/include/dtk.h
@@ -83,7 +83,7 @@
   uint32_t last_batch_step_slots;
   uint32_t device_errors;
   uint32_t last_batch_step_fp8_mfma;
-  uint32_t reserved0;
+  uint32_t w13_counts;
 } dtk_stats;
 
 int  dtk_abi_version(void);
@@ -303,6 +303,10 @@
                       const uint16_t* x, const uint16_t* norm_w, const uint16_t* rope_cos, const uint16_t* rope_sin,
                       int S, const float* pm, const float* pl, const float* po, int scratch_fill,
                       uint16_t* q_io, uint16_t* k_io, uint16_t* v_io, uint16_t* y_io, float* logits_io);
+int  dtk_w13_row_bytes(int K);
+int  dtk_w13_pack_host(const uint16_t* W, int N, int K, uint8_t* planes, uint8_t* hb, int32_t* bad);
+int  dtk_w13_unpack_host(const uint8_t* planes, const uint8_t* hb, int N, int K, uint16_t* W);
+int  dtk_w13_op_bad_rows(dtk_ctx* ctx);
 int  dtk_op_layernorm(dtk_ctx* ctx, const uint16_t* X, const uint16_t* w, const uint16_t* b,
                       int M, int D, float eps, uint16_t* Y);
 int  dtk_op_sample(dtk_ctx* ctx, const float* logits, int V, int step, int64_t* token_out,
```

Measured after the change: 400.2 tokens/s, median of 6. 1.05x the previous value.
